# bminixhofer/zett

Measured on AMD Instinct MI355X. Metric: predicted token-embeddings/sec (full target vocab), higher is better.
Workload: dtype f16

## Files before the change

### include/zett_hip.h

```cpp
#ifndef ZETT_HIP_H
#define ZETT_HIP_H

#include <stdint.h>

#ifdef __cplusplus
extern "C" {
#endif

#define ZETT_ABI_VERSION 8

enum zett_status {
    ZETT_OK = 0,
    ZETT_E_INVALID = -1,
    ZETT_E_HIP = -2,
    ZETT_E_STATE = -3,
    ZETT_E_INDEX = -4,
    ZETT_E_NOT_IMPLEMENTED = -5,
    ZETT_E_KEY = -6,
    ZETT_E_RANGE = -7
};

enum zett_range_bits {
    ZETT_RANGE_SOURCE = 1,
    ZETT_RANGE_ACTIVATION = 2,
    ZETT_RANGE_OUTPUT = 4,
    ZETT_RANGE_WEIGHT = 8,
    ZETT_RANGE_DEST = 16
};

enum zett_dtype { ZETT_F32 = 0, ZETT_F16 = 1, ZETT_BF16 = 2 };

enum zett_precision { ZETT_PREC_BF16 = 0, ZETT_PREC_F32 = 1, ZETT_PREC_F16 = 2 };

typedef struct zett_config {
    int32_t n_embd;
    int32_t n_in_embd;
    int32_t hidden;
    int32_t intermediate;
    int32_t heads;
    int32_t layers;
    int32_t n_extra;
    int32_t original_vocab_size;
    int32_t pad_token_id;
    int32_t separate_out;
    int32_t single_head;
    int32_t rescale;
    int32_t predict_bias;
    int32_t embed_lang;
    int32_t n_langs;
    int32_t max_positions;
    float ln_eps_encoder;
    float ln_eps_projector;
} zett_config;

typedef struct zett_stats {
    int64_t rows;
    int64_t packed_tokens;
    int64_t distinct_ids;
    int64_t chunks;
    double executed_flops;
    double gemm_ms;
    int64_t gemm_launches;
    double gemm_flops_timed;
    int64_t distinct_positions;
} zett_stats;

typedef struct zett_hypernet zett_hypernet;
typedef struct zett_retok zett_retok;
typedef struct zett_lexical zett_lexical;

const char* zett_last_error(void);
int zett_abi_version(void);


int zett_create(const zett_config* cfg, int device, int precision, zett_hypernet** out);
int zett_destroy(zett_hypernet* h);

int zett_load_weight(zett_hypernet* h, const char* name, const void* data, int dtype,
                     const int64_t* shape, int ndim);

int zett_finalize(zett_hypernet* h);

int zett_forward(zett_hypernet* h, const int32_t* surface_forms, int64_t n_rows, int32_t seq,
                 const void* source_embeddings, int src_dtype, int64_t v_src, int32_t lang_index,
                 float* out_in, float* out_out, float* out_bias, void* stream);

typedef struct zett_dest {
    void* in; void* out; void* bias;
    int32_t dtype; int32_t bias_dtype;
    int64_t ld_in; int64_t ld_out;
    const int64_t* rows;
    int64_t n_dest_rows;
} zett_dest;
int zett_forward_into(zett_hypernet* h, const int32_t* surface_forms, int64_t n_rows, int32_t seq,
                      const void* source_embeddings, int src_dtype, int64_t v_src, int32_t lang_index,
                      const zett_dest* dest, void* stream);

int zett_forward_prepare(zett_hypernet* h, const int32_t* surface_forms, int64_t n_rows, int32_t seq, void* input_stream);

int zett_get_stats(const zett_hypernet* h, zett_stats* out);

typedef struct zett_gemm_record {
    int32_t m, n, k;
    int32_t variant;
    int32_t epilogue;
    float ms;
    double flops;
    double bytes;
} zett_gemm_record;
int zett_get_gemm_log(const zett_hypernet* h, zett_gemm_record* out, int64_t capacity, int64_t* count);

int zett_check_range(zett_hypernet* h, void* stream, int32_t* flags);

enum zett_output { ZETT_OUT_IN = 0, ZETT_OUT_BIAS = 1 };
int zett_stream_wait_output(zett_hypernet* h, int which, void* stream);

int zett_workspace_bytes(const zett_hypernet* h, int64_t n_rows, int32_t seq, int64_t* out_bytes);

int zett_set_option(zett_hypernet* h, const char* key, int64_t value);

int zett_partition_workspace_bytes(int64_t n_rows, int32_t n_ids, int64_t* out_bytes);
int zett_partition_rows(const int32_t* surface_forms, int64_t n_rows, int32_t seq, int32_t pad_id, int32_t n_ids, int32_t world,
                        const int32_t* caps, int32_t* perm_out, void* workspace, int64_t workspace_bytes, int32_t device, void* stream);
int zett_scatter_rows(const void* src, void* dst, const int64_t* order, int64_t n_rows, int64_t row_bytes, int32_t device, void* stream);

int zett_table_plan(zett_hypernet* h, const int32_t* surface_forms, int64_t n_rows, int32_t seq, int32_t* id_slot_out, int32_t* id_list_out,
                    int64_t* n_ids_out, void* stream);
int zett_table_rows(zett_hypernet* h, const int32_t* id_list, int64_t first, int64_t count, const void* source_embeddings, int src_dtype,
                    int64_t v_src, void* table_out, float* stats_out, void* stream);
int zett_forward_table(zett_hypernet* h, const int32_t* surface_forms, int64_t n_rows, int32_t seq, const void* table, const float* table_stats,
                       const int32_t* id_slot, int32_t lang_index, float* out_in, float* out_out, float* out_bias, void* stream);
int zett_forward_table_into(zett_hypernet* h, const int32_t* surface_forms, int64_t n_rows, int32_t seq, const void* table,
                            const float* table_stats, const int32_t* id_slot, int32_t lang_index, const zett_dest* dest, void* stream);


enum zett_retok_kind { ZETT_RETOK_BPE = 0, ZETT_RETOK_UNIGRAM = 1, ZETT_RETOK_WORDPIECE = 2 };

typedef struct zett_retok_model {
    int32_t kind;
    int32_t n_pieces;
    const uint8_t* piece_bytes;
    const int32_t* piece_offsets;
    const int32_t* piece_ids;
    const double* piece_scores;
    double unigram_min_score;
    int32_t n_merges;
    const int32_t* merges;
    int32_t unk_id;
    int32_t fuse_unk;
    int32_t byte_fallback;
    const int32_t* byte_fallback_ids;
    int32_t ignore_merges;
    int32_t n_special;
    const uint8_t* special_bytes;
    const int32_t* special_offsets;
    const int32_t* special_ids;
    const uint8_t* piece_continuing;
    int32_t max_input_chars_per_word;
} zett_retok_model;

int zett_retok_create(const zett_retok_model* model, int device, zett_retok** out);
int zett_retok_destroy(zett_retok* r);
int zett_retok_set_option(zett_retok* r, const char* key, int64_t value);

int zett_retokenize(zett_retok* r, const uint8_t* token_chars, const int32_t* offsets,
                    int64_t n_tokens, int32_t maxlen, int32_t pad_id, int32_t* out,
                    int64_t* n_truncated, int64_t* bad_token, void* stream);

int zett_retokenize_async(zett_retok* r, const uint8_t* token_chars, const int32_t* offsets, int64_t n_tokens, int64_t n_text,
                          int32_t maxlen, int32_t pad_id, int32_t* out, void* stream);
int zett_retok_result(zett_retok* r, int64_t* n_truncated, int64_t* bad_call, int64_t* bad_token);

enum zett_lexical_mode { ZETT_LEXICAL_NO = 0, ZETT_LEXICAL_FVT = 1, ZETT_LEXICAL_BFVT = 2 };

int zett_lexical_create(const zett_retok_model* model, int32_t n_vocab, const uint8_t* vocab_bytes, const int32_t* vocab_offsets,
                        const int32_t* vocab_ids, int device, zett_lexical** out);
int zett_lexical_destroy(zett_lexical* h);

int zett_lexical_plan(zett_lexical* h, const uint8_t* token_chars, int64_t n_tokens, int64_t n_text, int64_t n_source_rows, int32_t fvt_mode,
                      int32_t width, int32_t* ids, int32_t* count, int64_t* n_overlap, int64_t* n_wide, int64_t* n_ids, int64_t* bad_token,
                      void* stream);

int zett_lexical_rows_into(zett_lexical* h, const int32_t* ids, const int32_t* count, int64_t n_tokens, int32_t width, const void* src_in,
                           int64_t ld_src_in, const void* src_out, int64_t ld_src_out, int32_t src_dtype, int64_t n_source_rows, int32_t n_embd,
                           int64_t fallback_id, const zett_dest* dest, void* stream);

int zett_op_gemm_f32(const float* a, int32_t lda, const float* w, int32_t ldw, int64_t m, int32_t n, int32_t k, const float* bias, int32_t act,
                     const float* residual, int32_t ld_res, float* out, int32_t ld_out, void* stream);
int zett_op_gemm_lo(int32_t prec, const void* a, int32_t lda, const void* w, int32_t ldw, int64_t m, int32_t n, int32_t k, const float* bias, int32_t act,
                    const float* residual, int32_t ld_res, float* out, int32_t ld_out, void* stream);
int zett_op_convert_lo(int32_t prec, const float* in, int32_t ld_in, void* out, int32_t ld_out, int64_t rows, int32_t cols, int32_t cols_padded, void* stream);
int zett_op_transpose_lo(int32_t prec, const float* in, int32_t ld_in, void* out, int32_t ld_out, int64_t rows, int32_t cols, int64_t rows_padded, void* stream);
int zett_op_transpose_lo16(int32_t prec, const void* in, int32_t ld_in, void* out, int32_t ld_out, int64_t rows, int32_t cols, int64_t rows_padded, void* stream);
int zett_op_grad_operands_lo(int32_t prec, const float* dy, int32_t ld, const float* act_z, int32_t ld_z, int32_t act_kind, int64_t rows, int32_t cols,
                             int64_t rows_padded, void* dy_lo, int32_t ld_lo, void* dy_t, int32_t ld_t, float* colsum_part, void* stream);
int zett_op_transpose_f32(const float* in, int32_t ld_in, float* out, int32_t ld_out, int64_t rows, int32_t cols, int64_t rows_padded, void* stream);
int zett_op_colsum_f32(const float* in, int32_t ld, int64_t rows, int32_t cols, float* out, int32_t accumulate, void* stream);
int zett_op_elementwise_f32(int32_t op, const float* a, const float* b, const float* vec, const float* vec2, const float* s, float* out,
                            int64_t n, int32_t cols, void* stream);
int zett_op_rowdot_f32(const float* a, int32_t ld, const float* w, const float* b, float* out, int64_t rows, int32_t cols, void* stream);
int zett_op_layernorm_fwd_f32(const float* x, int32_t ld, const float* gamma, const float* beta, float eps, float* y, float* stats,
                              int64_t rows, int32_t h, void* y_lo, int32_t prec, void* stream);
int zett_op_layernorm_bwd_f32(const float* dy, const float* dy2, const float* x, int32_t ld, const float* stats, const float* gamma, float* dx,
                              float* partials, int32_t n_part, int64_t rows, int32_t h, void* stream);
int zett_op_gelu_fwd_f32(const float* z, float* h, int64_t n, int32_t kind, void* stream);
int zett_op_gelu_bwd_f32(const float* z, const float* dh, float* dz, int64_t n, int32_t kind, void* stream);
int zett_op_gelu_fwd_lo(int32_t prec, const float* z, void* h_lo, int64_t n, int32_t kind, void* stream);
int zett_op_attention_fwd_f32(const float* q, int32_t ldq, const float* k, const float* v, int32_t ld, const uint8_t* mask, const int32_t* row_offset,
                              int64_t n_rows, int32_t seq, int32_t heads, int32_t head_dim, int32_t cls_only, float* ctx, int32_t ld_ctx, float* probs,
                              void* ctx_lo, int32_t prec, void* stream);
int zett_op_attention_bwd_f32(const float* dctx, int32_t ld_ctx, const float* q, int32_t ldq, const float* k, const float* v, int32_t ld, const float* probs,
                              const int32_t* row_offset, int64_t n_rows, int32_t seq, int32_t heads, int32_t head_dim, int32_t cls_only, float* dq, int32_t ld_dq,
                              float* dk, float* dv, int32_t ld_d, void* stream);
int zett_op_gather_rows_f32(const float* a, const float* src, int32_t ld_src, const int32_t* idx, float* out, int64_t rows, int32_t cols, void* stream);
int zett_op_scatter_add_rows_f32(float* dst, int32_t ld_dst, const int32_t* idx, const float* src, int64_t rows, int32_t cols, void* stream);
int zett_op_gather_fwd_f32(const int32_t* ids, int64_t n_tokens, const void* src, int32_t src_dtype, int32_t e_in, int32_t v0, const float* fallback,
                           const float* sw, const float* sb, float* x, void* stream);
int zett_op_gather_bwd_f32(const int32_t* ids, int64_t n_tokens, const void* src, int32_t src_dtype, int32_t e_in, int32_t v0, const float* dx,
                           float* dfallback, float* prod, float* keep, void* stream);
int zett_op_gather_bwd_rows_f32(const int32_t* ids, int64_t n_tokens, const void* src, int32_t src_dtype, int32_t e_in, int32_t v0, const float* dx, float* prod,
                                float* keep, void* stream);

enum zett_ln_kernel {
    ZETT_LN_ROWS8_32 = 0,
    ZETT_LN_ROWS8_64 = 1,
    ZETT_LN_WAVE = 2,
    ZETT_LN_WORKGROUP = 3
};
int zett_op_fwd_layernorm(int32_t prec, const float* in, const void* in_lo, int32_t ld_in, int32_t rows, int32_t h, const float* gamma, const float* beta,
                          float eps, int32_t ln_rows8, float* out_f32, void* out_lo, float* stats, const float* bias_w, const float* bias_b, void* out_bias,
                          const int64_t* bias_rows, int32_t bias_dtype, int32_t* range_flag, int32_t* kernel_id, void* stream);
int zett_op_fwd_embed_layernorm(int32_t prec, const float* table, const void* table_lo, const float* table_stats, const float* table_gamma, const float* table_beta,
                                const int32_t* tok_slot, const int32_t* tok_pos, const float* type0, const float* pos_emb, const float* lang, int32_t lang_pos,
                                const int32_t* tok_row, const int32_t* row_offset, int64_t row0, int32_t rows, int32_t tok0, int32_t m, int32_t h, const float* gamma,
                                const float* beta, float eps, int32_t ln_rows8, void* out_lo, float* stats, float* sum, int32_t* kernel_id, void* stream);
int zett_op_fwd_attention(int32_t prec, const void* q, int64_t ldq, const void* k, const void* v, int64_t ldkv, int32_t h, int32_t head_dim,
                          const int32_t* row_offset, const uint8_t* row_uniform, const uint8_t* tok_key, int64_t row0, int32_t rows, int32_t tok0, float scaling,
                          int32_t flags, const int32_t* tok_pair, void* ctx, void* stream);
int zett_op_fwd_gather_src(int32_t prec, const int32_t* id_list, int32_t slot0, int32_t n_slots, const void* src, int32_t src_dtype, int32_t e_in, int32_t v0,
                           const float* fallback, const float* sc_w, const float* sc_b, void* out, int32_t* range_flag, void* stream);
int zett_op_fwd_ln_stats(int32_t prec, const float* parts, int32_t ld_part, int32_t rows, int32_t h, float eps, float* stats, void* stream);
int zett_op_fwd_fold_weight(int32_t prec, const float* w, int32_t n, int32_t k, const float* gamma, const float* beta, const float* bias, void* w_fold,
                            float* c_out, float* b_out, int32_t* range_flag, void* stream);

enum zett_distance { ZETT_DIST_MSE = 0, ZETT_DIST_RMSE = 1, ZETT_DIST_HUBER = 2 };
enum zett_loss_mode { ZETT_LOSS_MEAN = 0, ZETT_LOSS_LEXICAL = 1 };
enum zett_adamw_flags { ZETT_ADAMW_DECAY = 1, ZETT_ADAMW_FROZEN = 2 };
#define ZETT_MT_CHUNK 65536
int zett_op_single_token_mask(const void* ids, int32_t ids_bytes, int64_t n, int32_t width, int64_t ld, int64_t pad_token_id, float* mask, void* stream);
int zett_op_embed_dist_rows(const float* pred, int64_t ld_pred, const void* src, int32_t src_dtype, int64_t ld_src, int64_t src_rows, int32_t col0, const void* ids,
                            int32_t ids_bytes, int64_t ids_stride, const float* mask, int64_t n, int32_t e, int32_t kind, float* row_dist, float* row_tnorm,
                            void* stream);
int zett_op_embed_dist_finalize(const float* row_dist, const float* row_tnorm, const float* mask, int64_t n, int32_t mode, float* record, void* stream);
// ... 128 lines not shown
```

### zett_amd/_lib.py

```python
from __future__ import annotations

import ctypes as C
import os
import threading

from .build import LIB_PATH

ZETT_OK = 0
E_INVALID, E_HIP, E_STATE, E_INDEX, E_NOT_IMPLEMENTED, E_KEY, E_RANGE = -1, -2, -3, -4, -5, -6, -7
RANGE_SOURCE, RANGE_ACTIVATION, RANGE_OUTPUT, RANGE_WEIGHT, RANGE_DEST = 1, 2, 4, 8, 16
DTYPE_F32, DTYPE_F16, DTYPE_BF16 = 0, 1, 2
PREC_BF16, PREC_F32, PREC_F16 = 0, 1, 2
RETOK_BPE, RETOK_UNIGRAM, RETOK_WORDPIECE = 0, 1, 2
OUT_IN, OUT_BIAS = 0, 1
LEXICAL_NO, LEXICAL_FVT, LEXICAL_BFVT = 0, 1, 2
DIST_MSE, DIST_RMSE, DIST_HUBER = 0, 1, 2
LOSS_MEAN, LOSS_LEXICAL = 0, 1
ADAMW_DECAY, ADAMW_FROZEN = 1, 2
MT_CHUNK = 65536
CE_AUTO, CE_ONCE, CE_TWICE = 0, 1, 2
CE_ONCE_MAX_COLS = 32768
SPLICE_MAX_ROWS = 256
EMBED_BWD_CHUNK = 64
BATCH_POSITIVES_ONLY, BATCH_RANDOM = 0, 1
BATCH_BAD_ID, BATCH_OVERFLOW, BATCH_BAD_ORDER, BATCH_REPEAT = 1, 2, 4, 8
LABEL_CLM, LABEL_MLM = 0, 1
LABEL_BAD_ID = 1
LABEL_WORKSPACE_BYTES = 16384
ENCODE_MAX_TEMPLATE = 8
ENCODE_MARKS_ARE_LETTERS, ENCODE_RESPLIT = 1, 2
ENCODE_PREFIX_NONE, ENCODE_PREFIX_ALWAYS, ENCODE_PREFIX_UNLESS_SPACE = 0, 1, 2
ENCODE_NO_UNK, ENCODE_BAD_OFFSETS = 1, 2
SAMPLE_BAD_OFFSETS, SAMPLE_TABLE_FULL, SAMPLE_LIST_FULL, SAMPLE_SUM_OVERFLOW, SAMPLE_OUT_FULL = 2, 4, 8, 16, 32
VOCAB_NOT_A_SAMPLE, VOCAB_DUPLICATE, VOCAB_TABLE_FULL, VOCAB_OUT_FULL = 1, 2, 4, 8
VOCAB_SCORES_THROUGH_JSON = 1
SAMPLED_VOCAB_KEY_BYTES = 64

ABI_SYMBOLS = (
    "zett_last_error", "zett_abi_version", "zett_create", "zett_destroy", "zett_load_weight",
    "zett_finalize", "zett_forward", "zett_get_stats", "zett_workspace_bytes", "zett_set_option",
    "zett_retok_create", "zett_retok_destroy", "zett_retokenize", "zett_check_range", "zett_get_gemm_log",
    "zett_stream_wait_output", "zett_forward_prepare", "zett_retokenize_async", "zett_retok_result", "zett_retok_set_option",
    "zett_partition_rows", "zett_partition_workspace_bytes", "zett_scatter_rows",
    "zett_table_plan", "zett_table_rows", "zett_forward_table",
    "zett_forward_into", "zett_forward_table_into",
    "zett_lexical_create", "zett_lexical_destroy", "zett_lexical_plan", "zett_lexical_rows_into",
    "zett_op_gemm_f32", "zett_op_transpose_f32", "zett_op_colsum_f32", "zett_op_elementwise_f32", "zett_op_rowdot_f32",
    "zett_op_layernorm_fwd_f32", "zett_op_layernorm_bwd_f32", "zett_op_gelu_fwd_f32", "zett_op_gelu_bwd_f32",
    "zett_op_attention_fwd_f32", "zett_op_attention_bwd_f32", "zett_op_gather_fwd_f32", "zett_op_gather_bwd_f32",
    "zett_op_gather_rows_f32", "zett_op_scatter_add_rows_f32", "zett_op_gemm_lo", "zett_op_convert_lo", "zett_op_transpose_lo", "zett_op_grad_operands_lo", "zett_op_transpose_lo16", "zett_op_gelu_fwd_lo",
    "zett_op_single_token_mask", "zett_op_embed_dist_rows", "zett_op_embed_dist_finalize", "zett_op_embed_dist_grad", "zett_op_grad_norm", "zett_op_adamw",
    "zett_op_ce_addend", "zett_op_ce_rows", "zett_op_ce_finalize", "zett_op_ce_colsum", "zett_op_ce_scale", "zett_op_ce_cast",
    "zett_op_splice_rows", "zett_op_embed_lookup", "zett_op_embed_lookup_workspace_bytes", "zett_op_embed_lookup_plan", "zett_op_embed_lookup_bwd",
    "zett_op_batch_vocab_workspace_bytes", "zett_op_batch_vocab",
    "zett_op_label_batch", "zett_op_pad_vocabulary",
    "zett_encode_workspace_bytes", "zett_encode_texts",
    "zett_sampler_create", "zett_sampler_destroy", "zett_sampler_depth", "zett_sampler_workspace_bytes", "zett_sampler_sample", "zett_sampler_table",
    "zett_retok_create_unigram_device", "zett_sampled_vocab_workspace_bytes", "zett_sampled_vocab_build", "zett_sampled_vocab_commit", "zett_sampled_vocab_table",
    "zett_sampled_vocab_patch_rows",
    "zett_op_embed_lookup_plan_base", "zett_op_gather_bwd_rows_f32",
    "zett_op_fwd_layernorm", "zett_op_fwd_embed_layernorm", "zett_op_fwd_attention", "zett_op_fwd_gather_src", "zett_op_fwd_ln_stats", "zett_op_fwd_fold_weight",
)


class ZettConfig(C.Structure):
    _fields_ = [(n, C.c_int32) for n in (
        "n_embd", "n_in_embd", "hidden", "intermediate", "heads", "layers", "n_extra",
        "original_vocab_size", "pad_token_id", "separate_out", "single_head", "rescale",
        "predict_bias", "embed_lang", "n_langs", "max_positions")] + [
        ("ln_eps_encoder", C.c_float), ("ln_eps_projector", C.c_float)]


ABI_VERSION = 8


class ZettStats(C.Structure):
    _fields_ = [("rows", C.c_int64), ("packed_tokens", C.c_int64), ("distinct_ids", C.c_int64),
                ("chunks", C.c_int64), ("executed_flops", C.c_double), ("gemm_ms", C.c_double),
                ("gemm_launches", C.c_int64), ("gemm_flops_timed", C.c_double), ("distinct_positions", C.c_int64)]


class ZettGemmRecord(C.Structure):
    _fields_ = [("m", C.c_int32), ("n", C.c_int32), ("k", C.c_int32), ("variant", C.c_int32), ("epilogue", C.c_int32),
                ("ms", C.c_float), ("flops", C.c_double), ("bytes", C.c_double)]


class ZettDest(C.Structure):
    _fields_ = [("in_", C.c_void_p), ("out", C.c_void_p), ("bias", C.c_void_p), ("dtype", C.c_int32), ("bias_dtype", C.c_int32),
                ("ld_in", C.c_int64), ("ld_out", C.c_int64), ("rows", C.c_void_p), ("n_dest_rows", C.c_int64)]


class ZettSampledVocabRecord(C.Structure):
    _fields_ = [("n_vocab", C.c_int32), ("n_removed", C.c_int32), ("n_text", C.c_int32), ("status", C.c_int32), ("min_score", C.c_double), ("table_min_score", C.c_double)]


class ZettRetokModel(C.Structure):
    _fields_ = [
        ("kind", C.c_int32), ("n_pieces", C.c_int32),
        ("piece_bytes", C.c_void_p), ("piece_offsets", C.c_void_p), ("piece_ids", C.c_void_p),
        ("piece_scores", C.c_void_p), ("unigram_min_score", C.c_double),
        ("n_merges", C.c_int32), ("merges", C.c_void_p),
        ("unk_id", C.c_int32), ("fuse_unk", C.c_int32), ("byte_fallback", C.c_int32),
        ("byte_fallback_ids", C.c_void_p), ("ignore_merges", C.c_int32),
        ("n_special", C.c_int32), ("special_bytes", C.c_void_p), ("special_offsets", C.c_void_p),
        ("special_ids", C.c_void_p),
        ("piece_continuing", C.c_void_p), ("max_input_chars_per_word", C.c_int32),
    ]


_lib = None
_lock = threading.Lock()


def lib_path() -> str:
    return os.environ.get("ZETT_HIP_LIB", LIB_PATH)


def load():
    global _lib
    if _lib is not None:
        return _lib
    with _lock:
        if _lib is not None:
            return _lib
        path = lib_path()
        if not os.path.exists(path):
            raise RuntimeError(
                f"{path} is missing: the HIP extension has not been built. Run "
                "`python -m zett_amd.build` (needs hipcc); zett_amd has no CPU fallback.")
        lib = C.CDLL(path)
        lib.zett_last_error.restype = C.c_char_p
        lib.zett_abi_version.restype = C.c_int
        lib.zett_create.argtypes = [C.POINTER(ZettConfig), C.c_int, C.c_int, C.POINTER(C.c_void_p)]
        lib.zett_destroy.argtypes = [C.c_void_p]
        lib.zett_load_weight.argtypes = [C.c_void_p, C.c_char_p, C.c_void_p, C.c_int, C.POINTER(C.c_int64), C.c_int]
        lib.zett_finalize.argtypes = [C.c_void_p]
        lib.zett_forward.argtypes = [C.c_void_p, C.c_void_p, C.c_int64, C.c_int32, C.c_void_p, C.c_int, C.c_int64,
                                     C.c_int32, C.c_void_p, C.c_void_p, C.c_void_p, C.c_void_p]
        lib.zett_get_stats.argtypes = [C.c_void_p, C.POINTER(ZettStats)]
        lib.zett_workspace_bytes.argtypes = [C.c_void_p, C.c_int64, C.c_int32, C.POINTER(C.c_int64)]
        lib.zett_set_option.argtypes = [C.c_void_p, C.c_char_p, C.c_int64]
        lib.zett_check_range.argtypes = [C.c_void_p, C.c_void_p, C.POINTER(C.c_int32)]
        lib.zett_stream_wait_output.argtypes = [C.c_void_p, C.c_int, C.c_void_p]
        lib.zett_get_gemm_log.argtypes = [C.c_void_p, C.POINTER(ZettGemmRecord), C.c_int64, C.POINTER(C.c_int64)]
        lib.zett_retok_create.argtypes = [C.POINTER(ZettRetokModel), C.c_int, C.POINTER(C.c_void_p)]
        lib.zett_retok_destroy.argtypes = [C.c_void_p]
        lib.zett_retok_set_option.argtypes = [C.c_void_p, C.c_char_p, C.c_int64]
        lib.zett_retokenize.argtypes = [C.c_void_p, C.c_void_p, C.c_void_p, C.c_int64, C.c_int32, C.c_int32,
                                        C.c_void_p, C.POINTER(C.c_int64), C.POINTER(C.c_int64), C.c_void_p]
        lib.zett_retokenize_async.argtypes = [C.c_void_p, C.c_void_p, C.c_void_p, C.c_int64, C.c_int64, C.c_int32, C.c_int32,
                                              C.c_void_p, C.c_void_p]
        lib.zett_retok_result.argtypes = [C.c_void_p, C.POINTER(C.c_int64), C.POINTER(C.c_int64), C.POINTER(C.c_int64)]
        lib.zett_forward_prepare.argtypes = [C.c_void_p, C.c_void_p, C.c_int64, C.c_int32, C.c_void_p]
        lib.zett_table_plan.argtypes = [C.c_void_p, C.c_void_p, C.c_int64, C.c_int32, C.c_void_p, C.c_void_p, C.POINTER(C.c_int64), C.c_void_p]
        lib.zett_table_rows.argtypes = [C.c_void_p, C.c_void_p, C.c_int64, C.c_int64, C.c_void_p, C.c_int, C.c_int64, C.c_void_p, C.c_void_p, C.c_void_p]
        lib.zett_forward_table.argtypes = [C.c_void_p, C.c_void_p, C.c_int64, C.c_int32, C.c_void_p, C.c_void_p, C.c_void_p, C.c_int32,
                                           C.c_void_p, C.c_void_p, C.c_void_p, C.c_void_p]
        lib.zett_forward_into.argtypes = [C.c_void_p, C.c_void_p, C.c_int64, C.c_int32, C.c_void_p, C.c_int, C.c_int64, C.c_int32,
                                          C.POINTER(ZettDest), C.c_void_p]
        lib.zett_forward_table_into.argtypes = [C.c_void_p, C.c_void_p, C.c_int64, C.c_int32, C.c_void_p, C.c_void_p, C.c_void_p, C.c_int32,
                                                C.POINTER(ZettDest), C.c_void_p]
        lib.zett_lexical_create.argtypes = [C.POINTER(ZettRetokModel), C.c_int32, C.c_void_p, C.c_void_p, C.c_void_p, C.c_int, C.POINTER(C.c_void_p)]
        lib.zett_lexical_destroy.argtypes = [C.c_void_p]
        lib.zett_lexical_plan.argtypes = [C.c_void_p, C.c_void_p, C.c_int64, C.c_int64, C.c_int64, C.c_int32, C.c_int32, C.c_void_p, C.c_void_p,
                                          C.POINTER(C.c_int64), C.POINTER(C.c_int64), C.POINTER(C.c_int64), C.POINTER(C.c_int64), C.c_void_p]
        lib.zett_lexical_rows_into.argtypes = [C.c_void_p, C.c_void_p, C.c_void_p, C.c_int64, C.c_int32, C.c_void_p, C.c_int64, C.c_void_p, C.c_int64,
                                               C.c_int32, C.c_int64, C.c_int32, C.c_int64, C.POINTER(ZettDest), C.c_void_p]
        lib.zett_partition_workspace_bytes.argtypes = [C.c_int64, C.c_int32, C.POINTER(C.c_int64)]
        lib.zett_scatter_rows.argtypes = [C.c_void_p, C.c_void_p, C.c_void_p, C.c_int64, C.c_int64, C.c_int32, C.c_void_p]
        lib.zett_partition_rows.argtypes = [C.c_void_p, C.c_int64, C.c_int32, C.c_int32, C.c_int32, C.c_int32, C.POINTER(C.c_int32),
                                            C.c_void_p, C.c_void_p, C.c_int64, C.c_int32, C.c_void_p]
        P, I32, I64, F = C.c_void_p, C.c_int32, C.c_int64, C.c_float
        lib.zett_op_gemm_f32.argtypes = [P, I32, P, I32, I64, I32, I32, P, I32, P, I32, P, I32, P]
        lib.zett_op_transpose_f32.argtypes = [P, I32, P, I32, I64, I32, I64, P]
        lib.zett_op_gemm_lo.argtypes = [I32, P, I32, P, I32, I64, I32, I32, P, I32, P, I32, P, I32, P]
        lib.zett_op_convert_lo.argtypes = [I32, P, I32, P, I32, I64, I32, I32, P]
        lib.zett_op_transpose_lo.argtypes = [I32, P, I32, P, I32, I64, I32, I64, P]
        lib.zett_op_grad_operands_lo.argtypes = [I32, P, I32, P, I32, I32, I64, I32, I64, P, I32, P, I32, P, P]
        lib.zett_op_transpose_lo16.argtypes = [I32, P, I32, P, I32, I64, I32, I64, P]
        lib.zett_op_gelu_fwd_lo.argtypes = [I32, P, P, I64, I32, P]
        lib.zett_op_colsum_f32.argtypes = [P, I32, I64, I32, P, I32, P]
        lib.zett_op_elementwise_f32.argtypes = [I32, P, P, P, P, P, P, I64, I32, P]
        lib.zett_op_rowdot_f32.argtypes = [P, I32, P, P, P, I64, I32, P]
        lib.zett_op_layernorm_fwd_f32.argtypes = [P, I32, P, P, F, P, P, I64, I32, P, I32, P]
        lib.zett_op_layernorm_bwd_f32.argtypes = [P, P, P, I32, P, P, P, P, I32, I64, I32, P]
        lib.zett_op_gelu_fwd_f32.argtypes = [P, P, I64, I32, P]
        lib.zett_op_gelu_bwd_f32.argtypes = [P, P, P, I64, I32, P]
        lib.zett_op_attention_fwd_f32.argtypes = [P, I32, P, P, I32, P, P, I64, I32, I32, I32, I32, P, I32, P, P, I32, P]
        lib.zett_op_attention_bwd_f32.argtypes = [P, I32, P, I32, P, P, I32, P, P, I64, I32, I32, I32, I32, P, I32, P, P, I32, P]
        lib.zett_op_gather_rows_f32.argtypes = [P, P, I32, P, P, I64, I32, P]
        lib.zett_op_scatter_add_rows_f32.argtypes = [P, I32, P, P, I64, I32, P]
        lib.zett_op_gather_fwd_f32.argtypes = [P, I64, P, I32, I32, I32, P, P, P, P, P]
        lib.zett_op_gather_bwd_f32.argtypes = [P, I64, P, I32, I32, I32, P, P, P, P, P]
        lib.zett_op_gather_bwd_rows_f32.argtypes = [P, I64, P, I32, I32, I32, P, P, P, P]
        D = C.c_double
        lib.zett_op_single_token_mask.argtypes = [P, I32, I64, I32, I64, I64, P, P]
        lib.zett_op_embed_dist_rows.argtypes = [P, I64, P, I32, I64, I64, I32, P, I32, I64, P, I64, I32, I32, P, P, P]
        lib.zett_op_embed_dist_finalize.argtypes = [P, P, P, I64, I32, P, P]
        lib.zett_op_embed_dist_grad.argtypes = [P, I64, P, I32, I64, I64, I32, P, I32, I64, P, P, I64, I32, I32, P, P, P, I64, I32, P]
        lib.zett_op_grad_norm.argtypes = [P, P, I32, D, D, D, P, I64, P, P]
        lib.zett_op_adamw.argtypes = [P, P, P, P, P, P, I32, D, D, D, D, D, I32, P, P]
        lib.zett_op_ce_addend.argtypes = [P, P, P, I32, I32, P, P]
        lib.zett_op_ce_rows.argtypes = [P, I64, P, P, I64, I32, I32, P, I32, I64, P, P, P, I32, P]
        lib.zett_op_ce_finalize.argtypes = [P, P, P, P, I64, P, P]
        lib.zett_op_ce_colsum.argtypes = [P, I32, I64, I64, I32, P, I32, P]
        lib.zett_op_ce_scale.argtypes = [P, I64, P, P, P, I32, P]
        lib.zett_op_ce_cast.argtypes = [P, I32, I64, P, I32, I64, I64, I32, I32, P]
        lib.zett_op_splice_rows.argtypes = [P, I64, P, I64, I64, I32, P, I32, I64, I64, I32, P, P, I32, P]
        lib.zett_op_embed_lookup.argtypes = [P, I32, I64, I64, I32, P, I32, I64, P, I32, P, P]
        lib.zett_op_embed_lookup_workspace_bytes.argtypes = [I64, I64, I32, C.POINTER(I64), C.POINTER(I64), C.POINTER(I64)]
        lib.zett_op_embed_lookup_plan.argtypes = [P, I32, I64, I64, P, I64, P, I64, P]
        lib.zett_op_embed_lookup_plan_base.argtypes = [P, I32, I64, I64, I64, P, I64, P, I64, P]
        lib.zett_op_embed_lookup_bwd.argtypes = [P, I32, I64, I64, I32, P, I64, P, I64, P, I64, P]
        lib.zett_op_batch_vocab_workspace_bytes.argtypes = [I64, I64, I64, C.POINTER(I64)]
        lib.zett_op_batch_vocab.argtypes = [P, I32, P, I32, I64, I64, I64, P, I32, I64, I32, P, P, I32, I32, P, P, P, I32, P, P, P, P, P, P, P, P, P, I64, P]
        U64 = C.c_uint64
        lib.zett_op_label_batch.argtypes = [P, I32, I64, I64, I32, P, I32, P, I32, I64, I64, I64, I64, I32, U64, U64, U64, U64, P, I64, P, P, P, P, P, I64, P]
        lib.zett_op_pad_vocabulary.argtypes = [P, I32, I64, I32, I64, I64, P, I32, P, P, P, P, P]
        lib.zett_encode_workspace_bytes.argtypes = [I64, I64, C.POINTER(I64)]
        lib.zett_encode_texts.argtypes = [P, P, P, I64, I64, P, I64, I32, I32, I32, P, I32, P, I32, P, P, I32, I32, P, P, I32, I64, P, I64, P, P]
        lib.zett_sampler_create.argtypes = [C.c_int, I32, I64, I64, I64, C.POINTER(P)]
        lib.zett_sampler_destroy.argtypes = [P]
        lib.zett_sampler_depth.argtypes = [P, C.POINTER(I32)]
        lib.zett_sampler_workspace_bytes.argtypes = [I64, I64, C.POINTER(I64)]
        lib.zett_sampler_sample.argtypes = [P, P, P, I64, I64, P, I64, I64, I32, I32, C.c_double, C.c_uint64, I32, I32, P, P, P, I64, P, P, I64, P, P]
        lib.zett_sampler_table.argtypes = [P, P, P, P, P, I64, P, P]
        lib.zett_retok_create_unigram_device.argtypes = [C.c_int, I64, C.POINTER(P)]
        lib.zett_sampled_vocab_workspace_bytes.argtypes = [I64, I32, C.POINTER(I64)]
        lib.zett_sampled_vocab_build.argtypes = [P, P, P, P, P, I64, I64, P, P, P, P, P, I32, I32, I32, P, P, P, I64, P, I64, P, I32, P, I64, P]
        lib.zett_sampled_vocab_commit.argtypes = [P, P]
        lib.zett_sampled_vocab_table.argtypes = [P, P, P, P, P, P, I64, P, P]
        lib.zett_sampled_vocab_patch_rows.argtypes = [P, P, P, P, I32, P, I64, I32, I32, P]
        lib.zett_op_fwd_layernorm.argtypes = [I32, P, P, I32, I32, I32, P, P, F, I32, P, P, P, P, P, P, P, I32, P, C.POINTER(I32), P]
        lib.zett_op_fwd_embed_layernorm.argtypes = [I32, P, P, P, P, P, P, P, P, P, P, I32, P, P, I64, I32, I32, I32, I32, P, P, F, I32, P, P, P, C.POINTER(I32), P]
        lib.zett_op_fwd_attention.argtypes = [I32, P, I64, P, P, I64, I32, I32, P, P, P, I64, I32, I32, F, I32, P, P, P]
        lib.zett_op_fwd_gather_src.argtypes = [I32, P, I32, I32, P, I32, I32, I32, P, P, P, P, P, P]
        lib.zett_op_fwd_ln_stats.argtypes = [I32, P, I32, I32, I32, F, P, P]
        lib.zett_op_fwd_fold_weight.argtypes = [I32, P, I32, I32, P, P, P, P, P, P, P, P]
        for name in ABI_SYMBOLS:
            fn = getattr(lib, name)
            if name != "zett_last_error":
                fn.restype = C.c_int
        if lib.zett_abi_version() != ABI_VERSION:
            raise RuntimeError(f"{path} has ABI version {lib.zett_abi_version()}, this package expects {ABI_VERSION}: "
                               "rebuild it (`python -m zett_amd.build`)")
        _lib = lib
    return _lib


class RangeError(OverflowError):
    """ZETT_E_RANGE: a value left the range of the 16-bit operand type, or an output is not finite."""


def check(rc: int, what: str = "") -> None:
    if rc == ZETT_OK:
        return
    msg = load().zett_last_error().decode("utf-8", "replace")
    if what:
        msg = f"{what}: {msg}"
    if rc == E_INDEX:
        raise IndexError(msg)
    if rc == E_NOT_IMPLEMENTED:
        raise NotImplementedError(msg)
    if rc == E_KEY:
        raise KeyError(msg)
    if rc == E_INVALID:
        raise ValueError(msg)
    if rc == E_RANGE:
        raise RangeError(msg)
    raise RuntimeError(msg)
```

### zett_amd/csrc/rowops.hip.h

```cpp
#pragma once

#include <hip/hip_runtime.h>
#include <stdint.h>

#include <type_traits>

#include "gemm.hip.h"
#include "scan.hip.h"

namespace zett {



struct PlanArrays {
    int32_t* row_count;
    int32_t* row_offset;
    uint8_t* row_uniform;
    int32_t* id_flag;
    int32_t* id_slot;
    int32_t* id_list;
    int32_t* tok_slot;
    int32_t* tok_pos;
    int32_t* tok_row;
    int32_t* tok_pkey;
    int32_t* pair_flag;
    int32_t* pair_slot;
    int32_t* tok_pair;
    int32_t* pair_tslot;
    int32_t* pair_pos;
    uint8_t* tok_key;
    int32_t* err;
    int32_t* counters;
    int32_t n_pair_keys;
};

static __global__ void plan_rows_kernel(const int32_t* __restrict__ sfm, int64_t n_rows, int seq, int pad, int lam,
                                 int n_ids, PlanArrays p) {
    const int64_t n = (int64_t)blockIdx.x * blockDim.x + threadIdx.x;
    if (n >= n_rows) return;
    const int32_t* row = sfm + n * seq;
    int visible = 0;
    for (int j = 0; j < seq; ++j) {
        const int id = row[j];
        if (id < 0 || id >= n_ids) {
            atomicMax(p.err, (int)(n < 0x7ffffffe ? n + 1 : 0x7fffffff));
            p.row_count[n] = 0;
            p.row_uniform[n] = 2;
            return;
        }
        visible += (id != pad);
    }
    const bool uniform = (visible + lam) == 0;
    int count;
    if (uniform) {
        count = seq;
        for (int j = 0; j < seq; ++j) p.id_flag[row[j]] = 1;
    } else {
        count = visible + lam + (row[0] == pad ? 1 : 0);
        for (int j = 0; j < seq; ++j)
            if (j == 0 || row[j] != pad) p.id_flag[row[j]] = 1;
    }
    p.row_count[n] = count;
    p.row_uniform[n] = uniform ? 1 : 0;
}

static __global__ __launch_bounds__(1024) void exclusive_scan_kernel(const int32_t* __restrict__ in,
                                                              int32_t* __restrict__ out, int64_t n) {
    __shared__ int32_t s_waves[16];
    const int t = threadIdx.x;
    const int64_t per = (n + 1023) / 1024;
    const int64_t b = (int64_t)t * per, e = (b + per < n) ? b + per : n;
    int32_t s = 0;
    for (int64_t i = b; i < e; ++i) s += in[i];
    int32_t total;
    int32_t run = block_exclusive_scan<1024>(s, s_waves, &total);
    for (int64_t i = b; i < e; ++i) { const int32_t v = in[i]; out[i] = run; run += v; }
    if (t == 1023) out[n] = total;
}

constexpr int SCAN_CHUNK = 4096;

static __global__ __launch_bounds__(256) void scan_chunk_sums_kernel(const int32_t* __restrict__ in, int64_t n, int32_t* __restrict__ sums) {
    __shared__ int32_t s_waves[4];
    const int64_t base = (int64_t)blockIdx.x * SCAN_CHUNK + threadIdx.x * 16;
    int32_t s = 0;
#pragma unroll
    for (int k = 0; k < 16; ++k) { const int64_t i = base + k; if (i < n) s += in[i]; }
    int32_t total;
    block_exclusive_scan<256>(s, s_waves, &total);
    if (threadIdx.x == 0) sums[blockIdx.x] = total;
}

static __global__ __launch_bounds__(256) void scan_apply_kernel(const int32_t* __restrict__ in, int64_t n, const int32_t* __restrict__ offs,
                                                         int32_t* __restrict__ out) {
    __shared__ int32_t s_waves[4];
    const int64_t base = (int64_t)blockIdx.x * SCAN_CHUNK + threadIdx.x * 16;
    int32_t v[16];
    int32_t s = 0;
#pragma unroll
    for (int k = 0; k < 16; ++k) { const int64_t i = base + k; v[k] = i < n ? in[i] : 0; s += v[k]; }
    int32_t run = offs[blockIdx.x] + block_exclusive_scan<256>(s, s_waves);
#pragma unroll
    for (int k = 0; k < 16; ++k) { const int64_t i = base + k; if (i < n) out[i] = run; run += v[k]; }
    if (blockIdx.x == gridDim.x - 1 && threadIdx.x == 0) out[n] = offs[gridDim.x];
}

inline void launch_exclusive_scan(const int32_t* in, int32_t* out, int64_t n, int32_t* scratch, hipStream_t st) {
    if (n <= SCAN_CHUNK * 4) {
        hipLaunchKernelGGL(exclusive_scan_kernel, dim3(1), dim3(1024), 0, st, in, out, n);
        return;
    }
    const int chunks = (int)((n + SCAN_CHUNK - 1) / SCAN_CHUNK);
    int32_t* sums = scratch;
    int32_t* offs = scratch + chunks;
    hipLaunchKernelGGL(scan_chunk_sums_kernel, dim3(chunks), dim3(256), 0, st, in, n, sums);
    hipLaunchKernelGGL(exclusive_scan_kernel, dim3(1), dim3(1024), 0, st, (const int32_t*)sums, offs, (int64_t)chunks);
    hipLaunchKernelGGL(scan_apply_kernel, dim3(chunks), dim3(256), 0, st, in, n, (const int32_t*)offs, out);
}

static __global__ void plan_tokens_kernel(const int32_t* __restrict__ sfm, int64_t n_rows, int seq, int pad, int lam,
                                   int n_ids, PlanArrays p) {
    const int64_t n = (int64_t)blockIdx.x * blockDim.x + threadIdx.x;
    if (n >= n_rows) return;
    const int32_t* row = sfm + n * seq;
    int t = p.row_offset[n];
    if (p.row_uniform[n] == 2) return;
    const bool uniform = p.row_uniform[n] == 1;
    const int lp = seq + lam;
    for (int j = 0; j < seq; ++j) {
        const int id = row[j];
        const bool vis = id != pad;
        if (uniform || vis || j == 0) {
            p.tok_slot[t] = p.id_slot[id];
            p.tok_pos[t] = j;
            p.tok_row[t] = (int32_t)n;
            p.tok_key[t] = vis ? 1 : 0;
            if (p.pair_flag) { const int key = id * lp + j; p.tok_pkey[t] = key; p.pair_flag[key] = 1; }
            ++t;
        }
    }
    if (lam) {
        p.tok_slot[t] = -1;
        p.tok_pos[t] = seq;
        p.tok_row[t] = (int32_t)n;
        p.tok_key[t] = 1;
        if (p.pair_flag) { const int key = n_ids * lp + seq; p.tok_pkey[t] = key; p.pair_flag[key] = 1; }
    }
}

static __global__ void plan_pairs_kernel(int64_t n_rows, PlanArrays p) {
    const int64_t t = (int64_t)blockIdx.x * blockDim.x + threadIdx.x;
    if (t >= p.row_offset[n_rows]) return;
    const int ps = p.pair_slot[p.tok_pkey[t]];
    p.tok_pair[t] = ps;
    p.pair_tslot[ps] = p.tok_slot[t];
    p.pair_pos[ps] = p.tok_pos[t];
}

__device__ __forceinline__ int chunk_row(int t_rel, int row_rel, bool first, int rows);
static __global__ void pair_rows_kernel(int m, int tok0, int64_t row0, int rows, PlanArrays p, int32_t* __restrict__ brow_pair) {
    const int t = blockIdx.x * blockDim.x + threadIdx.x;
    if (t >= m) return;
    const int n = p.tok_row[tok0 + t];
    brow_pair[chunk_row(t, (int)(n - row0), p.row_offset[n] == tok0 + t, rows)] = p.tok_pair[tok0 + t];
}

static __global__ void plan_idlist_kernel(int n_ids, PlanArrays p) {
    const int id = blockIdx.x * blockDim.x + threadIdx.x;
    if (id < n_ids && p.id_flag[id]) p.id_list[p.id_slot[id]] = id;
    if (id == 0) {
        p.counters[0] = p.id_slot[n_ids];
        p.counters[1] = p.err[0];
        p.counters[2] = p.n_pair_keys ? p.pair_slot[p.n_pair_keys] : 0;
    }
}

__device__ __forceinline__ float wave_sum(float v) {
#pragma unroll
    for (int off = 32; off > 0; off >>= 1) v += __shfl_xor(v, off, 64);
    return v;
}

__device__ __forceinline__ float block_sum_256(float v, float* red ) {
    v = wave_sum(v);
    __syncthreads();
    if ((threadIdx.x & 63) == 0) red[threadIdx.x >> 6] = v;
    __syncthreads();
    return red[0] + red[1] + red[2] + red[3];
}

template <typename T> __device__ __forceinline__ void store_lo4(T* dst, float4 v);
template <> __device__ __forceinline__ void store_lo4<float>(float* dst, float4 v) { *(float4*)dst = v; }
template <> __device__ __forceinline__ void store_lo4<bf16_t>(bf16_t* dst, float4 v) {
    *(uint2*)dst = make_uint2(pack2_lo<bf16_t>(v.x, v.y), pack2_lo<bf16_t>(v.z, v.w));
}
template <> __device__ __forceinline__ void store_lo4<f16_t>(f16_t* dst, float4 v) {
    *(uint2*)dst = make_uint2(pack2_lo<f16_t>(v.x, v.y), pack2_lo<f16_t>(v.z, v.w));
}

template <int SRC_DTYPE> __device__ __forceinline__ float4 load_src4(const void* base, size_t elem);
template <> __device__ __forceinline__ float4 load_src4<0>(const void* base, size_t e) {
    return *(const float4*)((const float*)base + e);
}
template <> __device__ __forceinline__ float4 load_src4<1>(const void* base, size_t e) {
    const uint2 u = *(const uint2*)((const uint16_t*)base + e);
    typedef __attribute__((ext_vector_type(4))) _Float16 f16x4;
    const f16x4 hv = __builtin_bit_cast(f16x4, u);
    return make_float4((float)hv[0], (float)hv[1], (float)hv[2], (float)hv[3]);
}
template <> __device__ __forceinline__ float4 load_src4<2>(const void* base, size_t e) {
    const uint2 u = *(const uint2*)((const uint16_t*)base + e);
    return make_float4(__uint_as_float(u.x << 16), __uint_as_float(u.x & 0xffff0000u),
                       __uint_as_float(u.y << 16), __uint_as_float(u.y & 0xffff0000u));
}

template <typename T, int SRC_DTYPE>
__global__ __launch_bounds__(256) void gather_src_kernel(const int32_t* __restrict__ id_list, int slot0, int n_slots,
                                                         const void* __restrict__ src, int e_in, int v0,
                                                         const float* __restrict__ fallback,
                                                         const float* __restrict__ sc_w, const float* __restrict__ sc_b,
                                                         T* __restrict__ out, int32_t* __restrict__ range_flag) {
    const int s = blockIdx.x;
    if (s >= n_slots) return;
    const int id = id_list[slot0 + s];
    T* dst = out + (size_t)s * e_in;
    bool bad = false;
    auto chk = [&](float4 v) {
        if (LoRange<T>::checked)
            bad |= out_of_range(v.x, LoRange<T>::limit) | out_of_range(v.y, LoRange<T>::limit) | out_of_range(v.z, LoRange<T>::limit) |
                   out_of_range(v.w, LoRange<T>::limit);
    };
    if (id >= v0) {
        const float* f = fallback + (size_t)(id - v0) * e_in;
        for (int c = threadIdx.x * 4; c < e_in; c += 1024) { const float4 v = *(const float4*)(f + c); chk(v); store_lo4<T>(dst + c, v); }
    } else {
        const size_t base = (size_t)id * e_in;
        for (int c = threadIdx.x * 4; c < e_in; c += 1024) {
            float4 v = load_src4<SRC_DTYPE>(src, base + c);
            if (sc_w) {
                const float4 w = *(const float4*)(sc_w + c), b = *(const float4*)(sc_b + c);
                v.x = w.x * v.x + b.x; v.y = w.y * v.y + b.y; v.z = w.z * v.z + b.z; v.w = w.w * v.w + b.w;
            }
            chk(v);
            store_lo4<T>(dst + c, v);
        }
    }
    range_report(range_flag, bad, ZETT_RANGE_BIT_SOURCE);
}

struct LnEmbed {
    const float* table;
    const int32_t* tok_slot;
    const int32_t* tok_pos;
    const float* type0;
    const float* pos_emb;
    const float* lang;
    int lang_pos;
    const int32_t* tok_row;
    const int32_t* row_offset;
    int64_t row0;
    int rows;
    const void* table_lo;
    const float* table_stats;
    const float* table_gamma;
    const float* table_beta;
};

__device__ __forceinline__ int chunk_row(int t_rel, int row_rel, bool first, int rows) {
    return first ? row_rel : rows + t_rel - row_rel - 1;
}

struct LnReadout {
    const float* bias_w;
    const float* bias_b;
    float* out_bias;
    const void* in_lo;
    const int64_t* bias_rows;
    int32_t* range_flag;
};

template <typename BT> __device__ __forceinline__ void ln_readout_store(const LnReadout& ro, int r, float v) {
    if constexpr (std::is_void<BT>::value) {
        ro.out_bias[r] = v;
    } else {
        const int64_t d = ro.bias_rows ? ro.bias_rows[r] : (int64_t)r;
        if (d < 0) return;
        ((BT*)ro.out_bias)[d] = to_lo<BT>(v);
        range_report(ro.range_flag, dest_overflow<BT>(v), ZETT_RANGE_BIT_DEST);
    }
}

constexpr int LN_MAX_VEC = 8;

template <typename T, bool EMBED, int TPR = 256, bool READOUT = false, typename BT = void>
__global__ __launch_bounds__(256) void layernorm_rows_kernel(const float* __restrict__ in, int ld_in, int rows, int H,
                                                             const float* __restrict__ gamma,
                                                             const float* __restrict__ beta, float eps,
                                                             float* __restrict__ out_f32, T* __restrict__ out_lo,
                                                             float* __restrict__ stats_out, float* __restrict__ sum_out,
                                                             LnEmbed emb, int tok0, LnReadout readout) {
    __shared__ float red[4];
    const int r = blockIdx.x * (256 / TPR) + (int)threadIdx.x / TPR;
    if (r >= rows) return;
    const int nvec = H >> 2;
    const int tid = threadIdx.x % TPR;
    auto row_sum = [&](float x_) { return TPR == 256 ? block_sum_256(x_, red) : wave_sum(x_); };
    const float* x = nullptr;
    const float* posr = nullptr;
    bool is_lang = false;
    int ro = r;
    const T* tbl_lo = nullptr;
    float2 tbl_st = make_float2(0.f, 1.f);
    if constexpr (EMBED) {
        const int slot = emb.tok_slot[tok0 + r];
        is_lang = slot < 0;
        if (emb.table_lo && !is_lang) {
            tbl_lo = (const T*)emb.table_lo + (size_t)slot * H;
            tbl_st = *(const float2*)(emb.table_stats + 2 * (size_t)slot);
            x = emb.lang;
        } else
        x = is_lang ? emb.lang : emb.table + (size_t)slot * H;
        posr = emb.pos_emb + (size_t)emb.tok_pos[tok0 + r] * H;
        if (emb.tok_row) {
            const int n = emb.tok_row[tok0 + r];
            ro = chunk_row(r, (int)(n - emb.row0), emb.row_offset[n] == tok0 + r, emb.rows);
        }
    } else {
        x = in + (size_t)r * ld_in;
    }
    auto load = [&](int v) -> float4 {
        if constexpr (READOUT && sizeof(T) == 2) {
            if (readout.in_lo) {
                const uint2 u = *(const uint2*)((const T*)readout.in_lo + (size_t)r * ld_in + v * 4);
                float4 a;
                unpack2_lo<T>(u.x, a.x, a.y); unpack2_lo<T>(u.y, a.z, a.w);
                return a;
            }
        }
        float4 a;
        if constexpr (EMBED && sizeof(T) == 2) {
            if (tbl_lo) {
                const uint2 u = *(const uint2*)(tbl_lo + v * 4);
                unpack2_lo<T>(u.x, a.x, a.y); unpack2_lo<T>(u.y, a.z, a.w);
                const float4 g = *(const float4*)(emb.table_gamma + v * 4), b = *(const float4*)(emb.table_beta + v * 4);
                a = make_float4(ln_affine(a.x, tbl_st.x, tbl_st.y, g.x, b.x), ln_affine(a.y, tbl_st.x, tbl_st.y, g.y, b.y),
                                ln_affine(a.z, tbl_st.x, tbl_st.y, g.z, b.z), ln_affine(a.w, tbl_st.x, tbl_st.y, g.w, b.w));
            } else {
                a = *(const float4*)(x + v * 4);
            }
        } else {
            a = *(const float4*)(x + v * 4);
        }
        if constexpr (EMBED) {
            const float4 t0 = *(const float4*)(emb.type0 + v * 4);
            const float4 p = *(const float4*)(posr + v * 4);
            if (is_lang) {
                const float4 pl = *(const float4*)(emb.pos_emb + (size_t)emb.lang_pos * H + v * 4);
                a.x -= (t0.x + pl.x); a.y -= (t0.y + pl.y); a.z -= (t0.z + pl.z); a.w -= (t0.w + pl.w);
            }
            a.x = (a.x + t0.x) + p.x; a.y = (a.y + t0.y) + p.y; a.z = (a.z + t0.z) + p.z; a.w = (a.w + t0.w) + p.w;
        }
        return a;
    };
    float4 v[LN_MAX_VEC];
    float s = 0.f;
#pragma unroll
    for (int j = 0; j < LN_MAX_VEC; ++j) {
        const int idx = tid + TPR * j;
        if (idx < nvec) { v[j] = load(idx); s += (v[j].x + v[j].y) + (v[j].z + v[j].w); }
    }
    for (int idx = tid + TPR * LN_MAX_VEC; idx < nvec; idx += TPR) { const float4 a = load(idx); s += (a.x + a.y) + (a.z + a.w); }
    const float mean = row_sum(s) / (float)H;
    float q = 0.f;
#pragma unroll
    for (int j = 0; j < LN_MAX_VEC; ++j) {
        const int idx = tid + TPR * j;
        if (idx < nvec) {
            const float a = v[j].x - mean, b = v[j].y - mean, c = v[j].z - mean, d = v[j].w - mean;
            q += (a * a + b * b) + (c * c + d * d);
        }
    }
    for (int idx = tid + TPR * LN_MAX_VEC; idx < nvec; idx += TPR) {
        const float4 t = load(idx);
        const float a = t.x - mean, b = t.y - mean, c = t.z - mean, d = t.w - mean;
        q += (a * a + b * b) + (c * c + d * d);
    }
    const float var = row_sum(q) / (float)H;
    const float rstd = 1.0f / sqrtf(var + eps);
    if (stats_out && tid == 0) *(float2*)(stats_out + 2 * (size_t)ro) = make_float2(mean, rstd);
    float dot = 0.f;
    auto emit = [&](int idx, float4 a) {
        const float4 g = *(const float4*)(gamma + idx * 4), b = *(const float4*)(beta + idx * 4);
        const float4 o = make_float4(ln_affine(a.x, mean, rstd, g.x, b.x), ln_affine(a.y, mean, rstd, g.y, b.y),
                                     ln_affine(a.z, mean, rstd, g.z, b.z), ln_affine(a.w, mean, rstd, g.w, b.w));
        if (EMBED && sum_out) *(float4*)(sum_out + (size_t)ro * H + idx * 4) = a;
        if (out_f32) *(float4*)(out_f32 + (size_t)ro * H + idx * 4) = o;
        if (out_lo) store_lo4<T>(out_lo + (size_t)ro * H + idx * 4, o);
        if (READOUT && readout.bias_w) {
            const float4 w = *(const float4*)(readout.bias_w + idx * 4);
            dot += (o.x * w.x + o.y * w.y) + (o.z * w.z + o.w * w.w);
        }
    };
#pragma unroll
    for (int j = 0; j < LN_MAX_VEC; ++j) {
        const int idx = tid + TPR * j;
        if (idx < nvec) emit(idx, v[j]);
    }
    for (int idx = tid + TPR * LN_MAX_VEC; idx < nvec; idx += TPR) emit(idx, load(idx));
    if constexpr (READOUT) {
        if (readout.out_bias) {
            const float tot = row_sum(dot);
            if (tid == 0) ln_readout_store<BT>(readout, r, readout.bias_w ? tot + readout.bias_b[0] : 0.f);
        }
    }
}

template <typename T> struct Vec8 { float v[8]; };

template <typename T> __device__ __forceinline__ void load8(const T* p, float (&o)[8]);
template <> __device__ __forceinline__ void load8<float>(const float* p, float (&o)[8]) {
    const float4 a = *(const float4*)p, b = *(const float4*)(p + 4);
    o[0] = a.x; o[1] = a.y; o[2] = a.z; o[3] = a.w; o[4] = b.x; o[5] = b.y; o[6] = b.z; o[7] = b.w;
}
template <typename T> __device__ __forceinline__ void load8_16bit(const T* p, float (&o)[8]) {
    const uint4 u = *(const uint4*)p;
    unpack2_lo<T>(u.x, o[0], o[1]); unpack2_lo<T>(u.y, o[2], o[3]);
    unpack2_lo<T>(u.z, o[4], o[5]); unpack2_lo<T>(u.w, o[6], o[7]);
}
template <> __device__ __forceinline__ void load8<bf16_t>(const bf16_t* p, float (&o)[8]) { load8_16bit<bf16_t>(p, o); }
template <> __device__ __forceinline__ void load8<f16_t>(const f16_t* p, float (&o)[8]) { load8_16bit<f16_t>(p, o); }
template <typename T> __device__ __forceinline__ void store8(T* p, const float (&o)[8]);
template <> __device__ __forceinline__ void store8<float>(float* p, const float (&o)[8]) {
    *(float4*)p = make_float4(o[0], o[1], o[2], o[3]);
    *(float4*)(p + 4) = make_float4(o[4], o[5], o[6], o[7]);
}
template <typename T> __device__ __forceinline__ void store8_16bit(T* p, const float (&o)[8]) {
    *(uint4*)p = make_uint4(pack2_lo<T>(o[0], o[1]), pack2_lo<T>(o[2], o[3]), pack2_lo<T>(o[4], o[5]), pack2_lo<T>(o[6], o[7]));
}
template <> __device__ __forceinline__ void store8<bf16_t>(bf16_t* p, const float (&o)[8]) { store8_16bit<bf16_t>(p, o); }
template <> __device__ __forceinline__ void store8<f16_t>(f16_t* p, const float (&o)[8]) { store8_16bit<f16_t>(p, o); }

template <int TPR>
__device__ __forceinline__ float group_sum(float v) {
#pragma unroll
    for (int off = TPR / 2; off > 0; off >>= 1) v += __shfl_xor(v, off, 64);
    return v;
}

inline int ln_rows8_tpr(int H) {
    if (H % 256 == 0 && H <= 1024) return 32;
    if (H % 512 == 0 && H <= 2048) return 64;
    return 0;
}

template <typename T, bool EMBED, int TPR, bool READOUT, typename BT = void>
__global__ __launch_bounds__(256) void layernorm_rows8_kernel(const float* __restrict__ in, int ld_in, int rows, int H,
                                                              const float* __restrict__ gamma,
                                                              const float* __restrict__ beta, float eps,
                                                              float* __restrict__ out_f32, T* __restrict__ out_lo,
                                                              float* __restrict__ stats_out, float* __restrict__ sum_out,
                                                              LnEmbed emb, int tok0, LnReadout readout) {
    static_assert(sizeof(T) == 2 && (TPR == 32 || TPR == 64), "16-bit operand types, 32 or 64 lanes per row");
    constexpr int NVMAX = 4;
    const int r = blockIdx.x * (256 / TPR) + (int)threadIdx.x / TPR;
    if (r >= rows) return;
    const int nv = H / (8 * TPR);
    const int tid = threadIdx.x % TPR;
    const float* x = nullptr;
    const float* posr = nullptr;
    bool is_lang = false;
    int ro = r;
    const T* tbl_lo = nullptr;
    float2 tbl_st = make_float2(0.f, 1.f);
    if constexpr (EMBED) {
        const int slot = emb.tok_slot[tok0 + r];
        is_lang = slot < 0;
        if (emb.table_lo && !is_lang) {
            tbl_lo = (const T*)emb.table_lo + (size_t)slot * H;
            tbl_st = *(const float2*)(emb.table_stats + 2 * (size_t)slot);
            x = emb.lang;
        } else
        x = is_lang ? emb.lang : emb.table + (size_t)slot * H;
        posr = emb.pos_emb + (size_t)emb.tok_pos[tok0 + r] * H;
        if (emb.tok_row) {
            const int n = emb.tok_row[tok0 + r];
            ro = chunk_row(r, (int)(n - emb.row0), emb.row_offset[n] == tok0 + r, emb.rows);
        }
    } else {
        x = in + (size_t)r * ld_in;
    }
    auto load = [&](int c, float (&a)[8]) {
        bool have = false;
        if constexpr (READOUT) {
            if (readout.in_lo) { load8<T>((const T*)readout.in_lo + (size_t)r * ld_in + c, a); have = true; }
        }
        if constexpr (EMBED) {
            if (tbl_lo) {
                load8<T>(tbl_lo + c, a);
                float g[8], b[8];
                load8<float>(emb.table_gamma + c, g);
                load8<float>(emb.table_beta + c, b);
#pragma unroll
                for (int k = 0; k < 8; ++k) a[k] = ln_affine(a[k], tbl_st.x, tbl_st.y, g[k], b[k]);
                have = true;
            }
        }
        if (!have) load8<float>(x + c, a);
        if constexpr (EMBED) {
            float t0[8], p[8];
            load8<float>(emb.type0 + c, t0);
            load8<float>(posr + c, p);
            if (is_lang) {
                float pl[8];
                load8<float>(emb.pos_emb + (size_t)emb.lang_pos * H + c, pl);
#pragma unroll
                for (int k = 0; k < 8; ++k) a[k] -= (t0[k] + pl[k]);
            }
#pragma unroll
            for (int k = 0; k < 8; ++k) a[k] = (a[k] + t0[k]) + p[k];
        }
    };
    float v[NVMAX][8];
    float s = 0.f;
#pragma unroll
    for (int j = 0; j < NVMAX; ++j) {
        if (j < nv) {
            load((tid + TPR * j) * 8, v[j]);
            s += ((v[j][0] + v[j][1]) + (v[j][2] + v[j][3])) + ((v[j][4] + v[j][5]) + (v[j][6] + v[j][7]));
        }
    }
    const float mean = group_sum<TPR>(s) / (float)H;
    float q = 0.f;
#pragma unroll
    for (int j = 0; j < NVMAX; ++j) {
        if (j < nv) {
            float d[8];
#pragma unroll
            for (int k = 0; k < 8; ++k) { d[k] = v[j][k] - mean; d[k] *= d[k]; }
            q += ((d[0] + d[1]) + (d[2] + d[3])) + ((d[4] + d[5]) + (d[6] + d[7]));
        }
    }
    const float var = group_sum<TPR>(q) / (float)H;
    const float rstd = 1.0f / sqrtf(var + eps);
    if (stats_out && tid == 0) *(float2*)(stats_out + 2 * (size_t)ro) = make_float2(mean, rstd);
    float dot = 0.f;
#pragma unroll
    for (int j = 0; j < NVMAX; ++j) {
        if (j < nv) {
            const int c = (tid + TPR * j) * 8;
            float g[8], b[8], o[8];
            load8<float>(gamma + c, g);
            load8<float>(beta + c, b);
#pragma unroll
            for (int k = 0; k < 8; ++k) o[k] = ln_affine(v[j][k], mean, rstd, g[k], b[k]);
            if (EMBED && sum_out) store8<float>(sum_out + (size_t)ro * H + c, v[j]);
            if (out_f32) store8<float>(out_f32 + (size_t)ro * H + c, o);
            if (out_lo) store8<T>(out_lo + (size_t)ro * H + c, o);
            if (READOUT && readout.bias_w) {
                float w[8];
                load8<float>(readout.bias_w + c, w);
                dot += ((o[0] * w[0] + o[1] * w[1]) + (o[2] * w[2] + o[3] * w[3])) + ((o[4] * w[4] + o[5] * w[5]) + (o[6] * w[6] + o[7] * w[7]));
            }
        }
    }
    if constexpr (READOUT) {
        if (readout.out_bias) {
            const float tot = group_sum<TPR>(dot);
            if (tid == 0) ln_readout_store<BT>(readout, r, readout.bias_w ? tot + readout.bias_b[0] : 0.f);
        }
    }
}

constexpr int ATT_FAST_KEYS = 8;

template <typename T> __device__ __forceinline__ float dot8_lo(const uint4& a, const uint4& b);
template <> __device__ __forceinline__ float dot8_lo<f16_t>(const uint4& a, const uint4& b) {
    typedef __attribute__((ext_vector_type(2))) _Float16 h2;
    float s = __builtin_amdgcn_fdot2(__builtin_bit_cast(h2, a.x), __builtin_bit_cast(h2, b.x), 0.f, false);
    s = __builtin_amdgcn_fdot2(__builtin_bit_cast(h2, a.y), __builtin_bit_cast(h2, b.y), s, false);
    s = __builtin_amdgcn_fdot2(__builtin_bit_cast(h2, a.z), __builtin_bit_cast(h2, b.z), s, false);
    return __builtin_amdgcn_fdot2(__builtin_bit_cast(h2, a.w), __builtin_bit_cast(h2, b.w), s, false);
}
template <> __device__ __forceinline__ float dot8_lo<bf16_t>(const uint4& a, const uint4& b) {
    float x[8], y[8];
    unpack2_lo<bf16_t>(a.x, x[0], x[1]); unpack2_lo<bf16_t>(a.y, x[2], x[3]); unpack2_lo<bf16_t>(a.z, x[4], x[5]); unpack2_lo<bf16_t>(a.w, x[6], x[7]);
    unpack2_lo<bf16_t>(b.x, y[0], y[1]); unpack2_lo<bf16_t>(b.y, y[2], y[3]); unpack2_lo<bf16_t>(b.z, y[4], y[5]); unpack2_lo<bf16_t>(b.w, y[6], y[7]);
    float s = 0.f;
#pragma unroll
    for (int c = 0; c < 8; ++c) s = fmaf(x[c], y[c], s);
    return s;
}
template <> __device__ __forceinline__ float dot8_lo<float>(const uint4&, const uint4&) { return 0.f; }

__device__ __forceinline__ float head_sum(float s, int lph) {
    auto dpp = [](float v, auto ctrl) {
        return __builtin_bit_cast(float, __builtin_amdgcn_update_dpp(0, __builtin_bit_cast(int, v), decltype(ctrl)::value, 0xf, 0xf, true));
    };
    if (lph >= 2) s += dpp(s, std::integral_constant<int, 0xB1>{});
    if (lph >= 4) s += dpp(s, std::integral_constant<int, 0x4E>{});
    if (lph >= 8) s += dpp(s, std::integral_constant<int, 0x141>{});
    if (lph >= 16) s += dpp(s, std::integral_constant<int, 0x140>{});
    if (lph >= 32) s += __builtin_bit_cast(float, __builtin_amdgcn_ds_swizzle(__builtin_bit_cast(int, s), (16 << 10) | 0x1f));
    if (lph >= 64) s += __shfl_xor(s, 32, 64);
    return s;
}

struct AttentionWaves { int64_t total, full; int full_groups, lanes_per_row; };
__host__ __device__ inline AttentionWaves attention_waves(int rows, int H, bool pack) {
    const int rem = H & 511, gfull = H >> 9;
    AttentionWaves a;
    if (pack && (rem == 256 || rem == 128 || rem == 64)) {
        a.full_groups = gfull; a.lanes_per_row = rem >> 3;
        a.full = (int64_t)rows * gfull;
        const int per = 64 / a.lanes_per_row;
        a.total = a.full + (rows + per - 1) / per;
    } else {
        a.full_groups = (H + 511) >> 9; a.lanes_per_row = 64;
        a.full = (int64_t)rows * a.full_groups;
        a.total = a.full;
    }
    return a;
}

template <typename T>
__global__ __launch_bounds__(256) void attention_rows_kernel(const T* __restrict__ qbase, size_t ldq,
                                                             const T* __restrict__ kbase, const T* __restrict__ vbase,
                                                             size_t ldkv, int H, int head_dim,
                                                             const int32_t* __restrict__ row_offset,
                                                             const uint8_t* __restrict__ row_uniform,
                                                             const uint8_t* __restrict__ tok_key, int64_t row0,
                                                             int rows, int tok0, float scaling, int flags ,
                                                             const int32_t* __restrict__ tok_pair, T* __restrict__ ctx) {
    const int cls_only = flags & 1;
    const int lane = threadIdx.x & 63;
    const int64_t w = (int64_t)blockIdx.x * 4 + (threadIdx.x >> 6);
    const AttentionWaves aw = attention_waves(rows, H, (flags & 4) != 0);
    if (w >= aw.total) return;
    int rl, grp, li = lane, base = 0, lpr = 64;
    bool valid = true;
    if (w < aw.full) { rl = (int)(w / aw.full_groups); grp = (int)(w % aw.full_groups); }
    else {
        lpr = aw.lanes_per_row;
        const int sub = lane / lpr;
        li = lane - sub * lpr;
        base = sub * lpr;
        rl = (int)(w - aw.full) * (64 / lpr) + sub;
        grp = aw.full_groups;
        valid = rl < rows;
        if (!valid) rl = rows - 1;
    }
    const int col = grp * 512 + li * 8;
    const bool active = valid && col < H;
    const int lph = head_dim >> 3;
    const int64_t n = row0 + rl;
    const int t0 = row_offset[n] - tok0, t1 = row_offset[n + 1] - tok0;
    const bool uniform = row_uniform[n];
    const int nq = cls_only ? 1 : (t1 - t0);
    const int ccol = active ? col : 0;
    auto brow = [&](int t) -> size_t { return (size_t)chunk_row(t, rl, t == t0, rows); };
    int pslot = 0;
    if (tok_pair) { const int t = t0 + li; pslot = t < t1 ? tok_pair[tok0 + t] : 0; }
    auto qrow = [&](int t) -> size_t {
        if (!tok_pair) return brow(t);
        return t - t0 < lpr ? (size_t)__shfl(pslot, base + (t - t0), 64) : (size_t)tok_pair[tok0 + t];
    };
    const int nk = t1 - t0;
    if constexpr (sizeof(T) == 2) {
        if (nk <= ATT_FAST_KEYS && (flags & 2)) {
            const bool mine = li < nk && (uniform || tok_key[tok0 + t0 + li] != 0);
            const unsigned on = (unsigned)(__ballot(mine) >> base) & (lpr >= 32 ? 0xffffffffu : ((1u << lpr) - 1u));
            uint4 kk[ATT_FAST_KEYS], vv[ATT_FAST_KEYS], qq[ATT_FAST_KEYS];
#pragma unroll
            for (int j = 0; j < ATT_FAST_KEYS; ++j) {
                if (j < nk) {
                    const size_t kr = qrow(t0 + j);
                    kk[j] = *(const uint4*)(kbase + kr * ldkv + ccol);
                    vv[j] = *(const uint4*)(vbase + kr * ldkv + ccol);
                    if (!cls_only) qq[j] = *(const uint4*)(qbase + kr * ldq + ccol);
                }
            }
            if (cls_only) qq[0] = *(const uint4*)(qbase + (size_t)rl * ldq + ccol);
            const float sc2 = scaling * 1.4426950408889634f;
#pragma unroll
            for (int qi = 0; qi < ATT_FAST_KEYS; ++qi) {
                if (qi < nq) {
                    float sj[ATT_FAST_KEYS];
                    float mx = -INFINITY;
#pragma unroll
                    for (int j = 0; j < ATT_FAST_KEYS; ++j) {
                        sj[j] = -INFINITY;
                        if (j < nk && ((on >> j) & 1u)) {
                            const float d = head_sum(dot8_lo<T>(qq[qi], kk[j]), lph);
                            sj[j] = uniform ? 0.f : d * sc2;
                            mx = fmaxf(mx, sj[j]);
                        }
                    }
                    float l = 0.f, acc[8];
#pragma unroll
                    for (int c = 0; c < 8; ++c) acc[c] = 0.f;
#pragma unroll
                    for (int j = 0; j < ATT_FAST_KEYS; ++j) {
                        if (j < nk && ((on >> j) & 1u)) {
                            const float pj = __builtin_amdgcn_exp2f(sj[j] - mx);
                            l += pj;
                            float v[8];
                            unpack2_lo<T>(vv[j].x, v[0], v[1]); unpack2_lo<T>(vv[j].y, v[2], v[3]);
                            unpack2_lo<T>(vv[j].z, v[4], v[5]); unpack2_lo<T>(vv[j].w, v[6], v[7]);
#pragma unroll
                            for (int c = 0; c < 8; ++c) acc[c] = fmaf(pj, v[c], acc[c]);
                        }
                    }
                    const float inv = 1.0f / l;
#pragma unroll
                    for (int c = 0; c < 8; ++c) acc[c] *= inv;
                    if (active) {
                        const size_t orow = cls_only ? (size_t)rl : brow(t0 + qi);
                        store8<T>(ctx + orow * H + col, acc);
                    }
                }
            }
            return;
        }
    }
    for (int qi = 0; qi < nq; ++qi) {
        float q[8];
        load8<T>(qbase + (cls_only ? (size_t)rl : qrow(t0 + qi)) * ldq + ccol, q);
        float mx = -INFINITY, l = 0.f, acc[8];
#pragma unroll
        for (int c = 0; c < 8; ++c) acc[c] = 0.f;
        for (int kj = t0; kj < t1; ++kj) {
            if (!uniform && !tok_key[tok0 + kj]) continue;
            float k[8], v[8];
            const size_t kr = qrow(kj);
            load8<T>(kbase + kr * ldkv + ccol, k);
            load8<T>(vbase + kr * ldkv + ccol, v);
            float s = 0.f;
#pragma unroll
            for (int c = 0; c < 8; ++c) s = fmaf(q[c], k[c], s);
            for (int off = 1; off < lph; off <<= 1) s += __shfl_xor(s, off, 64);
            s = uniform ? 0.f : s * scaling;
            const float nm = fmaxf(mx, s);
            const float corr = expf(mx - nm);
            const float p = expf(s - nm);
            l = fmaf(l, corr, p);
#pragma unroll
            for (int c = 0; c < 8; ++c) acc[c] = fmaf(acc[c], corr, p * v[c]);
            mx = nm;
        }
        const float inv = 1.0f / l;
#pragma unroll
        for (int c = 0; c < 8; ++c) acc[c] *= inv;
        if (active) {
            const size_t orow = cls_only ? (size_t)rl : brow(t0 + qi);
            store8<T>(ctx + orow * H + col, acc);
        }
    }
}

static __global__ __launch_bounds__(64) void ln_stats_kernel(const float2* __restrict__ part, int parts, int ld_part, int rows, int H, float eps,
                                                      float* __restrict__ stats) {
    const int r = blockIdx.x * blockDim.x + threadIdx.x;
    if (r >= rows) return;
    float s = 0.f, q = 0.f;
    const float2* col = part + r;
    int p = 0;
    for (; p + 8 <= parts; p += 8) {
        float2 v[8];
#pragma unroll
        for (int j = 0; j < 8; ++j) v[j] = col[(size_t)(p + j) * ld_part];
#pragma unroll
        for (int j = 0; j < 8; ++j) { s += v[j].x; q += v[j].y; }
    }
    {
        float2 v[8];
#pragma unroll
        for (int j = 0; j < 8; ++j) v[j] = p + j < parts ? col[(size_t)(p + j) * ld_part] : make_float2(0.f, 0.f);
#pragma unroll
        for (int j = 0; j < 8; ++j)
            if (p + j < parts) { s += v[j].x; q += v[j].y; }
    }
    const float mean = s / (float)H;
    const float var = fmaxf(q / (float)H - mean * mean, 0.f);
    *(float2*)(stats + 2 * (size_t)r) = make_float2(mean, 1.0f / sqrtf(var + eps));
}

template <typename T>
__global__ __launch_bounds__(256) void fold_weight_kernel(const float* __restrict__ w, int K, const float* __restrict__ gamma,
                                                          const float* __restrict__ beta, const float* __restrict__ bias,
                                                          T* __restrict__ w_fold, float* __restrict__ c_out, float* __restrict__ b_out,
                                                          int32_t* __restrict__ range_flag) {
    __shared__ float red[4];
    const int n = blockIdx.x;
    const float* row = w + (size_t)n * K;
    float cs = 0.f, bs = 0.f;
    for (int k = threadIdx.x; k < K; k += 256) {
        const float x = row[k];
        if (LoRange<T>::checked) range_report(range_flag, out_of_range(x * gamma[k], LoRange<T>::limit), ZETT_RANGE_BIT_WEIGHT);
        const T lo = to_lo<T>(x * gamma[k]);
        w_fold[(size_t)n * K + k] = lo;
        cs += lo_to_f32<T>(lo);
        bs = fmaf(x, beta[k], bs);
    }
    const float ct = block_sum_256(cs, red);
    const float bt = block_sum_256(bs, red);
    if (threadIdx.x == 0) { c_out[n] = ct; b_out[n] = bias[n] + bt; }
}

template <typename T>
__global__ void convert_f32_to_lo_kernel(const float* __restrict__ in, T* __restrict__ out, size_t n, int32_t* __restrict__ range_flag) {
    size_t i = ((size_t)blockIdx.x * blockDim.x + threadIdx.x) * 4;
    const size_t stride = (size_t)gridDim.x * blockDim.x * 4;
    bool bad = false;
    for (; i + 3 < n; i += stride) {
        const float4 v = *(const float4*)(in + i);
        if (LoRange<T>::checked)
            bad |= out_of_range(v.x, LoRange<T>::limit) | out_of_range(v.y, LoRange<T>::limit) | out_of_range(v.z, LoRange<T>::limit) |
                   out_of_range(v.w, LoRange<T>::limit);
        store_lo4<T>(out + i, v);
    }
    if (blockIdx.x == 0 && threadIdx.x == 0) {
        for (size_t j = n & ~(size_t)3; j < n; ++j) { out[j] = to_lo<T>(in[j]); if (LoRange<T>::checked) bad |= out_of_range(in[j], LoRange<T>::limit); }
    }
    range_report(range_flag, bad, ZETT_RANGE_BIT_WEIGHT);
}
template <int SRC_DTYPE>
__global__ void convert_to_f32_kernel(const void* __restrict__ in, float* __restrict__ out, size_t n) {
    size_t i = (size_t)blockIdx.x * blockDim.x + threadIdx.x;
    const size_t stride = (size_t)gridDim.x * blockDim.x;
    for (; i < n; i += stride) {
        if constexpr (SRC_DTYPE == 1) out[i] = (float)((const _Float16*)in)[i];
        else out[i] = __uint_as_float(((uint32_t)((const uint16_t*)in)[i]) << 16);
    }
}

template <typename OT> __device__ __forceinline__ void store4_dst(OT* d, float4 v) {
    if constexpr (std::is_same<OT, float>::value) *(float4*)d = v;
    else *(uint2*)d = make_uint2(pack2_lo<OT>(v.x, v.y), pack2_lo<OT>(v.z, v.w));
}

template <typename OT, bool VEC>
__global__ __launch_bounds__(256) void dest_store_rows_kernel(const float* __restrict__ src, int64_t ld_src, OT* __restrict__ dst, int64_t ld_dst,
                                                              const int64_t* __restrict__ rows, int64_t n_rows, int cols, int32_t* range_flag) {
    bool bad = false;
    for (int64_t i = blockIdx.x; i < n_rows; i += gridDim.x) {
        const int64_t d = rows ? rows[i] : i;
        if (d < 0) continue;
        const float* s = src + i * ld_src;
        OT* o = dst + d * ld_dst;
        if constexpr (VEC) {
            for (int c = (int)threadIdx.x * 4; c < cols; c += 256 * 4) {
                const float4 v = *(const float4*)(s + c);
                store4_dst<OT>(o + c, v);
                bad |= dest_overflow<OT>(v.x) | dest_overflow<OT>(v.y) | dest_overflow<OT>(v.z) | dest_overflow<OT>(v.w);
            }
        } else {
            for (int c = (int)threadIdx.x; c < cols; c += 256) {
                const float v = s[c];
                o[c] = to_lo<OT>(v);
                bad |= dest_overflow<OT>(v);
            }
        }
    }
    range_report(range_flag, bad, ZETT_RANGE_BIT_DEST);
}

static __global__ void dest_rows_check_kernel(const int64_t* __restrict__ rows, int64_t n, int64_t n_dest, int32_t* err) {
    const int64_t i = (int64_t)blockIdx.x * blockDim.x + threadIdx.x;
    if (i < n && rows[i] >= n_dest) atomicMax(err, (int)(i < 0x7ffffffe ? i + 1 : 0x7fffffff));
}

}
```

### zett_amd/csrc/rowops_launch.hip.h

```cpp
#pragma once

#include "../../include/zett_hip.h"
#include "rowops.hip.h"

namespace zett {

template <typename T, bool EMBED, bool READOUT, typename BT>
inline int launch_layernorm(hipStream_t st, int H, int ln_rows8, const float* in, int ld_in, int rows, const float* gamma, const float* beta, float eps,
                            float* of, T* ol, float* stats, float* sum, const LnEmbed& embed, int t0, const LnReadout& readout) {
    auto go = [&](auto kernel, dim3 grid) {
        hipLaunchKernelGGL(kernel, grid, dim3(256), 0, st, in, ld_in, rows, H, gamma, beta, eps, of, ol, stats, sum, embed, t0, readout);
    };
    if constexpr (sizeof(T) == 2) {
        if (const int tpr8 = ln_rows8 ? ln_rows8_tpr(H) : 0) {
            const dim3 grid8((rows + 256 / tpr8 - 1) / (256 / tpr8));
            if (tpr8 == 32) { go(layernorm_rows8_kernel<T, EMBED, 32, READOUT, BT>, grid8); return ZETT_LN_ROWS8_32; }
            go(layernorm_rows8_kernel<T, EMBED, 64, READOUT, BT>, grid8);
            return ZETT_LN_ROWS8_64;
        }
    }
    if (H <= 2048) { go(layernorm_rows_kernel<T, EMBED, 64, READOUT, BT>, dim3((rows + 3) / 4)); return ZETT_LN_WAVE; }
    go(layernorm_rows_kernel<T, EMBED, 256, READOUT, BT>, dim3(rows));
    return ZETT_LN_WORKGROUP;
}

template <typename T>
inline int launch_attention(hipStream_t st, int H, int attention_fast, int attention_pack, const T* q, size_t ldq, const T* k, const T* v, size_t ldkv,
                            int head_dim, const int32_t* row_offset, const uint8_t* row_uniform, const uint8_t* tok_key, int64_t row0, int rows, int tok0,
                            float scaling, int cls_only, const int32_t* tok_pair, T* ctx) {
    const int64_t waves = attention_waves(rows, H, attention_pack != 0).total;
    const int flags = (cls_only ? 1 : 0) | (attention_fast ? 2 : 0) | (attention_pack ? 4 : 0);
    hipLaunchKernelGGL((attention_rows_kernel<T>), dim3((unsigned)((waves + 3) / 4)), dim3(256), 0, st, q, ldq, k, v, ldkv, H, head_dim, row_offset,
                       row_uniform, tok_key, row0, rows, tok0, scaling, flags, tok_pair, ctx);
    return flags;
}

inline int launch_ln_stats(hipStream_t st, int H, const float2* parts, int ld_part, int rows, float eps, float* stats) {
    hipLaunchKernelGGL(ln_stats_kernel, dim3((rows + 63) / 64), dim3(64), 0, st, parts, H / 128, ld_part, rows, H, eps, stats);
    return H / 128;
}

template <typename T, int SRC_DTYPE>
inline int launch_gather_src(hipStream_t st, const int32_t* id_list, int slot0, int n_slots, const void* src, int e_in, int v0, const float* fallback,
                             const float* sc_w, const float* sc_b, T* out, int32_t* range_flag) {
    hipLaunchKernelGGL((gather_src_kernel<T, SRC_DTYPE>), dim3(n_slots), dim3(256), 0, st, id_list, slot0, n_slots, src, e_in, v0, fallback, sc_w, sc_b, out,
                       range_flag);
    return SRC_DTYPE;
}

template <typename T>
inline int launch_fold_weight(hipStream_t st, const float* w, int N, int K, const float* gamma, const float* beta, const float* bias, T* w_fold, float* c_out,
                              float* b_out, int32_t* range_flag) {
    hipLaunchKernelGGL(fold_weight_kernel<T>, dim3((unsigned)N), dim3(256), 0, st, w, K, gamma, beta, bias, w_fold, c_out, b_out, range_flag);
    return N;
}

}
```

### zett_amd/csrc/zett_hip.hip

```cpp
#include <hip/hip_runtime.h>

#include <algorithm>
#include <cstdlib>
#include <cmath>
#include <cstdarg>
#include <cstdio>
#include <cstring>
#include <map>
#include <string>
#include <type_traits>
#include <vector>

#include "../../include/zett_hip.h"
#include "common.hip.h"
#include "gemm.hip.h"
#include "gemm_launch.hip.h"
#include "rowops.hip.h"
#include "rowops_launch.hip.h"
#include "retok.hip.h"
#include "lexical.hip.h"
#include "partition.hip.h"

using namespace zett;

namespace {

struct Tensor {
    float* f32 = nullptr;
    void* lo = nullptr;
    std::vector<int64_t> shape;
    size_t numel = 0;
};

inline size_t round_up(size_t v, size_t m) { return (v + m - 1) / m * m; }

}

struct zett_hypernet {
    zett_config cfg{};
    int device = 0;
    int precision = ZETT_PREC_BF16;
    bool finalized = false;
    std::map<std::string, Tensor> w;
    std::vector<void*> qkv_w;
    std::vector<float*> qkv_b;
    struct Folded { void* w = nullptr; float* c = nullptr; float* b = nullptr; };
    std::vector<Folded> fold_qkv, fold_up;
    Folded fold_head_in, fold_head_out;
    float* head_one = nullptr;
    float* head_zero = nullptr;
    int ln_fold = 1;
    float* head_scale = nullptr;
    float* head_shift = nullptr;
    std::vector<void*> owned;
    int64_t max_chunk_tokens = 0;
    int time_gemm = 0;
    int cls_only_last = 1;
    int pair_dedupe = 1;
    int residual_lo = 1;
    int concurrent_lanes = 0;
    hipStream_t lane_stream = nullptr;
    hipEvent_t lane_ev[4] = {nullptr, nullptr, nullptr, nullptr};
    int attention_fast = 1;
    int attention_pack = 1;
    int gemm_tail_split = 1;
    int gemm_tile_order = 0;
    int ln_rows8 = 1;
    int table_lo = 1;
    int gemm_group = 0;
    int gemm4d_min_k = 512;
    int gemm_variant = 0;
    struct PlanSlot {
        DevBuf i32, u8;
        int32_t* host = nullptr;
        size_t host_ints = 0;
        hipEvent_t done = nullptr;
        hipEvent_t released = nullptr;
        const int32_t* sfm = nullptr;
        int64_t n_rows = 0;
        int seq = 0;
        bool pair_plan = false;
        const int32_t* ext_id_slot = nullptr;
        bool pending = false;
    } plan[2];
    PlanSlot table_plan;
    struct ExtTable { const void* table = nullptr; const float* stats = nullptr; const int32_t* id_slot = nullptr; } ext;
    int plan_cur = 0;
    hipStream_t plan_stream = nullptr;
    hipEvent_t plan_fork = nullptr;
    DevBuf table, x0, yf, yt, big, pre, ctx, cf, ct, lnstats, lnparts;
    hipEvent_t out_ready[2] = {nullptr, nullptr};
    bool out_recorded = false;
    int range_accumulate = 0;
    int32_t* range_word = nullptr;
    int32_t* range_host = nullptr;
    DevBuf dest_word, dest_stage[2], dest_sink;
    int32_t* dest_host = nullptr;
    hipEvent_t dest_checked = nullptr;
    std::vector<hipEvent_t> ev;
    size_t ev_used = 0;
    std::vector<zett_gemm_record> gemm_log;
    zett_stats stats{};
};

namespace {

size_t elt_size(int precision) { return precision == ZETT_PREC_F32 ? 4 : 2; }

bool is_gemm_weight(const std::string& n) {
    static const char* suffixes[] = {"input_projection.0.weight", "dense1.weight", "dense2.weight",
                                     "query.weight", "key.weight", "value.weight", "dense.weight",
                                     "output_projection.1.weight", "output_projection_out.1.weight"};
    for (const char* s : suffixes) {
        const size_t ls = strlen(s);
        if (n.size() >= ls && n.compare(n.size() - ls, ls, s) == 0) return true;
    }
    return false;
}

void expected_shapes(const zett_config& c, std::map<std::string, std::vector<int64_t>>& s) {
    const int64_t H = c.hidden, I = c.intermediate;
    auto proj = [&](const std::string& p) {
        s[p + "dense1.weight"] = {I, H}; s[p + "dense1.bias"] = {I};
        s[p + "dense2.weight"] = {H, I}; s[p + "dense2.bias"] = {H};
        s[p + "ln.weight"] = {H}; s[p + "ln.bias"] = {H};
    };
    if (c.embed_lang) s["lang_embeddings.weight"] = {c.n_langs, H};
    s["model.embeddings.token_type_embeddings.weight"] = {1, H};
    s["model.embeddings.LayerNorm.weight"] = {H};
    s["model.embeddings.LayerNorm.bias"] = {H};
    s["model.embeddings.position_embeddings.weight"] = {c.max_positions, H};
    for (int l = 0; l < c.layers; ++l) {
        const std::string p = "model.encoder.layer." + std::to_string(l) + ".";
        for (const char* q : {"query", "key", "value"}) {
            s[p + "attention.self." + q + ".weight"] = {H, H};
            s[p + "attention.self." + q + ".bias"] = {H};
        }
        s[p + "attention.output.dense.weight"] = {H, H}; s[p + "attention.output.dense.bias"] = {H};
        s[p + "attention.output.LayerNorm.weight"] = {H}; s[p + "attention.output.LayerNorm.bias"] = {H};
        s[p + "intermediate.dense.weight"] = {I, H}; s[p + "intermediate.dense.bias"] = {I};
        s[p + "output.dense.weight"] = {H, I}; s[p + "output.dense.bias"] = {H};
        s[p + "output.LayerNorm.weight"] = {H}; s[p + "output.LayerNorm.bias"] = {H};
    }
    s["fallback_embeddings.weight"] = {c.n_extra, c.n_in_embd};
    s["input_projection.0.weight"] = {H, c.n_in_embd}; s["input_projection.0.bias"] = {H};
    proj("input_projection.1.");
    proj("output_projection.0.");
    const int64_t w0 = c.single_head ? c.n_in_embd : c.n_embd;
    s["output_projection.1.weight"] = {w0, H}; s["output_projection.1.bias"] = {w0};
    if (c.separate_out && !c.single_head) {
        proj("output_projection_out.0.");
        s["output_projection_out.1.weight"] = {c.n_embd, H}; s["output_projection_out.1.bias"] = {c.n_embd};
    }
    if (c.rescale) {
        s["in_scaler.w"] = {1, c.n_in_embd}; s["in_scaler.b"] = {1, c.n_in_embd};
        s["scaler.w"] = {1, c.n_embd}; s["scaler.b"] = {1, c.n_embd};
        if (c.separate_out) { s["out_scaler.w"] = {1, c.n_embd}; s["out_scaler.b"] = {1, c.n_embd}; }
    }
    if (c.predict_bias) { s["bias_projection.weight"] = {1, H}; s["bias_projection.bias"] = {1}; }
}

int validate_config(const zett_config& c, int precision) {
    if (c.n_embd <= 0 || c.hidden <= 0 || c.intermediate <= 0 || c.heads <= 0 || c.layers <= 0)
        return fail(ZETT_E_INVALID, "non-positive dimension in zett_config");
    if (c.n_in_embd != (c.separate_out ? 2 * c.n_embd : c.n_embd))
        return fail(ZETT_E_INVALID, "n_in_embd must be 2*n_embd iff separate_out");
    if (c.hidden % c.heads) return fail(ZETT_E_INVALID, "hidden %d not divisible by heads %d", c.hidden, c.heads);
    const int d = c.hidden / c.heads;
    if (d < 8 || d > 512 || (d & (d - 1))) return fail(ZETT_E_INVALID, "head_dim %d unsupported (need a power of two in [8,512])", d);
    const int kq = precision == ZETT_PREC_F32 ? 32 : 64;
    for (int k : {c.n_in_embd, c.hidden, c.intermediate})
        if (k % kq) return fail(ZETT_E_INVALID, "contraction width %d is not a multiple of %d", k, kq);
    if (c.n_embd % 4) return fail(ZETT_E_INVALID, "n_embd must be a multiple of 4");
    if (c.n_extra < 1) return fail(ZETT_E_INVALID, "n_extra must be >= 1 (reference allocates max(hn_n_extra_tokens,1))");
    if (c.pad_token_id < 0) return fail(ZETT_E_INVALID, "pad_token_id is required");
    if (c.embed_lang && c.n_langs <= 0) return fail(ZETT_E_INVALID, "hn_embed_lang_id needs n_langs");
    return 0;
}

struct WorkspaceSizes {
    int64_t chunk_tokens;
    size_t table, x0, f32_rows, lo_rows, big, stats, parts;
    size_t total() const { return table + x0 + 3 * f32_rows + 3 * lo_rows + big + stats + parts; }
};

static int64_t pair_keys(const zett_config& c, int seq) {
    return ((int64_t)c.original_vocab_size + c.n_extra + 1) * (int64_t)(seq + (c.embed_lang ? 1 : 0));
}

static int64_t chunk_token_cap(const zett_config& c, size_t es) {
    const size_t wide = (size_t)std::max(c.intermediate, 3 * c.hidden);
    const size_t per_token = (size_t)c.n_in_embd * es + 3 * (size_t)c.hidden * 4 + 3 * (size_t)c.hidden * es + wide * es + 24;
    return std::max<int64_t>(131072, (int64_t)(((size_t)12 << 30) / per_token));
}

static WorkspaceSizes workspace_sizes(const zett_config& c, size_t es, int seq, int64_t Ttot, int64_t D, int64_t cap) {
    const int lam = c.embed_lang ? 1 : 0;
    WorkspaceSizes w{};
    if (cap <= 0) cap = chunk_token_cap(c, es);
    w.chunk_tokens = std::max<int64_t>(std::min<int64_t>(cap, std::max<int64_t>(Ttot, D)), seq + lam);
    const size_t MC = (size_t)w.chunk_tokens, MCS = MC + 768;
    const size_t wide = (size_t)std::max(c.intermediate, 3 * c.hidden);
    w.table = (size_t)D * c.hidden * 4;
    w.x0 = MCS * c.n_in_embd * es;
    w.f32_rows = MCS * c.hidden * 4;
    w.lo_rows = MCS * c.hidden * es;
    w.big = MCS * wide * es;
    w.stats = 2 * MCS * 2 * sizeof(float);
    w.parts = c.hidden % 128 == 0 ? (size_t)(c.hidden / 128) * MCS * sizeof(float2) : 0;
    return w;
}

struct PlanLayout {
    PlanArrays p{};
    int32_t* scan_tmp = nullptr;
    bool pair_plan = false;
    int64_t PK = 0;
    size_t n_clear = 0;
    size_t words = 0;
};
static PlanLayout plan_layout(const zett_hypernet* h, const zett_hypernet::PlanSlot* s, int64_t N, int seq, bool worst_case = false) {
    const zett_config& c = h->cfg;
    const int lam = c.embed_lang ? 1 : 0;
    const int64_t V = (int64_t)c.original_vocab_size + c.n_extra;
    const int64_t max_tok = N * (int64_t)(seq + lam);
    PlanLayout L;
    PlanArrays& p = L.p;
    L.PK = pair_keys(c, seq);
    L.pair_plan = worst_case || (h->pair_dedupe && c.layers >= 2 && L.PK <= std::max<int64_t>(4 * max_tok, (int64_t)1 << 23) && L.PK < (int64_t)0x7fffffff);
    int32_t* const base = s ? s->i32.as<int32_t>() : nullptr;
    auto take = [&](int32_t*& array, int64_t n) { array = base ? base + L.words : nullptr; L.words += (size_t)n; };
    take(p.id_flag, V);
    if (L.pair_plan) take(p.pair_flag, L.PK);
    take(p.err, 1);
    L.n_clear = L.words;
    take(p.row_count, N); take(p.row_offset, N + 1); take(p.counters, 3);
    take(p.id_slot, V + 1); take(p.id_list, V);
    take(p.tok_slot, max_tok); take(p.tok_pos, max_tok); take(p.tok_row, max_tok);
    p.n_pair_keys = L.pair_plan ? (int32_t)L.PK : 0;
    if (L.pair_plan) {
        take(p.tok_pkey, max_tok); take(p.tok_pair, max_tok); take(p.pair_tslot, max_tok); take(p.pair_pos, max_tok);
        take(p.pair_slot, L.PK + 1);
    }
    take(L.scan_tmp, 2 * (std::max<int64_t>(std::max<int64_t>(N, V), L.PK) / SCAN_CHUNK + 2) + 1);
    if (s) {
        p.row_uniform = s->u8.as<uint8_t>();
        p.tok_key = p.row_uniform + N;
    }
    return L;
}
static size_t plan_i32_bytes(const zett_hypernet* h, int64_t N, int seq) { return plan_layout(h, nullptr, N, seq, true).words * 4; }

static int enqueue_plan(zett_hypernet* h, zett_hypernet::PlanSlot& s, const int32_t* sfm, int64_t N, int seq, hipStream_t st) {
    const zett_config& c = h->cfg;
    const int lam = c.embed_lang ? 1 : 0;
    const int V = c.original_vocab_size + c.n_extra;
    const int64_t max_tok = N * (int64_t)(seq + lam);
    if (int rc = s.i32.reserve(plan_i32_bytes(h, N, seq))) return rc;
    if (int rc = s.u8.reserve((size_t)N + (size_t)max_tok)) return rc;
    const size_t need_ints = (size_t)N + 1 + 3;
    if (s.host_ints < need_ints) {
        if (s.host) (void)hipHostFree(s.host);
        s.host = nullptr;
        HIP_TRY(hipHostMalloc((void**)&s.host, need_ints * 4, hipHostMallocDefault));
        s.host_ints = need_ints;
    }
    if (!s.done) HIP_TRY(hipEventCreateWithFlags(&s.done, hipEventDisableTiming));
    if (!s.released) HIP_TRY(hipEventCreateWithFlags(&s.released, hipEventDisableTiming));
    const PlanLayout L = plan_layout(h, &s, N, seq);
    const PlanArrays& p = L.p;
    HIP_TRY(hipMemsetAsync(s.i32.p, 0, L.n_clear * 4, st));
    const int rb = (int)((N + 255) / 256);
    hipLaunchKernelGGL(plan_rows_kernel, dim3(rb), dim3(256), 0, st, sfm, N, seq, c.pad_token_id, lam, V, p);
    launch_exclusive_scan(p.row_count, p.row_offset, N, L.scan_tmp, st);
    launch_exclusive_scan(p.id_flag, p.id_slot, (int64_t)V, L.scan_tmp, st);
    {
        PlanArrays pt = p;
        if (h->ext.id_slot) pt.id_slot = const_cast<int32_t*>(h->ext.id_slot);
        hipLaunchKernelGGL(plan_tokens_kernel, dim3(rb), dim3(256), 0, st, sfm, N, seq, c.pad_token_id, lam, V, pt);
    }
    if (L.pair_plan) {
        launch_exclusive_scan(p.pair_flag, p.pair_slot, L.PK, L.scan_tmp, st);
        hipLaunchKernelGGL(plan_pairs_kernel, dim3((unsigned)((max_tok + 255) / 256)), dim3(256), 0, st, N, p);
    }
    hipLaunchKernelGGL(plan_idlist_kernel, dim3((V + 255) / 256), dim3(256), 0, st, V, p);
    HIP_TRY(hipGetLastError());
    HIP_TRY(hipMemcpyAsync(s.host, p.row_offset, ((size_t)N + 1 + 3) * 4, hipMemcpyDeviceToHost, st));
    HIP_TRY(hipEventRecord(s.done, st));
    s.sfm = sfm; s.n_rows = N; s.seq = seq; s.pair_plan = L.pair_plan; s.ext_id_slot = h->ext.id_slot;
    return 0;
}

template <typename T>
int do_forward(zett_hypernet* h, const int32_t* sfm, int64_t N, int seq, const void* src, int src_dtype, const zett_dest* dest,
               int lang_index, float* out_in, float* out_out, float* out_bias, hipStream_t st);
template <typename T>
int do_table_rows(zett_hypernet* h, const int32_t* id_list, int first, int count, const void* src, int src_dtype, void* table_out, float* stats_out, hipStream_t st);

constexpr int CALL_EMPTY = 1;
struct CallCheck {
    int64_t n_rows = 0; int32_t seq = 1;
    bool shape = true;
    bool empty_ok = false;
    bool null_arg = false, null_first = false;
    const char* null_text = "null tensor argument";
    bool encoder = false, need_out_out = false; int32_t lang_index = 0;
    bool source = false; int src_dtype = ZETT_F32; int64_t v_src = 0;
    const char* table_mode = nullptr;
};
int check_call(const zett_hypernet* h, const CallCheck& k) {
    if (!h) return fail(ZETT_E_INVALID, "null handle");
    if (!h->finalized) return fail(ZETT_E_STATE, "zett_finalize has not been called");
    const zett_config& c = h->cfg;
    if (k.null_first && k.null_arg) return fail(ZETT_E_INVALID, "%s", k.null_text);
    if (k.shape && (k.n_rows < (k.empty_ok ? 0 : 1) || k.seq < 1)) return fail(ZETT_E_INVALID, "bad surface-form shape [%lld, %d]", (long long)k.n_rows, k.seq);
    if (k.encoder && k.seq + (c.embed_lang ? 1 : 0) > c.max_positions)
        return fail(ZETT_E_INDEX, "sequence %d exceeds position_embeddings (%d rows)", k.seq, c.max_positions);
    if (k.shape && k.n_rows == 0) return CALL_EMPTY;
    if (k.null_arg) return fail(ZETT_E_INVALID, "%s", k.null_text);
    if (k.need_out_out) return fail(ZETT_E_INVALID, "out_out is required when separate_out_embeddings is set");
    if (k.source) {
        if (!is_dtype(k.src_dtype)) return fail(ZETT_E_INVALID, "unknown source dtype %d", k.src_dtype);
        if (k.v_src < c.original_vocab_size)
            return fail(ZETT_E_INDEX, "source_embeddings has %lld rows, config.original_vocab_size is %d", (long long)k.v_src, c.original_vocab_size);
    }
    if (k.encoder && c.embed_lang && (k.lang_index < 0 || k.lang_index >= c.n_langs)) return fail(ZETT_E_INDEX, "lang_index %d outside [0,%d)", k.lang_index, c.n_langs);
    if (k.shape && k.n_rows * (int64_t)(k.seq + 1) >= (int64_t)0x7fffffff) return fail(ZETT_E_INVALID, "too many positions for one call");
    if (k.table_mode && h->precision == ZETT_PREC_F32) return fail(ZETT_E_INVALID, "%s: the folded 16-bit table exists in the 16-bit modes only", k.table_mode);
    return 0;
}

}

extern "C" {

const char* zett_last_error(void) { return g_err.c_str(); }
int zett_abi_version(void) { return ZETT_ABI_VERSION; }

int zett_create(const zett_config* cfg, int device, int precision, zett_hypernet** out) {
    if (!cfg || !out) return fail(ZETT_E_INVALID, "null argument");
    if (precision != ZETT_PREC_BF16 && precision != ZETT_PREC_F32 && precision != ZETT_PREC_F16) return fail(ZETT_E_INVALID, "unknown precision %d", precision);
    if (int rc = validate_config(*cfg, precision)) return rc;
    int ndev = 0;
    HIP_TRY(hipGetDeviceCount(&ndev));
    if (device < 0 || device >= ndev) return fail(ZETT_E_INVALID, "device %d out of range (%d visible)", device, ndev);
    ZETT_ON_DEVICE(device);
    auto* h = new zett_hypernet();
    h->cfg = *cfg;
    h->device = device;
    h->precision = precision;
    if (hipMalloc((void**)&h->range_word, 64) != hipSuccess || hipHostMalloc((void**)&h->range_host, 64, hipHostMallocDefault) != hipSuccess ||
        hipMemset(h->range_word, 0, 64) != hipSuccess) {
        if (h->range_word) (void)hipFree(h->range_word);
        if (h->range_host) (void)hipHostFree(h->range_host);
        delete h;
        return fail(ZETT_E_HIP, "allocation of the range word failed");
    }
    *out = h;
    return 0;
}

int zett_destroy(zett_hypernet* h) {
    if (!h) return 0;
    ::zett::DeviceScope _scope(h->device);
    for (auto& kv : h->w) {
        if (kv.second.f32) (void)hipFree(kv.second.f32);
        if (kv.second.lo && kv.second.lo != (void*)kv.second.f32) (void)hipFree(kv.second.lo);
    }
    for (void* p : h->owned) (void)hipFree(p);
    for (DevBuf* b : {&h->table, &h->x0, &h->yf, &h->yt, &h->big, &h->pre, &h->ctx, &h->cf, &h->ct, &h->lnstats, &h->lnparts, &h->dest_word, &h->dest_stage[0], &h->dest_stage[1], &h->dest_sink})
        b->release();
    for (zett_hypernet::PlanSlot* psp : {&h->plan[0], &h->plan[1], &h->table_plan}) {
        zett_hypernet::PlanSlot& ps = *psp;
        ps.i32.release(); ps.u8.release();
        if (ps.host) (void)hipHostFree(ps.host);
        if (ps.done) (void)hipEventDestroy(ps.done);
        if (ps.released) (void)hipEventDestroy(ps.released);
    }
    if (h->plan_stream) (void)hipStreamDestroy(h->plan_stream);
    if (h->plan_fork) (void)hipEventDestroy(h->plan_fork);
    if (h->range_word) (void)hipFree(h->range_word);
    if (h->range_host) (void)hipHostFree(h->range_host);
    if (h->dest_host) (void)hipHostFree(h->dest_host);
    if (h->dest_checked) (void)hipEventDestroy(h->dest_checked);
    for (hipEvent_t e : h->out_ready) if (e) (void)hipEventDestroy(e);
    for (hipEvent_t e : h->lane_ev) if (e) (void)hipEventDestroy(e);
    if (h->lane_stream) (void)hipStreamDestroy(h->lane_stream);
    for (hipEvent_t e : h->ev) (void)hipEventDestroy(e);
    delete h;
    return 0;
}

int zett_load_weight(zett_hypernet* h, const char* name, const void* data, int dtype, const int64_t* shape, int ndim) {
    if (!h || !name || !data || !shape || ndim < 1) return fail(ZETT_E_INVALID, "null argument");
    if (h->finalized) return fail(ZETT_E_STATE, "weights are frozen after zett_finalize");
    std::map<std::string, std::vector<int64_t>> exp;
    expected_shapes(h->cfg, exp);
    const std::string n(name);
    auto it = exp.find(n);
    if (it == exp.end()) return 0;
    std::vector<int64_t> got(shape, shape + ndim);
    if (got != it->second) {
        std::string a, b;
        for (auto v : got) a += std::to_string(v) + ",";
        for (auto v : it->second) b += std::to_string(v) + ",";
        return fail(ZETT_E_INVALID, "%s: shape [%s] does not match the config's [%s]", name, a.c_str(), b.c_str());
    }
    ZETT_ON_DEVICE(h->device);
    size_t numel = 1;
    for (auto v : got) numel *= (size_t)v;
    Tensor& t = h->w[n];
    if (t.f32) { (void)hipFree(t.f32); t.f32 = nullptr; }
    t.shape = got;
    t.numel = numel;
    HIP_TRY(hipMalloc((void**)&t.f32, numel * 4));
    if (dtype == ZETT_F32) {
        HIP_TRY(hipMemcpy(t.f32, data, numel * 4, hipMemcpyDefault));
    } else if (dtype == ZETT_F16 || dtype == ZETT_BF16) {
        void* stage = nullptr;
        HIP_TRY(hipMalloc(&stage, numel * 2));
        hipError_t e = hipMemcpy(stage, data, numel * 2, hipMemcpyDefault);
        if (e == hipSuccess) {
            const int blocks = (int)std::min<size_t>((numel + 255) / 256, 65535);
            if (dtype == ZETT_F16) hipLaunchKernelGGL(convert_to_f32_kernel<1>, dim3(blocks), dim3(256), 0, 0, stage, t.f32, numel);
            else hipLaunchKernelGGL(convert_to_f32_kernel<2>, dim3(blocks), dim3(256), 0, 0, stage, t.f32, numel);
            e = hipDeviceSynchronize();
        }
        (void)hipFree(stage);
        if (e != hipSuccess) return fail(ZETT_E_HIP, "upload of %s failed: %s", name, hipGetErrorString(e));
    } else {
        return fail(ZETT_E_INVALID, "unknown dtype %d", dtype);
    }
    return 0;
}

int zett_finalize(zett_hypernet* h) {
    if (!h) return fail(ZETT_E_INVALID, "null handle");
    if (h->finalized) return 0;
    ZETT_ON_DEVICE(h->device);
    std::map<std::string, std::vector<int64_t>> exp;
    expected_shapes(h->cfg, exp);
    for (auto& kv : exp)
        if (!h->w.count(kv.first)) return fail(ZETT_E_STATE, "missing weight: %s", kv.first.c_str());
    const zett_config& c = h->cfg;
    const size_t es = elt_size(h->precision);
    for (auto& kv : h->w) {
        Tensor& t = kv.second;
        if (!is_gemm_weight(kv.first)) continue;
        if (h->precision == ZETT_PREC_F32) { t.lo = t.f32; continue; }
        HIP_TRY(hipMalloc(&t.lo, t.numel * 2));
        const int blocks = (int)std::min<size_t>((t.numel / 4 + 255) / 256 + 1, 65535);
        with_precision(h->precision, [&](auto a) {
            using T = typename decltype(a)::type;
            if constexpr (sizeof(T) == 2)
                hipLaunchKernelGGL(convert_f32_to_lo_kernel<T>, dim3(blocks), dim3(256), 0, 0, t.f32, (T*)t.lo, t.numel, h->range_word);
        });
    }
    HIP_TRY(hipDeviceSynchronize());
    const size_t H = c.hidden;
    for (int l = 0; l < c.layers; ++l) {
        const std::string p = "model.encoder.layer." + std::to_string(l) + ".attention.self.";
        void* wq = nullptr; float* bq = nullptr;
        HIP_TRY(hipMalloc(&wq, 3 * H * H * es));
        HIP_TRY(hipMalloc((void**)&bq, 3 * H * 4));
        h->owned.push_back(wq); h->owned.push_back(bq);
        int k = 0;
        for (const char* q : {"query", "key", "value"}) {
            Tensor& tw = h->w[p + q + ".weight"];
            Tensor& tb = h->w[p + q + ".bias"];
            HIP_TRY(hipMemcpy((char*)wq + (size_t)k * H * H * es, tw.lo, H * H * es, hipMemcpyDeviceToDevice));
            HIP_TRY(hipMemcpy(bq + (size_t)k * H, tb.f32, H * 4, hipMemcpyDeviceToDevice));
            ++k;
        }
        h->qkv_w.push_back(wq);
        h->qkv_b.push_back(bq);
    }
    if (h->precision != ZETT_PREC_F32 && c.hidden % 128 == 0) {
        auto fold = [&](const float* w32, size_t N, size_t K, const float* gamma, const float* beta, const float* bias,
                        zett_hypernet::Folded& f) -> int {
            HIP_TRY(hipMalloc(&f.w, N * K * es));
            HIP_TRY(hipMalloc((void**)&f.c, N * 4));
            HIP_TRY(hipMalloc((void**)&f.b, N * 4));
            h->owned.push_back(f.w); h->owned.push_back(f.c); h->owned.push_back(f.b);
            with_precision(h->precision, [&](auto a) {
                using T = typename decltype(a)::type;
                if constexpr (sizeof(T) == 2)
                    launch_fold_weight<T>(0, w32, (int)N, (int)K, gamma, beta, bias, (T*)f.w, f.c, f.b, h->range_word);
            });
            return 0;
        };
        h->fold_qkv.resize(c.layers); h->fold_up.resize(c.layers);
        float* tmp = nullptr;
        HIP_TRY(hipMalloc((void**)&tmp, 3 * H * H * 4));
        for (int l = 0; l < c.layers; ++l) {
            const std::string lp = "model.encoder.layer." + std::to_string(l) + ".";
            if (int rc = fold(h->w[lp + "intermediate.dense.weight"].f32, c.intermediate, H, h->w[lp + "attention.output.LayerNorm.weight"].f32,
                              h->w[lp + "attention.output.LayerNorm.bias"].f32, h->w[lp + "intermediate.dense.bias"].f32, h->fold_up[l])) return rc;
            if (l == 0) continue;
            const std::string pp = "model.encoder.layer." + std::to_string(l - 1) + ".output.LayerNorm.";
            int k = 0;
            for (const char* q : {"query", "key", "value"}) {
                HIP_TRY(hipMemcpy(tmp + (size_t)k * H * H, h->w[lp + "attention.self." + q + ".weight"].f32, H * H * 4, hipMemcpyDeviceToDevice));
                ++k;
            }
            if (int rc = fold(tmp, 3 * H, H, h->w[pp + "weight"].f32, h->w[pp + "bias"].f32, h->qkv_b[l], h->fold_qkv[l])) return rc;
        }
        if (!(c.single_head && c.separate_out)) {
            const size_t w0 = c.single_head ? c.n_in_embd : c.n_embd;
            if (int rc = fold(h->w["output_projection.1.weight"].f32, w0, H, h->w["output_projection.0.ln.weight"].f32,
                              h->w["output_projection.0.ln.bias"].f32, h->w["output_projection.1.bias"].f32, h->fold_head_in)) return rc;
            if (c.separate_out && !c.single_head)
                if (int rc = fold(h->w["output_projection_out.1.weight"].f32, c.n_embd, H, h->w["output_projection_out.0.ln.weight"].f32,
                                  h->w["output_projection_out.0.ln.bias"].f32, h->w["output_projection_out.1.bias"].f32, h->fold_head_out)) return rc;
            std::vector<float> ones(w0, 1.0f), zeros(w0, 0.0f);
            HIP_TRY(hipMalloc((void**)&h->head_one, w0 * 4));
            HIP_TRY(hipMalloc((void**)&h->head_zero, w0 * 4));
            h->owned.push_back(h->head_one); h->owned.push_back(h->head_zero);
            HIP_TRY(hipMemcpy(h->head_one, ones.data(), w0 * 4, hipMemcpyHostToDevice));
            HIP_TRY(hipMemcpy(h->head_zero, zeros.data(), w0 * 4, hipMemcpyHostToDevice));
        }
        HIP_TRY(hipDeviceSynchronize());
        (void)hipFree(tmp);
    }
    HIP_TRY(hipMemcpy(h->range_host, h->range_word, 4, hipMemcpyDeviceToHost));
    if (h->range_host[0] & ZETT_RANGE_WEIGHT)
        return fail(ZETT_E_RANGE, "a GEMM weight (or a LayerNorm-folded weight W*gamma) exceeds the half range (|w| > 65504 or not finite): "
                                  "this checkpoint needs ZETT_PREC_BF16 or ZETT_PREC_F32");
    if (c.rescale) {
        const size_t w0 = c.single_head ? c.n_in_embd : c.n_embd;
        HIP_TRY(hipMalloc((void**)&h->head_scale, w0 * 4));
        HIP_TRY(hipMalloc((void**)&h->head_shift, w0 * 4));
        h->owned.push_back(h->head_scale); h->owned.push_back(h->head_shift);
        HIP_TRY(hipMemcpy(h->head_scale, h->w["scaler.w"].f32, c.n_embd * 4, hipMemcpyDeviceToDevice));
        HIP_TRY(hipMemcpy(h->head_shift, h->w["scaler.b"].f32, c.n_embd * 4, hipMemcpyDeviceToDevice));
        if (c.single_head && c.separate_out) {
            HIP_TRY(hipMemcpy(h->head_scale + c.n_embd, h->w["out_scaler.w"].f32, c.n_embd * 4, hipMemcpyDeviceToDevice));
            HIP_TRY(hipMemcpy(h->head_shift + c.n_embd, h->w["out_scaler.b"].f32, c.n_embd * 4, hipMemcpyDeviceToDevice));
        }
    }
    if (h->precision != ZETT_PREC_F32) {
        for (auto& kv : h->w) {
            Tensor& t = kv.second;
            if (is_gemm_weight(kv.first) && t.f32) { (void)hipFree(t.f32); t.f32 = nullptr; }
        }
    }
    h->finalized = true;
    return 0;
}

int zett_set_option(zett_hypernet* h, const char* key, int64_t value) {
    if (!h || !key) return fail(ZETT_E_INVALID, "null argument");
    const std::string k(key);
    if (k == "max_chunk_tokens") {
        if (value < 1024) return fail(ZETT_E_INVALID, "max_chunk_tokens must be >= 1024");
        h->max_chunk_tokens = value;
    } else if (k == "time_gemm") {
        h->time_gemm = value != 0;
    } else if (k == "cls_only_last_layer") {
        h->cls_only_last = value != 0;
    } else if (k == "pair_dedupe") {
        h->pair_dedupe = value != 0;
    } else if (k == "residual_lo") {
        if (value < 0 || value > 2) return fail(ZETT_E_INVALID, "residual_lo must be 0 (fp32 residual stream), 1 (16-bit stream in f16 mode) or 2 (in bf16 mode too)");
        h->residual_lo = (int)value;
    } else if (k == "concurrent_lanes") {
        if (value < 0 || value > 2) return fail(ZETT_E_INVALID, "concurrent_lanes must be 0 (never), 1 (auto) or 2 (whenever a call is one chunk of >= 512 rows)");
        h->concurrent_lanes = (int)value;
    } else if (k == "attention_fast") {
        h->attention_fast = value != 0;
    } else if (k == "ln_fold") {
        if (value < 0 || value > 2) return fail(ZETT_E_INVALID, "ln_fold must be 0 (off), 1 (encoder and output heads) or 2 (encoder only: A/B)");
        h->ln_fold = (int)value;
    } else if (k == "gemm_tail_split") {
        if (value < 0 || value > 3) return fail(ZETT_E_INVALID, "gemm_tail_split must be 0 (never), 1 (auto), 2 (cut every gemm4d launch in the middle) or 3 (128x256 tiles only)");
        h->gemm_tail_split = (int)value;
    } else if (k == "attention_pack") {
        h->attention_pack = value != 0;
    } else if (k == "ln_rows8") {
        h->ln_rows8 = value != 0;
    } else if (k == "table_lo") {
        h->table_lo = value != 0;
    } else if (k == "gemm_group") {
        if (value < 0 || value > 64) return fail(ZETT_E_INVALID, "gemm_group must be 0 (default: 4) .. 64");
        h->gemm_group = (int)value;
    } else if (k == "gemm_tile_order") {
        if (value < 0 || value > 1) return fail(ZETT_E_INVALID, "gemm_tile_order must be 0 or 1");
        h->gemm_tile_order = (int)value;
    } else if (k == "gemm4d_min_k") {
        if (value < 64) return fail(ZETT_E_INVALID, "gemm4d_min_k must be >= 64");
        h->gemm4d_min_k = (int)value;
    } else if (k == "range_accumulate") {
        h->range_accumulate = value != 0;
    } else if (k == "gemm_variant") {
        if (value != 0 && value != 1 && value != 2 && value != 3 && value != 7 && value != 8)
            return fail(ZETT_E_INVALID, "gemm_variant must be 0 (auto), 1 (128x128), 2 (256x256 register-staged), 3 (384x256), 7 (256x256 four-wave direct-to-LDS) or 8 (7 with the generic epilogue drain)");
        h->gemm_variant = (int)value;
    } else {
        return fail(ZETT_E_INVALID, "unknown option %s", key);
    }
    return 0;
}

int zett_workspace_bytes(const zett_hypernet* h, int64_t n_rows, int32_t seq, int64_t* out_bytes) {
    if (!h || !out_bytes) return fail(ZETT_E_INVALID, "null argument");
    if (n_rows < 0 || seq < 1) return fail(ZETT_E_INVALID, "bad surface-form shape [%lld, %d]", (long long)n_rows, seq);
    const zett_config& c = h->cfg;
    const int64_t V = (int64_t)c.original_vocab_size + c.n_extra;
    const int64_t max_tok = n_rows * (int64_t)(seq + (c.embed_lang ? 1 : 0));
    const WorkspaceSizes w = workspace_sizes(c, elt_size(h->precision), seq, max_tok, std::min<int64_t>(V, max_tok), h->max_chunk_tokens);
    *out_bytes = (int64_t)(w.total() + plan_i32_bytes(h, n_rows, seq) + (size_t)n_rows + (size_t)max_tok);
    return 0;
}

int zett_get_stats(const zett_hypernet* h, zett_stats* out) {
    if (!h || !out) return fail(ZETT_E_INVALID, "null argument");
    *out = h->stats;
    return 0;
}

int zett_stream_wait_output(zett_hypernet* h, int which, void* stream) {
    if (!h) return fail(ZETT_E_INVALID, "null handle");
    if (which != ZETT_OUT_IN && which != ZETT_OUT_BIAS) return fail(ZETT_E_INVALID, "which must be ZETT_OUT_IN or ZETT_OUT_BIAS");
    if (!h->out_recorded) return fail(ZETT_E_STATE, "no forward has run on this handle");
    ZETT_ON_DEVICE(h->device);
    HIP_TRY(hipStreamWaitEvent((hipStream_t)stream, h->out_ready[which], 0));
    return 0;
}

int zett_get_gemm_log(const zett_hypernet* h, zett_gemm_record* out, int64_t capacity, int64_t* count) {
    if (!h || !count || capacity < 0 || (capacity > 0 && !out)) return fail(ZETT_E_INVALID, "null argument");
    *count = (int64_t)h->gemm_log.size();
    for (int64_t i = 0; i < capacity && i < *count; ++i) out[i] = h->gemm_log[(size_t)i];
    return 0;
}

int zett_check_range(zett_hypernet* h, void* stream, int32_t* flags) {
    if (!h) return fail(ZETT_E_INVALID, "null handle");
    ZETT_ON_DEVICE(h->device);
    hipStream_t st = (hipStream_t)stream;
    HIP_TRY(hipMemcpyAsync(h->range_host, h->range_word, 4, hipMemcpyDeviceToHost, st));
    HIP_TRY(hipStreamSynchronize(st));
    const int32_t w = h->range_host[0];
    if (h->range_accumulate && w) HIP_TRY(hipMemsetAsync(h->range_word, 0, 4, st));
    if (flags) *flags = w;
    if (!w) return 0;
    return fail(ZETT_E_RANGE, "the last forward left the range of its arithmetic:%s%s%s%s (precision %s)",
                (w & ZETT_RANGE_SOURCE) ? " in_scaler(source_embeddings) beyond the half range;" : "",
                (w & ZETT_RANGE_ACTIVATION) ? " a 16-bit activation (Q/K/V, FFN intermediate or the operand copy of the residual sum) beyond the half range;" : "",
                (w & ZETT_RANGE_OUTPUT) ? " non-finite predicted embeddings;" : "",
                (w & ZETT_RANGE_DEST) ? " a finite value beyond the range of an f16 destination (stored as inf);" : "",
                h->precision == ZETT_PREC_F16 ? "f16: re-run with ZETT_PREC_BF16" : h->precision == ZETT_PREC_BF16 ? "bf16" : "f32");
}

int zett_partition_workspace_bytes(int64_t n_rows, int32_t n_ids, int64_t* out_bytes) {
    if (!out_bytes || n_rows < 0 || n_ids < 1) return fail(ZETT_E_INVALID, "bad argument");
    *out_bytes = (int64_t)partition_workspace_bytes(n_rows, n_ids);
    return 0;
}

int zett_partition_rows(const int32_t* surface_forms, int64_t n_rows, int32_t seq, int32_t pad_id, int32_t n_ids, int32_t world,
                        const int32_t* caps, int32_t* perm_out, void* workspace, int64_t workspace_bytes, int32_t device, void* stream) {
    if (n_rows < 0 || seq < 1 || n_ids < 1) return fail(ZETT_E_INVALID, "bad surface-form shape [%lld, %d] / id range %d", (long long)n_rows, seq, n_ids);
    if (world < 1 || world > PART_MAX_RANKS) return fail(ZETT_E_INVALID, "zett_partition_rows handles 1..%d ranks (one node), got %d", PART_MAX_RANKS, world);
    if (n_rows == 0) return 0;
    if (!surface_forms || !caps || !perm_out || !workspace) return fail(ZETT_E_INVALID, "null argument");
    if (n_rows >= (int64_t)0x7fffffff) return fail(ZETT_E_INVALID, "too many rows for one call");
    int64_t total = 0;
    for (int r = 0; r < world; ++r) { if (caps[r] < 0) return fail(ZETT_E_INVALID, "negative capacity"); total += caps[r]; }
    if (total != n_rows) return fail(ZETT_E_INVALID, "the ranks' capacities sum to %lld, the matrix has %lld rows", (long long)total, (long long)n_rows);
    if ((size_t)workspace_bytes < partition_workspace_bytes(n_rows, n_ids)) return fail(ZETT_E_INVALID, "workspace too small (zett_partition_workspace_bytes)");
    ZETT_ON_DEVICE(device);
    hipStream_t st = (hipStream_t)stream;
    const size_t have_bytes = ((size_t)(n_ids + 3) / 4) * 4 + 64;
    uint32_t* have = (uint32_t*)workspace;
    PartCaps caps_arg = {};
    for (int r = 0; r < world; ++r) caps_arg.v[r] = caps[r];
    HIP_TRY(hipMemsetAsync(have, 0, have_bytes, st));
    const size_t lds_have = ((size_t)(n_ids + 3) / 4) * 4;
    if (lds_have <= 150 * 1024) {
        static bool attr_set[64] = {};
        if (device >= 64 || !attr_set[device]) {
            HIP_TRY(hipFuncSetAttribute((const void*)partition_rows_kernel<true>, hipFuncAttributeMaxDynamicSharedMemorySize, 150 * 1024));
            if (device < 64) attr_set[device] = true;
        }
        hipLaunchKernelGGL(partition_rows_kernel<true>, dim3(1), dim3(PART_THREADS), lds_have, st, surface_forms, n_rows, (int)seq, (int)pad_id, (int)n_ids,
                           (int)world, caps_arg, have, perm_out);
    } else {
        hipLaunchKernelGGL(partition_rows_kernel<false>, dim3(1), dim3(PART_THREADS), 0, st, surface_forms, n_rows, (int)seq, (int)pad_id, (int)n_ids,
                           (int)world, caps_arg, have, perm_out);
    }
    HIP_TRY(hipGetLastError());
    return 0;
}

int zett_scatter_rows(const void* src, void* dst, const int64_t* order, int64_t n_rows, int64_t row_bytes, int32_t device, void* stream) {
    if (n_rows < 0 || row_bytes < 1) return fail(ZETT_E_INVALID, "bad shape");
    if (n_rows == 0) return 0;
    if (!src || !dst || !order) return fail(ZETT_E_INVALID, "null argument");
    if (row_bytes != 4 && row_bytes % 16 != 0) return fail(ZETT_E_INVALID, "row_bytes must be 4 or a multiple of 16, got %lld", (long long)row_bytes);
    if (((uintptr_t)src | (uintptr_t)dst) % (row_bytes == 4 ? 4 : 16)) return fail(ZETT_E_INVALID, "misaligned buffer");
    ZETT_ON_DEVICE(device);
    hipStream_t st = (hipStream_t)stream;
    if (row_bytes == 4)
        hipLaunchKernelGGL(scatter_words_kernel, dim3((unsigned)((n_rows + 255) / 256)), dim3(256), 0, st, (const uint32_t*)src, (uint32_t*)dst, order, n_rows);
    else
        hipLaunchKernelGGL(scatter_rows_kernel, dim3((unsigned)std::min<int64_t>(n_rows, 65535 * 16)), dim3(256), 0, st, (const unsigned char*)src, (unsigned char*)dst,
                           order, n_rows, row_bytes);
    HIP_TRY(hipGetLastError());
    return 0;
}

int zett_forward_prepare(zett_hypernet* h, const int32_t* surface_forms, int64_t n_rows, int32_t seq, void* input_stream) {
    CallCheck k;
    k.n_rows = n_rows; k.seq = seq; k.empty_ok = true; k.null_arg = !surface_forms;
    if (int rc = check_call(h, k)) return rc == CALL_EMPTY ? 0 : rc;
    ZETT_ON_DEVICE(h->device);
    if (!h->plan_stream) {
        int least = 0, greatest = 0;
        HIP_TRY(hipDeviceGetStreamPriorityRange(&least, &greatest));
        HIP_TRY(hipStreamCreateWithPriority(&h->plan_stream, hipStreamNonBlocking, greatest));
    }
    if (!h->plan_fork) HIP_TRY(hipEventCreateWithFlags(&h->plan_fork, hipEventDisableTiming));
    zett_hypernet::PlanSlot& ps = h->plan[h->plan_cur ^ 1];
    if (ps.pending) HIP_TRY(hipEventSynchronize(ps.done));
    HIP_TRY(hipEventRecord(h->plan_fork, (hipStream_t)input_stream));
    HIP_TRY(hipStreamWaitEvent(h->plan_stream, h->plan_fork, 0));
    if (ps.released) HIP_TRY(hipStreamWaitEvent(h->plan_stream, ps.released, 0));
    if (int rc = enqueue_plan(h, ps, surface_forms, n_rows, seq, h->plan_stream)) return rc;
    ps.pending = true;
    return 0;
}

}

namespace {

int check_dest(const zett_hypernet* h, const zett_dest* d, int64_t n_rows) {
    const zett_config& c = h->cfg;
    if (!d) return fail(ZETT_E_INVALID, "null destination");
    if (!d->in) return fail(ZETT_E_INVALID, "the destination's `in` matrix is null");
    if (c.separate_out != (d->out != nullptr))
        return fail(ZETT_E_INVALID, c.separate_out ? "the destination's `out` matrix is required when separate_out_embeddings is set"
                                                   : "the destination's `out` must be null: this config has no second output");
    if (d->dtype < ZETT_F32 || d->dtype > ZETT_BF16) return fail(ZETT_E_INVALID, "unknown destination dtype %d", d->dtype);
    if (d->bias && (d->bias_dtype < ZETT_F32 || d->bias_dtype > ZETT_BF16)) return fail(ZETT_E_INVALID, "unknown bias destination dtype %d", d->bias_dtype);
    if (d->ld_in < c.n_embd || (d->out && d->ld_out < c.n_embd))
        return fail(ZETT_E_INVALID, "destination leading dimension (%lld, %lld) below n_embd %d", (long long)d->ld_in, (long long)d->ld_out, c.n_embd);
    if (d->n_dest_rows < 0 || (!d->rows && d->n_dest_rows < n_rows))
        return fail(ZETT_E_INVALID, "the destination has %lld rows, the identity map needs %lld", (long long)d->n_dest_rows, (long long)n_rows);
    return 0;
}

int forward_entry(zett_hypernet* h, const int32_t* surface_forms, int64_t n_rows, int32_t seq, const void* source_embeddings, int src_dtype,
                  int64_t v_src, int32_t lang_index, const zett_dest* dest, float* out_in, float* out_out, float* out_bias, void* stream) {
    CallCheck k;
    k.n_rows = n_rows; k.seq = seq; k.empty_ok = true; k.encoder = true; k.lang_index = lang_index;
    k.null_arg = !surface_forms || !source_embeddings || (!dest && (!out_in || !out_bias));
    k.need_out_out = h && !dest && h->cfg.separate_out && !out_out;
    k.source = true; k.src_dtype = src_dtype; k.v_src = v_src;
    const int checked = check_call(h, k);
    if (checked != 0 && checked != CALL_EMPTY) return checked;
    ZETT_ON_DEVICE(h->device);
    hipStream_t st = (hipStream_t)stream;
    if (checked == CALL_EMPTY) {
        h->stats = zett_stats{};
        if (!h->range_accumulate) HIP_TRY(hipMemsetAsync(h->range_word, 0, 4, st));
        for (hipEvent_t& e : h->out_ready) {
            if (!e) HIP_TRY(hipEventCreateWithFlags(&e, hipEventDisableTiming));
            HIP_TRY(hipEventRecord(e, st));
// ... 264 lines not shown
        check("ln_stats");
    }

    void projector(const std::string& p, const T* x_lo, const float* x_f32, int rows, T* big, float* pre, float* of, T* ol,
                   float2* fold_parts = nullptr, int ld_part = 0, float* fold_stats = nullptr) {
        const zett_config& c = h->cfg;
        GemmEpilogue<T> e1 = epi();
        e1.bias = Wf(p + "dense1.bias"); e1.act = ACT_GELU_TANH; e1.out_lo = big; e1.ld_lo = c.intermediate;
        gemm(x_lo, c.hidden, Wlo(p + "dense1.weight"), c.hidden, rows, c.intermediate, c.hidden, e1);
        GemmEpilogue<T> e2 = epi();
        e2.bias = Wf(p + "dense2.bias"); e2.act = ACT_GELU_TANH; e2.residual = x_f32; e2.ld_res = c.hidden;
        e2.ld_f32 = c.hidden;
        if (fold_parts) { e2.out_lo = ol; e2.ld_lo = c.hidden; e2.stats_part = fold_parts; e2.ld_part = ld_part; }
        else e2.out_f32 = pre;
        gemm(big, c.intermediate, Wlo(p + "dense2.weight"), c.intermediate, rows, c.hidden, c.intermediate, e2);
        if (fold_parts) ln_stats(fold_parts, ld_part, rows, c.ln_eps_projector, fold_stats);
        else layernorm(pre, rows, Wf(p + "ln.weight"), Wf(p + "ln.bias"), c.ln_eps_projector, of, ol);
    }
};

struct ForwardMode { bool fold, lo_stream, table_lo, fold_heads; };
template <typename T>
ForwardMode forward_mode(const zett_hypernet* h) {
    const zett_config& c = h->cfg;
    ForwardMode m{};
    m.fold = h->ln_fold && !std::is_same<T, float>::value && h->gemm_variant == 0 && c.hidden % 128 == 0 && c.hidden >= 512 && (int)h->fold_up.size() == c.layers;
    m.lo_stream = m.fold && c.layers >= 1 && sizeof(T) == 2 && (h->residual_lo == 2 || (h->residual_lo == 1 && std::is_same<T, f16_t>::value));
    m.table_lo = m.lo_stream && h->table_lo != 0;
    m.fold_heads = m.fold && h->ln_fold == 1 && h->fold_head_in.w != nullptr;
    return m;
}
int needs_folded_table(const char* entry) {
    return fail(ZETT_E_INVALID, "%s needs the folded 16-bit table: f16 arithmetic with the LayerNorm fold, the 16-bit residual stream and table_lo on", entry);
}

int reserve_workspace(zett_hypernet* h, const WorkspaceSizes& ws, bool fold, bool encoder) {
    const struct { DevBuf* buf; size_t bytes; bool encoder_only; } list[] = {
        {&h->table, ws.table, true}, {&h->x0, ws.x0, false}, {&h->yf, ws.f32_rows, false}, {&h->yt, ws.lo_rows, false}, {&h->big, ws.big, false},
        {&h->pre, ws.f32_rows, false}, {&h->ctx, ws.lo_rows, true}, {&h->cf, ws.f32_rows, true}, {&h->ct, ws.lo_rows, true},
        {&h->lnstats, ws.stats, true}, {&h->lnparts, fold ? ws.parts : 0, false}};
    for (const auto& r : list)
        if (encoder || !r.encoder_only)
            if (int rc = r.buf->reserve(r.bytes)) return rc;
    return 0;
}

template <typename T>
struct Workspace {
    T* X0; float* Zf; T* Zt; T* BIG; float* PRE; T* CTX; float* Cf; T* Ct; float* STa; float* STb; float2* PARTS;
    int ld_parts;
    long a_rows;
};
template <typename U> U* buf_at(const DevBuf& b, size_t n) { return b.p ? (U*)b.p + n : nullptr; }
template <typename T>
Workspace<T> lane_workspace(const zett_hypernet* h, size_t off, size_t MCS) {
    const size_t H = h->cfg.hidden, wide = (size_t)std::max(h->cfg.intermediate, 3 * h->cfg.hidden);
    Workspace<T> w{};
    w.X0 = buf_at<T>(h->x0, 0);
    w.Zf = buf_at<float>(h->yf, off * H); w.Zt = buf_at<T>(h->yt, off * H);
    w.BIG = buf_at<T>(h->big, off * wide); w.PRE = buf_at<float>(h->pre, off * H);
    w.CTX = buf_at<T>(h->ctx, off * H); w.Cf = buf_at<float>(h->cf, off * H); w.Ct = buf_at<T>(h->ct, off * H);
    w.STa = buf_at<float>(h->lnstats, 2 * off); w.STb = buf_at<float>(h->lnstats, 2 * off + 2 * MCS);
    w.PARTS = buf_at<float2>(h->lnparts, off);
    w.ld_parts = (int)MCS;
    w.a_rows = (long)(MCS - off);
    return w;
}

template <typename T>
void table_phase(Runner<T>& R, const Workspace<T>& w, const int32_t* id_list, int first, int count, const void* src, int src_dtype, int64_t MC,
                 bool table_lo, T* tbl16, float* tblst, float* tbl32) {
    zett_hypernet* h = R.h;
    const zett_config& c = h->cfg;
    const int H = c.hidden, EIN = c.n_in_embd;
    const float* in_w = c.rescale ? R.Wf("in_scaler.w") : nullptr;
    const float* in_b = c.rescale ? R.Wf("in_scaler.b") : nullptr;
    for (int s0 = first; s0 < first + count && !R.rc; s0 += (int)MC) {
        const int m = (int)std::min<int64_t>(MC, first + count - s0);
        const float* fb = R.Wf("fallback_embeddings.weight");
        with_dtype(src_dtype, [&](auto sd) {
            launch_gather_src<T, decltype(sd)::value>(R.st, id_list, s0, m, src, c.n_in_embd, c.original_vocab_size, fb, in_w, in_b, w.X0, h->range_word);
        });
        R.check("gather_src");
        GemmEpilogue<T> e0 = R.epi();
        e0.bias = R.Wf("input_projection.0.bias"); e0.out_f32 = w.Zf; e0.ld_f32 = H; e0.out_lo = w.Zt; e0.ld_lo = H;
        R.gemm(w.X0, EIN, R.Wlo("input_projection.0.weight"), EIN, m, H, EIN, e0);
        if (table_lo) R.projector("input_projection.1.", w.Zt, w.Zf, m, w.BIG, w.PRE, nullptr, tbl16 + (size_t)s0 * H, w.PARTS, w.ld_parts, tblst + 2 * (size_t)s0);
        else R.projector("input_projection.1.", w.Zt, w.Zf, m, w.BIG, w.PRE, tbl32 + (size_t)s0 * H, nullptr);
    }
}

template <typename T>
int do_table_rows(zett_hypernet* h, const int32_t* id_list, int first, int count, const void* src, int src_dtype, void* table_out, float* stats_out, hipStream_t st) {
    const ForwardMode mode = forward_mode<T>(h);
    if (!mode.table_lo) return needs_folded_table("zett_table_rows");
    const WorkspaceSizes ws = workspace_sizes(h->cfg, sizeof(T), 1, count, count, h->max_chunk_tokens);
    const size_t MCS = (size_t)ws.chunk_tokens + 768;
    if (int rc = reserve_workspace(h, ws, mode.fold, false)) return rc;
    Runner<T> R{h, st};
    R.a_rows_readable = (long)MCS;
    struct NoTiming { zett_hypernet* h; int saved; ~NoTiming() { h->time_gemm = saved; } } no_timing{h, h->time_gemm};
    h->time_gemm = 0;
    table_phase<T>(R, lane_workspace<T>(h, 0, MCS), id_list, first, count, src, src_dtype, ws.chunk_tokens, true, (T*)table_out, stats_out, nullptr);
    return R.rc;
}

struct SlotGuard {
    zett_hypernet* h; zett_hypernet::PlanSlot* ps; hipStream_t st; bool lane_forked = false;
    ~SlotGuard() {
        if (lane_forked && h->lane_stream && h->lane_ev[3]) {
            (void)hipEventRecord(h->lane_ev[3], h->lane_stream);
            (void)hipStreamWaitEvent(st, h->lane_ev[3], 0);
        }
        if (ps->released) (void)hipEventRecord(ps->released, st);
    }
};

int read_gemm_timing(zett_hypernet* h, hipStream_t st) {
    HIP_TRY(hipStreamSynchronize(st));
    const bool print = getenv("ZETT_GEMM_LOG") != nullptr;
    double ms = 0.0, fl = 0.0;
    for (size_t k = 0; 2 * k + 1 < h->ev_used && k < h->gemm_log.size(); ++k) {
        zett_gemm_record& r = h->gemm_log[k];
        float t = 0.f;
        if (hipEventElapsedTime(&t, h->ev[2 * k], h->ev[2 * k + 1]) == hipSuccess) { ms += t; fl += r.flops; r.ms = t; }
        if (print)
            fprintf(stderr, "[zett gemm] M=%6d N=%6d K=%5d tile=%s %8.3f ms %7.1f TF\n", r.m, r.n, r.k,
                    r.variant == 7 ? "4d " : r.variant == 8 ? "4dg" : r.variant == 3 ? "384" : r.variant == 2 ? "8r " : "128", t, r.flops / (t * 1e9));
    }
    h->stats.gemm_ms = ms;
    h->stats.gemm_flops_timed = fl;
    return 0;
}

template <typename T>
struct Forward {
    using DestOut = typename Runner<T>::DestOut;
    zett_hypernet* h; const int32_t* sfm; int64_t N; int seq; const void* src; int src_dtype; const zett_dest* dest; int lang_index;
    float* out_in; float* out_out; float* out_bias; hipStream_t st;
    Runner<T> R{h, st};
    const zett_config& c = h->cfg;
    const int H = c.hidden, I = c.intermediate, E = c.n_embd;
    const ForwardMode mode = forward_mode<T>(h);
    zett_hypernet::PlanSlot* ps = nullptr;
    PlanArrays p{};
    bool pair_plan = false;
    const int32_t* hoff = nullptr;
    int64_t Ttot = 0;
    int D = 0;
    int64_t MC = 0; size_t MCS = 0;
    float* TBL = nullptr; T* TBL16 = nullptr; float* TBLST = nullptr;
    const float* lang_vec = nullptr;
    const float scaling = 1.0f / std::sqrt((float)(H / c.heads));

    int run() {
        h->stats = zett_stats{};
        h->stats.rows = N;
        h->ev_used = 0;
        h->gemm_log.clear();
        if (int rc = take_plan()) return rc;
        SlotGuard guard{h, ps, st};
        if (int rc = read_plan()) return rc;
        if (int rc = reserve()) return rc;
        if (!h->ext.table)
            table_phase<T>(R, lane_workspace<T>(h, 0, MCS), p.id_list, 0, D, src, src_dtype, MC, mode.table_lo, TBL16, TBLST, TBL);
        if (R.rc) return R.rc;
        if (int rc = run_chunks(guard)) return rc;
        h->out_recorded = true;
        return h->time_gemm ? read_gemm_timing(h, st) : 0;
    }

    int take_plan() {
        zett_hypernet::PlanSlot& s = h->plan[h->plan_cur ^ 1];
        if (s.pending && s.sfm == sfm && s.n_rows == N && s.seq == seq && s.pair_plan == plan_layout(h, &s, N, seq).pair_plan &&
            s.ext_id_slot == h->ext.id_slot) {
            HIP_TRY(hipStreamWaitEvent(st, s.done, 0));
        } else {
            if (s.pending) HIP_TRY(hipEventSynchronize(s.done));
            if (s.released) HIP_TRY(hipStreamWaitEvent(st, s.released, 0));
            if (int rc = enqueue_plan(h, s, sfm, N, seq, st)) return rc;
        }
        s.pending = false;
        h->plan_cur ^= 1;
        ps = &s;
        return 0;
    }

    int read_plan() {
        const PlanLayout PL = plan_layout(h, ps, N, seq);
        p = PL.p;
        pair_plan = PL.pair_plan;
        if (!h->range_accumulate) HIP_TRY(hipMemsetAsync(h->range_word, 0, 4, st));
        for (hipEvent_t& e : h->out_ready)
            if (!e) HIP_TRY(hipEventCreateWithFlags(&e, hipEventDisableTiming));
        const bool dest_check = dest && dest->rows;
        if (dest_check) {
            if (int rc = h->dest_word.reserve(4)) return rc;
            if (!h->dest_host) HIP_TRY(hipHostMalloc((void**)&h->dest_host, 4, hipHostMallocDefault));
            if (!h->dest_checked) HIP_TRY(hipEventCreateWithFlags(&h->dest_checked, hipEventDisableTiming));
            HIP_TRY(hipMemsetAsync(h->dest_word.p, 0, 4, st));
            hipLaunchKernelGGL(dest_rows_check_kernel, dim3((unsigned)((N + 255) / 256)), dim3(256), 0, st, dest->rows, N, dest->n_dest_rows, h->dest_word.as<int32_t>());
            HIP_TRY(hipGetLastError());
            HIP_TRY(hipMemcpyAsync(h->dest_host, h->dest_word.p, 4, hipMemcpyDeviceToHost, st));
            HIP_TRY(hipEventRecord(h->dest_checked, st));
        }
        HIP_TRY(hipEventSynchronize(ps->done));
        hoff = ps->host;
        if (hoff[N + 2] != 0)
            return fail(ZETT_E_INDEX, "surface-form row %d holds an id outside [0, %d) (original_vocab_size %d + %d fallback rows)",
                        hoff[N + 2] - 1, c.original_vocab_size + c.n_extra, c.original_vocab_size, c.n_extra);
        if (dest_check) {
            HIP_TRY(hipEventSynchronize(h->dest_checked));
            if (h->dest_host[0] != 0)
                return fail(ZETT_E_INDEX, "destination row map: rows[%d] is outside the destination's %lld rows", h->dest_host[0] - 1, (long long)dest->n_dest_rows);
        }
        Ttot = hoff[N];
        D = hoff[N + 1];
        h->stats.packed_tokens = Ttot;
        h->stats.distinct_ids = D;
        h->stats.distinct_positions = Ttot;
        return 0;
    }

    int reserve() {
        const WorkspaceSizes ws = workspace_sizes(c, sizeof(T), seq, Ttot, D, h->max_chunk_tokens);
        MC = ws.chunk_tokens;
        MCS = (size_t)MC + 768;
        if (int rc = reserve_workspace(h, ws, mode.fold, true)) return rc;
        R.a_rows_readable = (long)MCS;
        const bool ext_table = h->ext.table != nullptr;
        if (ext_table && !mode.table_lo) return needs_folded_table("zett_forward_table");
        TBL = h->table.as<float>();
        TBL16 = ext_table ? (T*)const_cast<void*>(h->ext.table) : (T*)h->table.as<float>();
        TBLST = ext_table ? const_cast<float*>(h->ext.stats) : (float*)((char*)h->table.as<float>() + (((size_t)D * H * sizeof(T) + 15) / 16) * 16);
        lang_vec = c.embed_lang ? R.Wf("lang_embeddings.weight") + (size_t)lang_index * H : nullptr;
        return 0;
    }

    struct Chunk {
        int64_t r0; int rows, tok0, m; hipStream_t st; int ev_mode; Workspace<T> w;
        float* hs_sum; float* hs_stats; const float* hs_gamma; const float* hs_beta;
        int zrows;
        bool raw = false;
        bool pairs = false;
        int P = 0;
        float* other(float* b) const { return b == w.Zf ? w.PRE : w.Zf; }
        float* other_stats(float* b) const { return b == w.STa ? w.STb : w.STa; }
    };

    int run_chunk(int64_t r0, int64_t r1, hipStream_t lane_st, size_t off, int ev_mode) {
        Chunk k{r0, (int)(r1 - r0), hoff[r0], hoff[r1] - hoff[r0], lane_st, ev_mode, lane_workspace<T>(h, off, MCS)};
        h->stats.chunks += 1;
        R.st = lane_st;
        R.stage_lane = ev_mode == 2 ? 1 : 0;
        R.a_rows_readable = k.w.a_rows;
        embeddings(k);
        for (int l = 0; l < c.layers && !R.rc; ++l) {
            const std::string lp = "model.encoder.layer." + std::to_string(l) + ".";
            attention(k, l);
            feed_forward(k, l, lp);
        }
        if (R.rc) return R.rc;
        if (int rc = readout(k)) return rc;
        return heads(k);
    }

    void embeddings(Chunk& k) {
        LnEmbed emb{TBL, p.tok_slot, p.tok_pos, R.Wf("model.embeddings.token_type_embeddings.weight"),
                    R.Wf("model.embeddings.position_embeddings.weight"), lang_vec, seq, p.tok_row, p.row_offset, k.r0, k.rows,
                    mode.table_lo ? (const void*)TBL16 : nullptr, TBLST, R.Wf("input_projection.1.ln.weight"), R.Wf("input_projection.1.ln.bias")};
        k.hs_sum = k.w.Zf;
        k.hs_stats = k.w.STb;
        k.hs_gamma = R.Wf("model.embeddings.LayerNorm.weight");
        k.hs_beta = R.Wf("model.embeddings.LayerNorm.bias");
        k.zrows = k.m;
        k.P = pair_plan ? hoff[N + 3] : 0;
        k.pairs = pair_plan && k.rows == N && k.P > 0 && (int64_t)k.P * 100 <= (int64_t)k.m * 85;
        float* sum = mode.lo_stream ? (float*)nullptr : k.hs_sum;
        if (k.pairs) {
            emb.tok_slot = p.pair_tslot; emb.tok_pos = p.pair_pos; emb.tok_row = nullptr;
            R.layernorm(nullptr, k.P, k.hs_gamma, k.hs_beta, c.ln_eps_encoder, nullptr, k.w.Zt, k.hs_stats, LnReadout{}, -1, &emb, 0, sum);
            hipLaunchKernelGGL(pair_rows_kernel, dim3((k.m + 255) / 256), dim3(256), 0, k.st, k.m, k.tok0, k.r0, k.rows, p, p.tok_pkey);
            R.check("pair_rows");
            h->stats.distinct_positions = k.P;
        } else {
            R.layernorm(nullptr, k.m, k.hs_gamma, k.hs_beta, c.ln_eps_encoder, nullptr, k.w.Zt, k.hs_stats, LnReadout{}, -1, &emb, k.tok0, sum);
        }
    }

    void attention(Chunk& k, int l) {
        const Workspace<T>& w = k.w;
        const bool cls_only = h->cls_only_last && l == c.layers - 1;
        const T* wqkv = k.raw ? (const T*)h->fold_qkv[l].w : (const T*)h->qkv_w[l];
        const float* bqkv = k.raw ? h->fold_qkv[l].b : h->qkv_b[l];
        const float* cqkv = k.raw ? h->fold_qkv[l].c : nullptr;
        auto qkv = [&](int col0, int cols, int M, T* out) {
            GemmEpilogue<T> e = R.epi();
            e.bias = bqkv + col0; e.out_lo = out; e.ld_lo = cols;
            if (k.raw) { e.fold_stats = k.hs_stats; e.fold_c = cqkv + col0; }
            R.gemm(w.Zt, H, wqkv + (size_t)col0 * H, H, M, cols, H, e);
        };
        const bool by_pair = !cls_only && k.pairs && l == 0;
        const T* Q = w.BIG;
        const T* KV = w.BIG + H;
        size_t ld_q = (size_t)3 * H, ld_kv = (size_t)3 * H;
        if (!cls_only) {
            qkv(0, 3 * H, by_pair ? k.P : k.m, w.BIG);
        } else {
            qkv(H, 2 * H, k.m, w.BIG);
            qkv(0, H, k.rows, w.BIG + (size_t)k.m * 2 * H);
            KV = w.BIG; Q = w.BIG + (size_t)k.m * 2 * H;
            ld_q = (size_t)H; ld_kv = (size_t)2 * H;
            k.zrows = k.rows;
        }
        launch_attention<T>(k.st, H, h->attention_fast, h->attention_pack, Q, ld_q, KV, KV + H, ld_kv, H / c.heads, p.row_offset, p.row_uniform, p.tok_key,
                            k.r0, k.rows, k.tok0, scaling, cls_only ? 1 : 0, by_pair ? (const int32_t*)p.tok_pair : (const int32_t*)nullptr, w.CTX);
        R.check(cls_only ? "attention(position 0)" : "attention");
    }

    void feed_forward(Chunk& k, int l, const std::string& lp) {
        const Workspace<T>& w = k.w;
        const bool last = l == c.layers - 1, fold = mode.fold, lo_stream = mode.lo_stream;
        const int zrows = k.zrows;
        float* s1 = k.other(k.hs_sum);
        float* st1 = k.other_stats(k.hs_stats);
        GemmEpilogue<T> eo = R.epi();
        eo.bias = R.Wf(lp + "attention.output.dense.bias");
        if (k.pairs && l == 0) eo.res_index = p.tok_pkey;
        if (lo_stream) {
            eo.residual_lo = w.Zt; eo.ld_res_lo = H;
            if (k.raw) { eo.res_stats = k.hs_stats; eo.res_gamma = k.hs_gamma; eo.res_beta = k.hs_beta; }
            eo.out_lo = w.Ct; eo.ld_lo = H; eo.stats_part = w.PARTS; eo.ld_part = w.ld_parts;
        } else {
            eo.residual = k.hs_sum; eo.ld_res = H;
            eo.res_stats = k.hs_stats; eo.res_gamma = k.hs_gamma; eo.res_beta = k.hs_beta;
            eo.out_f32 = s1; eo.ld_f32 = H;
            if (fold) { eo.out_lo = w.Zt; eo.ld_lo = H; eo.stats_part = w.PARTS; eo.ld_part = w.ld_parts; }
        }
        R.gemm(w.CTX, H, R.Wlo(lp + "attention.output.dense.weight"), H, zrows, H, H, eo);
        const float* g1 = R.Wf(lp + "attention.output.LayerNorm.weight");
        const float* b1 = R.Wf(lp + "attention.output.LayerNorm.bias");
        const T* mid = lo_stream ? w.Ct : w.Zt;
        GemmEpilogue<T> ei = R.epi();
        ei.act = ACT_GELU_ERF; ei.out_lo = w.BIG; ei.ld_lo = I;
        if (fold) {
            R.ln_stats(w.PARTS, w.ld_parts, zrows, c.ln_eps_encoder, st1);
            ei.bias = h->fold_up[l].b; ei.fold_stats = st1; ei.fold_c = h->fold_up[l].c;
            R.gemm(mid, H, (const T*)h->fold_up[l].w, H, zrows, I, H, ei);
        } else {
            R.layernorm(s1, zrows, g1, b1, c.ln_eps_encoder, nullptr, w.Zt, st1);
            ei.bias = R.Wf(lp + "intermediate.dense.bias");
            R.gemm(w.Zt, H, R.Wlo(lp + "intermediate.dense.weight"), H, zrows, I, H, ei);
        }
        float* s2 = k.other(s1);
        float* st2 = k.other_stats(st1);
        GemmEpilogue<T> ef = R.epi();
        ef.bias = R.Wf(lp + "output.dense.bias");
        if (lo_stream) {
            ef.residual_lo = w.Ct; ef.ld_res_lo = H; ef.res_stats = st1; ef.res_gamma = g1; ef.res_beta = b1;
            ef.out_lo = w.Zt; ef.ld_lo = H; ef.stats_part = w.PARTS; ef.ld_part = w.ld_parts;
        } else {
            ef.residual = s1; ef.ld_res = H;
            ef.res_stats = st1; ef.res_gamma = g1; ef.res_beta = b1;
            ef.out_f32 = s2; ef.ld_f32 = H;
            if (fold && !last) { ef.out_lo = w.Zt; ef.ld_lo = H; ef.stats_part = w.PARTS; ef.ld_part = w.ld_parts; }
        }
        R.gemm(w.BIG, I, R.Wlo(lp + "output.dense.weight"), I, zrows, H, I, ef);
        k.hs_gamma = R.Wf(lp + "output.LayerNorm.weight");
        k.hs_beta = R.Wf(lp + "output.LayerNorm.bias");
        k.hs_sum = s2; k.hs_stats = st2;
        if (!last) {
            if (fold) { R.ln_stats(w.PARTS, w.ld_parts, zrows, c.ln_eps_encoder, st2); k.raw = true; }
            else R.layernorm(s2, zrows, k.hs_gamma, k.hs_beta, c.ln_eps_encoder, nullptr, w.Zt, st2);
        }
    }

    int output_ready(const Chunk& k, int which, hipEvent_t lane_ev) {
        if (k.ev_mode == 2) HIP_TRY(hipEventRecord(lane_ev, k.st));
        if (k.ev_mode == 3) HIP_TRY(hipStreamWaitEvent(k.st, lane_ev, 0));
        if (k.ev_mode == 1 || k.ev_mode == 3) HIP_TRY(hipEventRecord(h->out_ready[which], k.st));
        return 0;
    }

    int readout(Chunk& k) {
        LnReadout ro{c.predict_bias ? R.Wf("bias_projection.weight") : (const float*)nullptr,
                     c.predict_bias ? R.Wf("bias_projection.bias") : (const float*)nullptr, out_bias ? out_bias + k.r0 : nullptr};
        int bias_dtype = -1;
        if (dest && dest->bias) {
            const size_t bes = dest->bias_dtype == ZETT_F32 ? 4 : 2;
            ro.bias_rows = dest->rows ? dest->rows + k.r0 : nullptr;
            ro.out_bias = (float*)((char*)dest->bias + (dest->rows ? 0 : (size_t)k.r0 * bes));
            bias_dtype = dest->bias_dtype;
        } else if (dest) {
            if (int rc = h->dest_sink.reserve((size_t)N * sizeof(float))) return rc;
            ro.out_bias = h->dest_sink.as<float>() + k.r0;
        }
        ro.range_flag = h->range_word;
        ro.in_lo = mode.lo_stream ? (const T*)k.w.Zt : (const T*)nullptr;
        R.layernorm(k.hs_sum, k.rows, k.hs_gamma, k.hs_beta, c.ln_eps_encoder, k.w.Cf, k.w.Ct, nullptr, ro, bias_dtype);
        return R.rc ? 0 : output_ready(k, ZETT_OUT_BIAS, h->lane_ev[1]);
    }

    DestOut dest_out(void* base, int64_t ld, int64_t r0) const {
        const size_t es = dest->dtype == ZETT_F32 ? 4 : 2;
        return DestOut{dest->rows ? base : (void*)((char*)base + (size_t)r0 * (size_t)ld * es), dest->rows ? dest->rows + r0 : nullptr, ld, dest->dtype};
    }

    void head(const Chunk& k, const std::string& name, const zett_hypernet::Folded& f, const float* scale, const float* shift, bool split,
              float* out, float* out_b, void* dst, int64_t ld_dst, void* dst_b, int64_t ld_dst_b) {
        const Workspace<T>& w = k.w;
        const bool fold = mode.fold_heads;
        if (fold) R.projector(name + ".0.", w.Ct, w.Cf, k.rows, w.BIG, w.PRE, nullptr, w.CTX, w.PARTS, w.ld_parts, w.STa);
        else R.projector(name + ".0.", w.Ct, w.Cf, k.rows, w.BIG, w.PRE, nullptr, w.CTX);
        GemmEpilogue<T> e = R.epi();
        e.bias = fold ? f.b : R.Wf(name + ".1.bias");
        e.scale = c.rescale ? scale : (fold ? h->head_one : nullptr);
        e.shift = c.rescale ? shift : (fold ? h->head_zero : nullptr);
        if (fold) { e.fold_stats = w.STa; e.fold_c = f.c; }
        e.ld_f32 = E; e.range_final = 1;
        if (split) e.split_col = E;
        const int width = split ? 2 * E : E;
        const T* wl = fold ? (const T*)f.w : R.Wlo(name + ".1.weight");
        if (dest) {
            const DestOut d = dest_out(dst, ld_dst, k.r0), d_b = split ? dest_out(dst_b, ld_dst_b, k.r0) : DestOut{};
            R.head_gemm(w.CTX, wl, k.rows, width, H, e, &d, split ? &d_b : nullptr, E);
        } else {
            e.out_f32 = out + (size_t)k.r0 * E;
            if (split) e.out_f32_b = out_b + (size_t)k.r0 * E;
            R.gemm(w.CTX, H, wl, H, k.rows, width, H, e);
        }
    }

    int heads(const Chunk& k) {
        const bool split = c.single_head && c.separate_out;
        head(k, "output_projection", h->fold_head_in, h->head_scale, h->head_shift, split, out_in, out_out,
             dest ? dest->in : nullptr, dest ? dest->ld_in : 0, dest ? dest->out : nullptr, dest ? dest->ld_out : 0);
        if (!R.rc)
            if (int rc = output_ready(k, ZETT_OUT_IN, h->lane_ev[2])) return rc;
        if (c.separate_out && !c.single_head)
            head(k, "output_projection_out", h->fold_head_out, c.rescale ? R.Wf("out_scaler.w") : nullptr, c.rescale ? R.Wf("out_scaler.b") : nullptr, false,
                 out_out, nullptr, dest ? dest->out : nullptr, dest ? dest->ld_out : 0, nullptr, 0);
        return R.rc;
    }

    bool two_lanes() const {
        if (!h->concurrent_lanes || Ttot > MC || N < 512) return false;
        const int Pn = pair_plan ? hoff[N + 3] : 0;
        const bool pairs_taken = pair_plan && Pn > 0 && (int64_t)Pn * 100 <= Ttot * 85;
        const double r = (double)((Ttot + 255) / 256) * (double)((H + 255) / 256) / 256.0;
        return h->concurrent_lanes == 2 || (!pairs_taken && !h->time_gemm && H >= 1024 && r < 4.0 && (std::ceil(r) - r) / std::ceil(r) > 0.08);
    }

    int run_chunks(SlotGuard& guard) {
        if (two_lanes()) {
            if (!h->lane_stream) HIP_TRY(hipStreamCreateWithFlags(&h->lane_stream, hipStreamNonBlocking));
            for (hipEvent_t& e : h->lane_ev)
                if (!e) HIP_TRY(hipEventCreateWithFlags(&e, hipEventDisableTiming));
            int64_t ra = ((N / 2 + 128) / 256) * 256;
            ra = std::min<int64_t>(std::max<int64_t>(ra, 256), N - 1);
            const size_t off1 = (size_t)(hoff[ra] - hoff[0]) + 384;
            HIP_TRY(hipEventRecord(h->lane_ev[0], st));
            HIP_TRY(hipStreamWaitEvent(h->lane_stream, h->lane_ev[0], 0));
            guard.lane_forked = true;
            if (int rc = run_chunk(ra, N, h->lane_stream, off1, 2)) return rc;
            if (int rc = run_chunk(0, ra, st, 0, 3)) return rc;
        } else {
            int64_t r0 = 0;
            while (r0 < N) {
                int64_t r1 = r0 + 1;
                while (r1 < N && (int64_t)hoff[r1 + 1] - hoff[r0] <= MC) ++r1;
                if (int rc = run_chunk(r0, r1, st, 0, r1 == N ? 1 : 0)) return rc;
                r0 = r1;
            }
        }
        R.st = st;
        if (R.rc) return R.rc;
        if (guard.lane_forked) {
            HIP_TRY(hipEventRecord(h->lane_ev[3], h->lane_stream));
            HIP_TRY(hipStreamWaitEvent(st, h->lane_ev[3], 0));
            guard.lane_forked = false;
        }
        return 0;
    }
};

template <typename T>
int do_forward(zett_hypernet* h, const int32_t* sfm, int64_t N, int seq, const void* src, int src_dtype, const zett_dest* dest,
               int lang_index, float* out_in, float* out_out, float* out_bias, hipStream_t st) {
    Forward<T> f{h, sfm, N, seq, src, src_dtype, dest, lang_index, out_in, out_out, out_bias, st};
    return f.run();
}

}
```

### zett_amd/hypernet.py

```python
from __future__ import annotations

import ctypes as C
import json
import os
from typing import Dict, Optional, Tuple

import torch
from torch import nn
from transformers import PreTrainedModel

from . import _glue, _lib
from ._glue import ptr, zett_dtypes
from .config import ZettHypernetConfig
from .dims import PROJECTOR_LN_EPS, ROBERTA_LN_EPS, ROBERTA_MAX_POSITIONS, HypernetDims, weight_shapes

DEFAULT_PRECISION = "f16"
_PRECISIONS = {"bf16": _lib.PREC_BF16, "bfloat16": _lib.PREC_BF16, "f32": _lib.PREC_F32,
               "fp32": _lib.PREC_F32, "float32": _lib.PREC_F32, "f16": _lib.PREC_F16, "fp16": _lib.PREC_F16,
               "float16": _lib.PREC_F16}


def _backbone_settings(name_or_path: str) -> Tuple[int, float]:
    path = os.path.join(str(name_or_path), "config.json")
    if os.path.isfile(path):
        with open(path) as f:
            d = json.load(f)
        return int(d.get("max_position_embeddings", ROBERTA_MAX_POSITIONS)), float(d.get("layer_norm_eps", ROBERTA_LN_EPS))
    return ROBERTA_MAX_POSITIONS, ROBERTA_LN_EPS


class _Node(nn.Module):
    """Plain container: gives parameters the dotted names of the reference modules."""


def _attach(root: nn.Module, dotted: str, param: nn.Parameter) -> None:
    *path, leaf = dotted.split(".")
    node = root
    for part in path:
        child = node._modules.get(part)
        if child is None:
            child = _Node()
            node.add_module(part, child)
        node = child
    node.register_parameter(leaf, param)


class HipEngine:

    def __init__(self, dims: HypernetDims, ln_eps_encoder: float, device: torch.device, precision: str):
        if device.type != "cuda":
            raise RuntimeError("zett_amd computes on MI355X only: tensors must live on a cuda (ROCm) device")
        self.lib = _lib.load()
        self.dims = dims
        self.device = device
        self.precision = precision
        cfg = _lib.ZettConfig(
            n_embd=dims.n_embd, n_in_embd=dims.n_in_embd, hidden=dims.hidden, intermediate=dims.intermediate,
            heads=dims.heads, layers=dims.layers, n_extra=dims.n_extra, original_vocab_size=dims.original_vocab_size,
            pad_token_id=dims.pad_token_id, separate_out=int(dims.separate_out), single_head=int(dims.single_head),
            rescale=int(dims.rescale), predict_bias=int(dims.predict_bias), embed_lang=int(dims.embed_lang),
            n_langs=dims.n_langs, max_positions=dims.max_positions, ln_eps_encoder=ln_eps_encoder,
            ln_eps_projector=PROJECTOR_LN_EPS)
        handle = C.c_void_p()
        index = device.index if device.index is not None else torch.cuda.current_device()
        _lib.check(self.lib.zett_create(C.byref(cfg), index, _PRECISIONS[precision], C.byref(handle)), "zett_create")
        self.handle = handle
        self.weights_stamp = None

    def load_weights(self, tensors: Dict[str, torch.Tensor]) -> None:
        for name, t in tensors.items():
            t = t.detach()
            if t.dtype not in zett_dtypes():
                t = t.float()
            t = t.contiguous()
            shape = (C.c_int64 * t.dim())(*t.shape)
            _lib.check(self.lib.zett_load_weight(self.handle, name.encode(), ptr(t), zett_dtypes()[t.dtype], shape, t.dim()), f"zett_load_weight({name})")
        _lib.check(self.lib.zett_finalize(self.handle), "zett_finalize")

    def set_option(self, key: str, value: int) -> None:
        _lib.check(self.lib.zett_set_option(self.handle, key.encode(), int(value)), f"zett_set_option({key})")

    def workspace_bytes(self, n_rows: int, seq: int) -> int:
        out = C.c_int64(0)
        _lib.check(self.lib.zett_workspace_bytes(self.handle, int(n_rows), int(seq), C.byref(out)), "zett_workspace_bytes")
        return out.value

    def range_flags(self) -> int:
        flags = C.c_int32(0)
        with torch.cuda.device(self.device):
            rc = self.lib.zett_check_range(self.handle, _glue.stream(self.device), C.byref(flags))
        if rc not in (_lib.ZETT_OK, _lib.E_RANGE):
            _lib.check(rc, "zett_check_range")
        return int(flags.value)

    def stream_wait_output(self, which: str, stream: "torch.cuda.Stream") -> None:
        code = {"in": _lib.OUT_IN, "bias": _lib.OUT_BIAS}[which]
        _lib.check(self.lib.zett_stream_wait_output(self.handle, code, _glue.stream(of=stream)), "zett_stream_wait_output")

    def gemm_log(self) -> list:
        n = C.c_int64(0)
        _lib.check(self.lib.zett_get_gemm_log(self.handle, None, 0, C.byref(n)), "zett_get_gemm_log")
        buf = (_lib.ZettGemmRecord * max(1, n.value))()
        _lib.check(self.lib.zett_get_gemm_log(self.handle, buf, n.value, C.byref(n)), "zett_get_gemm_log")
        return [{f: getattr(buf[i], f) for f, _ in _lib.ZettGemmRecord._fields_} for i in range(n.value)]

    def stats(self) -> dict:
        s = _lib.ZettStats()
        _lib.check(self.lib.zett_get_stats(self.handle, C.byref(s)))
        return {n: getattr(s, n) for n, _ in s._fields_}

    def prepare(self, surface_forms: torch.Tensor, input_stream: Optional["torch.cuda.Stream"] = None) -> None:
        if surface_forms.dtype != torch.int32 or not surface_forms.is_contiguous() or surface_forms.device != self.device or surface_forms.dim() != 2:
            raise ValueError("prepare() takes the int32, contiguous [n_tokens, surface_maxlen] tensor on the engine's device that forward() will get")
        n, seq = surface_forms.shape
        with torch.cuda.device(self.device):
            _lib.check(self.lib.zett_forward_prepare(self.handle, ptr(surface_forms), n, seq, _glue.stream(self.device, of=input_stream)),
                       "zett_forward_prepare")
        self._prepared = surface_forms

    def forward(self, surface_forms: torch.Tensor, source_embeddings: torch.Tensor, lang_index: int):
        d = self.dims
        if surface_forms.dim() != 2:
            raise ValueError("target_surface_forms must be [n_tokens, surface_maxlen]")
        if surface_forms.device != self.device or source_embeddings.device != self.device:
            raise RuntimeError(f"all tensors must be on {self.device}")
        ids = surface_forms.to(torch.int32).contiguous()
        src = source_embeddings
        if src.dtype not in zett_dtypes():
            src = src.float()
        src = src.contiguous()
        if src.dim() != 2 or src.shape[1] != d.n_in_embd:
            raise ValueError(f"source_embeddings must be [V, {d.n_in_embd}], got {tuple(src.shape)}")
        n, seq = ids.shape
        out_in = torch.empty((n, d.n_embd), dtype=torch.float32, device=self.device)
        out_out = torch.empty((n, d.n_embd), dtype=torch.float32, device=self.device) if d.separate_out else None
        out_bias = torch.empty((n,), dtype=torch.float32, device=self.device)
        with torch.cuda.device(self.device):
            rc = self.lib.zett_forward(self.handle, ptr(ids), n, seq, ptr(src), zett_dtypes()[src.dtype], src.shape[0], int(lang_index),
                                       ptr(out_in), ptr(out_out), ptr(out_bias), _glue.stream(self.device))
        self._prepared = None
        _lib.check(rc, "zett_forward")
        return out_in, out_out, out_bias

    def _dest(self, n: int, out_in: torch.Tensor, out_out: Optional[torch.Tensor], out_bias: Optional[torch.Tensor], rows):
        d = self.dims

        def matrix(t, what):
            if not torch.is_tensor(t) or t.dim() != 2:
                raise ValueError(f"{what} must be a 2-d tensor")
            if t.device != self.device:
                raise ValueError(f"{what} must live on {self.device}, got {t.device}")
            if t.dtype not in zett_dtypes():
                raise ValueError(f"{what}: dtype {t.dtype} is not one of float32 / float16 / bfloat16")
            if t.shape[1] != d.n_embd or t.stride(1) != 1:
                raise ValueError(f"{what} must be [rows, {d.n_embd}] with unit column stride, got shape {tuple(t.shape)} strides {t.stride()}")
            return t

        out_in = matrix(out_in, "out_in")
        if d.separate_out:
            if out_out is None:
                raise ValueError("out_out is required: this hypernetwork predicts separate output embeddings")
            out_out = matrix(out_out, "out_out")
            if out_out.dtype != out_in.dtype or out_out.shape[0] != out_in.shape[0]:
                raise ValueError("out_out must have out_in's dtype and number of rows")
        elif out_out is not None:
            raise ValueError("out_out must be None: this hypernetwork has no separate output embeddings")
        if out_bias is not None:
            if not torch.is_tensor(out_bias) or out_bias.dim() != 1 or out_bias.device != self.device or out_bias.dtype not in zett_dtypes():
                raise ValueError(f"out_bias must be a 1-d float32 / float16 / bfloat16 tensor on {self.device}")
            if out_bias.stride(0) != 1 or out_bias.shape[0] != out_in.shape[0]:
                raise ValueError("out_bias must be contiguous with one entry per row of out_in")
        keep = [out_in, out_out, out_bias]
        if rows is not None:
            if not torch.is_tensor(rows) or rows.dtype != torch.int64 or rows.device != self.device or rows.dim() != 1 or rows.shape[0] != n:
                raise ValueError(f"rows must be an int64 tensor of {n} entries on {self.device}")
            rows = rows.contiguous()
            keep.append(rows)
        st = _lib.ZettDest(in_=out_in.data_ptr(), out=out_out.data_ptr() if out_out is not None else None,
                           bias=out_bias.data_ptr() if out_bias is not None else None, dtype=zett_dtypes()[out_in.dtype],
                           bias_dtype=zett_dtypes()[out_bias.dtype] if out_bias is not None else 0, ld_in=out_in.stride(0),
                           ld_out=out_out.stride(0) if out_out is not None else 0, rows=rows.data_ptr() if rows is not None else None,
                           n_dest_rows=out_in.shape[0])
        return st, keep

    def forward_into(self, surface_forms: torch.Tensor, source_embeddings: torch.Tensor, lang_index: int, out_in: torch.Tensor,
                     out_out: Optional[torch.Tensor] = None, out_bias: Optional[torch.Tensor] = None, rows: Optional[torch.Tensor] = None) -> None:
        d = self.dims
        if surface_forms.dim() != 2:
            raise ValueError("target_surface_forms must be [n_tokens, surface_maxlen]")
        if surface_forms.device != self.device or source_embeddings.device != self.device:
            raise RuntimeError(f"all tensors must be on {self.device}")
        ids = surface_forms.to(torch.int32).contiguous()
        src = source_embeddings
        if src.dtype not in zett_dtypes():
            src = src.float()
        src = src.contiguous()
        if src.dim() != 2 or src.shape[1] != d.n_in_embd:
            raise ValueError(f"source_embeddings must be [V, {d.n_in_embd}], got {tuple(src.shape)}")
        n, seq = ids.shape
        dest, keep = self._dest(n, out_in, out_out, out_bias, rows)
        with torch.cuda.device(self.device):
            rc = self.lib.zett_forward_into(self.handle, ptr(ids), n, seq, ptr(src), zett_dtypes()[src.dtype],
                                            src.shape[0], int(lang_index), C.byref(dest), _glue.stream(self.device))
        self._prepared = None
        _lib.check(rc, "zett_forward_into")
        del keep

    def forward_table_into(self, surface_forms: torch.Tensor, table: torch.Tensor, stats: torch.Tensor, id_slot: torch.Tensor, lang_index: int,
                           out_in: torch.Tensor, out_out: Optional[torch.Tensor] = None, out_bias: Optional[torch.Tensor] = None,
                           rows: Optional[torch.Tensor] = None) -> None:
        if surface_forms.dim() != 2 or surface_forms.device != self.device:
            raise ValueError(f"target_surface_forms must be [n_tokens, surface_maxlen] on {self.device}")
        ids = surface_forms.to(torch.int32).contiguous()
        n, seq = ids.shape
        dest, keep = self._dest(n, out_in, out_out, out_bias, rows)
        with torch.cuda.device(self.device):
            rc = self.lib.zett_forward_table_into(self.handle, ptr(ids), n, seq, ptr(table), ptr(stats),
                                                  ptr(id_slot), int(lang_index), C.byref(dest), _glue.stream(self.device))
        self._prepared = None
        _lib.check(rc, "zett_forward_table_into")
        del keep

    def table_plan(self, surface_forms_all: torch.Tensor):
        ids = surface_forms_all.to(torch.int32).contiguous()
        if ids.dim() != 2 or ids.device != self.device:
            raise ValueError(f"table_plan takes the [n_tokens, surface_maxlen] matrix on {self.device}")
        v = self.dims.original_vocab_size + self.dims.n_extra
        id_slot = torch.empty((v + 1,), dtype=torch.int32, device=self.device)
        id_list = torch.empty((v,), dtype=torch.int32, device=self.device)
        n_ids = C.c_int64(0)
        with torch.cuda.device(self.device):
            _lib.check(self.lib.zett_table_plan(self.handle, ptr(ids), ids.shape[0], ids.shape[1], ptr(id_slot),
                                                ptr(id_list), C.byref(n_ids), _glue.stream(self.device)), "zett_table_plan")
        return id_slot, id_list[:n_ids.value], int(n_ids.value)

    def table_buffers(self, n_rows: int):
        lo = {"f16": torch.float16, "fp16": torch.float16, "float16": torch.float16, "bf16": torch.bfloat16}.get(self.precision)
        if lo is None:
            raise ValueError("the folded 16-bit table exists in the 16-bit modes only")
        return (torch.empty((n_rows, self.dims.hidden), dtype=lo, device=self.device), torch.empty((n_rows, 2), dtype=torch.float32, device=self.device))

    def table_rows(self, id_list: torch.Tensor, first: int, count: int, source_embeddings: torch.Tensor, table: torch.Tensor, stats: torch.Tensor) -> None:
        src = source_embeddings
        if src.dtype not in zett_dtypes():
            src = src.float()
        src = src.contiguous()
        if src.dim() != 2 or src.shape[1] != self.dims.n_in_embd or src.device != self.device:
            raise ValueError(f"source_embeddings must be [V, {self.dims.n_in_embd}] on {self.device}, got {tuple(src.shape)}")
        if not (table.is_contiguous() and stats.is_contiguous() and table.shape[0] >= first + count and stats.shape[0] >= first + count and id_list.numel() >= first + count):
            raise ValueError("table / stats / id_list are smaller than the requested rows")
        with torch.cuda.device(self.device):
            _lib.check(self.lib.zett_table_rows(self.handle, ptr(id_list), first, count, ptr(src), zett_dtypes()[src.dtype],
                                                src.shape[0], ptr(table), ptr(stats), _glue.stream(self.device)), "zett_table_rows")

    def forward_table(self, surface_forms: torch.Tensor, table: torch.Tensor, stats: torch.Tensor, id_slot: torch.Tensor, lang_index: int):
        d = self.dims
        if surface_forms.dim() != 2 or surface_forms.device != self.device:
            raise ValueError(f"target_surface_forms must be [n_tokens, surface_maxlen] on {self.device}")
        ids = surface_forms.to(torch.int32).contiguous()
        n, seq = ids.shape
        out_in = torch.empty((n, d.n_embd), dtype=torch.float32, device=self.device)
        out_out = torch.empty((n, d.n_embd), dtype=torch.float32, device=self.device) if d.separate_out else None
# ... 245 lines not shown
```

Measured before the change: 624,500.

## Reorder single-token rows first and skip their Q/K projections and attention

Rows whose surface form is a single token are permuted to the front of the CLS slots via a host-built map. The Q and K projections then skip those rows, since softmax over one key is identity and the context equals V. Attention copies V directly for them, and outputs are scattered through a composed row map. This adds a host pass over the row offsets, a pinned-memory copy, an event sync per call and scatter-style output writes.

```diff
diff --git a/include/zett_hip.h b/include/zett_hip.h
--- a/include/zett_hip.h
+++ b/include/zett_hip.h
@@ -99,6 +99,8 @@
 int zett_forward_prepare(zett_hypernet* h, const int32_t* surface_forms, int64_t n_rows, int32_t seq, void* input_stream);
 
 int zett_get_stats(const zett_hypernet* h, zett_stats* out);
+
+int zett_single_rows(const zett_hypernet* h, int64_t* out);
 
 typedef struct zett_gemm_record {
     int32_t m, n, k;
diff --git a/zett_amd/_lib.py b/zett_amd/_lib.py
--- a/zett_amd/_lib.py
+++ b/zett_amd/_lib.py
@@ -60,6 +60,7 @@
     "zett_sampled_vocab_patch_rows",
     "zett_op_embed_lookup_plan_base", "zett_op_gather_bwd_rows_f32",
     "zett_op_fwd_layernorm", "zett_op_fwd_embed_layernorm", "zett_op_fwd_attention", "zett_op_fwd_gather_src", "zett_op_fwd_ln_stats", "zett_op_fwd_fold_weight",
+    "zett_single_rows",
 )
 
 
@@ -138,6 +139,7 @@
         lib.zett_forward.argtypes = [C.c_void_p, C.c_void_p, C.c_int64, C.c_int32, C.c_void_p, C.c_int, C.c_int64,
                                      C.c_int32, C.c_void_p, C.c_void_p, C.c_void_p, C.c_void_p]
         lib.zett_get_stats.argtypes = [C.c_void_p, C.POINTER(ZettStats)]
+        lib.zett_single_rows.argtypes = [C.c_void_p, C.POINTER(C.c_int64)]
         lib.zett_workspace_bytes.argtypes = [C.c_void_p, C.c_int64, C.c_int32, C.POINTER(C.c_int64)]
         lib.zett_set_option.argtypes = [C.c_void_p, C.c_char_p, C.c_int64]
         lib.zett_check_range.argtypes = [C.c_void_p, C.c_void_p, C.POINTER(C.c_int32)]
diff --git a/zett_amd/csrc/rowops.hip.h b/zett_amd/csrc/rowops.hip.h
--- a/zett_amd/csrc/rowops.hip.h
+++ b/zett_amd/csrc/rowops.hip.h
@@ -157,12 +157,13 @@
     p.pair_pos[ps] = p.tok_pos[t];
 }
 
-__device__ __forceinline__ int chunk_row(int t_rel, int row_rel, bool first, int rows);
-static __global__ void pair_rows_kernel(int m, int tok0, int64_t row0, int rows, PlanArrays p, int32_t* __restrict__ brow_pair) {
+__device__ __forceinline__ int chunk_row(int t_rel, int row_rel, bool first, int rows, const int32_t* cls_slot);
+static __global__ void pair_rows_kernel(int m, int tok0, int64_t row0, int rows, PlanArrays p, int32_t* __restrict__ brow_pair,
+                                        const int32_t* __restrict__ cls_slot) {
     const int t = blockIdx.x * blockDim.x + threadIdx.x;
     if (t >= m) return;
     const int n = p.tok_row[tok0 + t];
-    brow_pair[chunk_row(t, (int)(n - row0), p.row_offset[n] == tok0 + t, rows)] = p.tok_pair[tok0 + t];
+    brow_pair[chunk_row(t, (int)(n - row0), p.row_offset[n] == tok0 + t, rows, cls_slot)] = p.tok_pair[tok0 + t];
 }
 
 static __global__ void plan_idlist_kernel(int n_ids, PlanArrays p) {
@@ -264,10 +265,11 @@
     const float* table_stats;
     const float* table_gamma;
     const float* table_beta;
+    const int32_t* cls_slot;
 };
 
-__device__ __forceinline__ int chunk_row(int t_rel, int row_rel, bool first, int rows) {
-    return first ? row_rel : rows + t_rel - row_rel - 1;
+__device__ __forceinline__ int chunk_row(int t_rel, int row_rel, bool first, int rows, const int32_t* cls_slot) {
+    return first ? (cls_slot ? cls_slot[row_rel] : row_rel) : rows + t_rel - row_rel - 1;
 }
 
 struct LnReadout {
@@ -323,7 +325,7 @@
         posr = emb.pos_emb + (size_t)emb.tok_pos[tok0 + r] * H;
         if (emb.tok_row) {
             const int n = emb.tok_row[tok0 + r];
-            ro = chunk_row(r, (int)(n - emb.row0), emb.row_offset[n] == tok0 + r, emb.rows);
+            ro = chunk_row(r, (int)(n - emb.row0), emb.row_offset[n] == tok0 + r, emb.rows, emb.cls_slot);
         }
     } else {
         x = in + (size_t)r * ld_in;
@@ -484,7 +486,7 @@
         posr = emb.pos_emb + (size_t)emb.tok_pos[tok0 + r] * H;
         if (emb.tok_row) {
             const int n = emb.tok_row[tok0 + r];
-            ro = chunk_row(r, (int)(n - emb.row0), emb.row_offset[n] == tok0 + r, emb.rows);
+            ro = chunk_row(r, (int)(n - emb.row0), emb.row_offset[n] == tok0 + r, emb.rows, emb.cls_slot);
         }
     } else {
         x = in + (size_t)r * ld_in;
@@ -629,8 +631,9 @@
                                                              const int32_t* __restrict__ row_offset,
                                                              const uint8_t* __restrict__ row_uniform,
                                                              const uint8_t* __restrict__ tok_key, int64_t row0,
-                                                             int rows, int tok0, float scaling, int flags ,
-                                                             const int32_t* __restrict__ tok_pair, T* __restrict__ ctx) {
+                                                             int rows, int tok0, float scaling,
+                                                             int flags ,
+                                                             const int32_t* __restrict__ tok_pair, T* __restrict__ ctx, const int32_t* __restrict__ cls_slot) {
     const int cls_only = flags & 1;
     const int lane = threadIdx.x & 63;
     const int64_t w = (int64_t)blockIdx.x * 4 + (threadIdx.x >> 6);
@@ -657,7 +660,8 @@
     const bool uniform = row_uniform[n];
     const int nq = cls_only ? 1 : (t1 - t0);
     const int ccol = active ? col : 0;
-    auto brow = [&](int t) -> size_t { return (size_t)chunk_row(t, rl, t == t0, rows); };
+    const int slot0 = chunk_row(t0, rl, true, rows, cls_slot), rest = chunk_row(0, rl, false, rows, nullptr);
+    auto brow = [&](int t) -> size_t { return (size_t)(t == t0 ? slot0 : rest + t); };
     int pslot = 0;
     if (tok_pair) { const int t = t0 + li; pslot = t < t1 ? tok_pair[tok0 + t] : 0; }
     auto qrow = [&](int t) -> size_t {
@@ -665,6 +669,17 @@
         return t - t0 < lpr ? (size_t)__shfl(pslot, base + (t - t0), 64) : (size_t)tok_pair[tok0 + t];
     };
     const int nk = t1 - t0;
+    if ((flags & 8) && nk == 1) {
+        const size_t vr = qrow(t0);
+        if (active) {
+            float v[8];
+            load8<T>(vbase + vr * ldkv + ccol, v);
+#pragma unroll
+            for (int c = 0; c < 8; ++c) v[c] += 0.f;
+            store8<T>(ctx + brow(t0) * H + col, v);
+        }
+        return;
+    }
     if constexpr (sizeof(T) == 2) {
         if (nk <= ATT_FAST_KEYS && (flags & 2)) {
             const bool mine = li < nk && (uniform || tok_key[tok0 + t0 + li] != 0);
@@ -679,7 +694,7 @@
                     if (!cls_only) qq[j] = *(const uint4*)(qbase + kr * ldq + ccol);
                 }
             }
-            if (cls_only) qq[0] = *(const uint4*)(qbase + (size_t)rl * ldq + ccol);
+            if (cls_only) qq[0] = *(const uint4*)(qbase + brow(t0) * ldq + ccol);
             const float sc2 = scaling * 1.4426950408889634f;
 #pragma unroll
             for (int qi = 0; qi < ATT_FAST_KEYS; ++qi) {
@@ -714,7 +729,7 @@
 #pragma unroll
                     for (int c = 0; c < 8; ++c) acc[c] *= inv;
                     if (active) {
-                        const size_t orow = cls_only ? (size_t)rl : brow(t0 + qi);
+                        const size_t orow = brow(t0 + qi);
                         store8<T>(ctx + orow * H + col, acc);
                     }
                 }
@@ -724,7 +739,7 @@
     }
     for (int qi = 0; qi < nq; ++qi) {
         float q[8];
-        load8<T>(qbase + (cls_only ? (size_t)rl : qrow(t0 + qi)) * ldq + ccol, q);
+        load8<T>(qbase + (cls_only ? brow(t0) : qrow(t0 + qi)) * ldq + ccol, q);
         float mx = -INFINITY, l = 0.f, acc[8];
 #pragma unroll
         for (int c = 0; c < 8; ++c) acc[c] = 0.f;
@@ -751,7 +766,7 @@
 #pragma unroll
         for (int c = 0; c < 8; ++c) acc[c] *= inv;
         if (active) {
-            const size_t orow = cls_only ? (size_t)rl : brow(t0 + qi);
+            const size_t orow = brow(t0 + qi);
             store8<T>(ctx + orow * H + col, acc);
         }
     }
@@ -864,6 +879,11 @@
     range_report(range_flag, bad, ZETT_RANGE_BIT_DEST);
 }
 
+static __global__ void compose_rows_kernel(const int64_t* __restrict__ outer, const int64_t* __restrict__ inner, int64_t n, int64_t* __restrict__ out) {
+    const int64_t i = (int64_t)blockIdx.x * blockDim.x + threadIdx.x;
+    if (i < n) out[i] = outer[inner[i]];
+}
+
 static __global__ void dest_rows_check_kernel(const int64_t* __restrict__ rows, int64_t n, int64_t n_dest, int32_t* err) {
     const int64_t i = (int64_t)blockIdx.x * blockDim.x + threadIdx.x;
     if (i < n && rows[i] >= n_dest) atomicMax(err, (int)(i < 0x7ffffffe ? i + 1 : 0x7fffffff));
diff --git a/zett_amd/csrc/rowops_launch.hip.h b/zett_amd/csrc/rowops_launch.hip.h
--- a/zett_amd/csrc/rowops_launch.hip.h
+++ b/zett_amd/csrc/rowops_launch.hip.h
@@ -27,11 +27,11 @@
 template <typename T>
 inline int launch_attention(hipStream_t st, int H, int attention_fast, int attention_pack, const T* q, size_t ldq, const T* k, const T* v, size_t ldkv,
                             int head_dim, const int32_t* row_offset, const uint8_t* row_uniform, const uint8_t* tok_key, int64_t row0, int rows, int tok0,
-                            float scaling, int cls_only, const int32_t* tok_pair, T* ctx) {
+                            float scaling, int cls_only, const int32_t* tok_pair, T* ctx, const int32_t* cls_slot = nullptr, int skip_single = 0) {
     const int64_t waves = attention_waves(rows, H, attention_pack != 0).total;
-    const int flags = (cls_only ? 1 : 0) | (attention_fast ? 2 : 0) | (attention_pack ? 4 : 0);
+    const int flags = (cls_only ? 1 : 0) | (attention_fast ? 2 : 0) | (attention_pack ? 4 : 0) | (skip_single ? 8 : 0);
     hipLaunchKernelGGL((attention_rows_kernel<T>), dim3((unsigned)((waves + 3) / 4)), dim3(256), 0, st, q, ldq, k, v, ldkv, H, head_dim, row_offset,
-                       row_uniform, tok_key, row0, rows, tok0, scaling, flags, tok_pair, ctx);
+                       row_uniform, tok_key, row0, rows, tok0, scaling, flags, tok_pair, ctx, cls_slot);
     return flags;
 }
 
diff --git a/zett_amd/csrc/zett_hip.hip b/zett_amd/csrc/zett_hip.hip
--- a/zett_amd/csrc/zett_hip.hip
+++ b/zett_amd/csrc/zett_hip.hip
@@ -97,6 +97,12 @@
     DevBuf dest_word, dest_stage[2], dest_sink;
     int32_t* dest_host = nullptr;
     hipEvent_t dest_checked = nullptr;
+    int single_rows = 1;
+    int64_t single_rows_last = 0;
+    DevBuf single_map;
+    void* single_host = nullptr;
+    size_t single_host_bytes = 0;
+    hipEvent_t single_copied = nullptr;
     std::vector<hipEvent_t> ev;
     size_t ev_used = 0;
     std::vector<zett_gemm_record> gemm_log;
@@ -368,8 +374,10 @@
         if (kv.second.lo && kv.second.lo != (void*)kv.second.f32) (void)hipFree(kv.second.lo);
     }
     for (void* p : h->owned) (void)hipFree(p);
-    for (DevBuf* b : {&h->table, &h->x0, &h->yf, &h->yt, &h->big, &h->pre, &h->ctx, &h->cf, &h->ct, &h->lnstats, &h->lnparts, &h->dest_word, &h->dest_stage[0], &h->dest_stage[1], &h->dest_sink})
+    for (DevBuf* b : {&h->table, &h->x0, &h->yf, &h->yt, &h->big, &h->pre, &h->ctx, &h->cf, &h->ct, &h->lnstats, &h->lnparts, &h->dest_word, &h->dest_stage[0], &h->dest_stage[1], &h->dest_sink, &h->single_map})
         b->release();
+    if (h->single_host) (void)hipHostFree(h->single_host);
+    if (h->single_copied) (void)hipEventDestroy(h->single_copied);
     for (zett_hypernet::PlanSlot* psp : {&h->plan[0], &h->plan[1], &h->table_plan}) {
         zett_hypernet::PlanSlot& ps = *psp;
         ps.i32.release(); ps.u8.release();
@@ -591,6 +599,9 @@
         h->gemm4d_min_k = (int)value;
     } else if (k == "range_accumulate") {
         h->range_accumulate = value != 0;
+    } else if (k == "single_rows") {
+        if (value < 0 || value > 2) return fail(ZETT_E_INVALID, "single_rows must be 0 (off), 1 (auto) or 2 (whenever a call is one chunk on one lane)");
+        h->single_rows = (int)value;
     } else if (k == "gemm_variant") {
         if (value != 0 && value != 1 && value != 2 && value != 3 && value != 7 && value != 8)
             return fail(ZETT_E_INVALID, "gemm_variant must be 0 (auto), 1 (128x128), 2 (256x256 register-staged), 3 (384x256), 7 (256x256 four-wave direct-to-LDS) or 8 (7 with the generic epilogue drain)");
@@ -615,6 +626,12 @@
 int zett_get_stats(const zett_hypernet* h, zett_stats* out) {
     if (!h || !out) return fail(ZETT_E_INVALID, "null argument");
     *out = h->stats;
+    return 0;
+}
+
+int zett_single_rows(const zett_hypernet* h, int64_t* out) {
+    if (!h || !out) return fail(ZETT_E_INVALID, "null argument");
+    *out = h->single_rows_last;
     return 0;
 }
 
@@ -1185,6 +1202,10 @@
     float* TBL = nullptr; T* TBL16 = nullptr; float* TBLST = nullptr;
     const float* lang_vec = nullptr;
     const float scaling = 1.0f / std::sqrt((float)(H / c.heads));
+    int n_s = 0;
+    const int32_t* cls_slot = nullptr;
+    const int64_t* cls_row = nullptr;
+    const int64_t* out_rows = nullptr;
 
     int run() {
         h->stats = zett_stats{};
@@ -1198,6 +1219,7 @@
         if (!h->ext.table)
             table_phase<T>(R, lane_workspace<T>(h, 0, MCS), p.id_list, 0, D, src, src_dtype, MC, mode.table_lo, TBL16, TBLST, TBL);
         if (R.rc) return R.rc;
+        if (int rc = plan_single_rows()) return rc;
         if (int rc = run_chunks(guard)) return rc;
         h->out_recorded = true;
         return h->time_gemm ? read_gemm_timing(h, st) : 0;
@@ -1270,6 +1292,46 @@
         return 0;
     }
 
+    int plan_single_rows() {
+        h->single_rows_last = 0;
+        if (!h->single_rows || seq + (c.embed_lang ? 1 : 0) <= 1 || Ttot > MC || two_lanes()) return 0;
+        int64_t ns = 0;
+        for (int64_t n = 0; n < N; ++n) ns += hoff[n + 1] - hoff[n] == 1;
+        if (ns == 0 || (h->single_rows == 1 && (ns / 256) * (int64_t)(2 * H / 256) < 256)) return 0;
+        const size_t map_bytes = (size_t)N * 12, comp_at = round_up(map_bytes, 16);
+        if (h->single_copied) HIP_TRY(hipEventSynchronize(h->single_copied));
+        else HIP_TRY(hipEventCreateWithFlags(&h->single_copied, hipEventDisableTiming));
+        if (h->single_host_bytes < map_bytes) {
+            if (h->single_host) (void)hipHostFree(h->single_host);
+            h->single_host = nullptr; h->single_host_bytes = 0;
+            HIP_TRY(hipHostMalloc(&h->single_host, map_bytes, hipHostMallocDefault));
+            h->single_host_bytes = map_bytes;
+        }
+        if (int rc = h->single_map.reserve(comp_at + (size_t)N * 8)) return rc;
+        int64_t* hrow = (int64_t*)h->single_host;
+        int32_t* hslot = (int32_t*)(hrow + N);
+        int64_t at_single = 0, at_other = ns;
+        for (int64_t n = 0; n < N; ++n) {
+            const int64_t slot = hoff[n + 1] - hoff[n] == 1 ? at_single++ : at_other++;
+            hslot[n] = (int32_t)slot;
+            hrow[slot] = n;
+        }
+        HIP_TRY(hipMemcpyAsync(h->single_map.p, h->single_host, map_bytes, hipMemcpyHostToDevice, st));
+        HIP_TRY(hipEventRecord(h->single_copied, st));
+        n_s = (int)ns;
+        cls_row = h->single_map.as<int64_t>();
+        cls_slot = (const int32_t*)(cls_row + N);
+        out_rows = cls_row;
+        if (dest && dest->rows) {
+            int64_t* comp = (int64_t*)((char*)h->single_map.p + comp_at);
+            hipLaunchKernelGGL(compose_rows_kernel, dim3((unsigned)((N + 255) / 256)), dim3(256), 0, st, dest->rows, cls_row, N, comp);
+            HIP_TRY(hipGetLastError());
+            out_rows = comp;
+        }
+        h->single_rows_last = ns;
+        return 0;
+    }
+
     struct Chunk {
         int64_t r0; int rows, tok0, m; hipStream_t st; int ev_mode; Workspace<T> w;
         float* hs_sum; float* hs_stats; const float* hs_gamma; const float* hs_beta;
@@ -1301,7 +1363,7 @@
     void embeddings(Chunk& k) {
         LnEmbed emb{TBL, p.tok_slot, p.tok_pos, R.Wf("model.embeddings.token_type_embeddings.weight"),
                     R.Wf("model.embeddings.position_embeddings.weight"), lang_vec, seq, p.tok_row, p.row_offset, k.r0, k.rows,
-                    mode.table_lo ? (const void*)TBL16 : nullptr, TBLST, R.Wf("input_projection.1.ln.weight"), R.Wf("input_projection.1.ln.bias")};
+                    mode.table_lo ? (const void*)TBL16 : nullptr, TBLST, R.Wf("input_projection.1.ln.weight"), R.Wf("input_projection.1.ln.bias"), cls_slot};
         k.hs_sum = k.w.Zf;
         k.hs_stats = k.w.STb;
         k.hs_gamma = R.Wf("model.embeddings.LayerNorm.weight");
@@ -1313,7 +1375,7 @@
         if (k.pairs) {
             emb.tok_slot = p.pair_tslot; emb.tok_pos = p.pair_pos; emb.tok_row = nullptr;
             R.layernorm(nullptr, k.P, k.hs_gamma, k.hs_beta, c.ln_eps_encoder, nullptr, k.w.Zt, k.hs_stats, LnReadout{}, -1, &emb, 0, sum);
-            hipLaunchKernelGGL(pair_rows_kernel, dim3((k.m + 255) / 256), dim3(256), 0, k.st, k.m, k.tok0, k.r0, k.rows, p, p.tok_pkey);
+            hipLaunchKernelGGL(pair_rows_kernel, dim3((k.m + 255) / 256), dim3(256), 0, k.st, k.m, k.tok0, k.r0, k.rows, p, p.tok_pkey, cls_slot);
             R.check("pair_rows");
             h->stats.distinct_positions = k.P;
         } else {
@@ -1327,27 +1389,39 @@
         const T* wqkv = k.raw ? (const T*)h->fold_qkv[l].w : (const T*)h->qkv_w[l];
         const float* bqkv = k.raw ? h->fold_qkv[l].b : h->qkv_b[l];
         const float* cqkv = k.raw ? h->fold_qkv[l].c : nullptr;
-        auto qkv = [&](int col0, int cols, int M, T* out) {
+        auto qkv = [&](int col0, int cols, int row0, int M, T* out, size_t ld) {
             GemmEpilogue<T> e = R.epi();
-            e.bias = bqkv + col0; e.out_lo = out; e.ld_lo = cols;
-            if (k.raw) { e.fold_stats = k.hs_stats; e.fold_c = cqkv + col0; }
-            R.gemm(w.Zt, H, wqkv + (size_t)col0 * H, H, M, cols, H, e);
+            e.bias = bqkv + col0; e.out_lo = out + (size_t)row0 * ld; e.ld_lo = (int)ld;
+            if (k.raw) { e.fold_stats = k.hs_stats + 2 * (size_t)row0; e.fold_c = cqkv + col0; }
+            R.a_rows_readable = k.w.a_rows - row0;
+            R.gemm(w.Zt + (size_t)row0 * H, H, wqkv + (size_t)col0 * H, H, M - row0, cols, H, e);
+            R.a_rows_readable = k.w.a_rows;
         };
         const bool by_pair = !cls_only && k.pairs && l == 0;
         const T* Q = w.BIG;
         const T* KV = w.BIG + H;
         size_t ld_q = (size_t)3 * H, ld_kv = (size_t)3 * H;
         if (!cls_only) {
-            qkv(0, 3 * H, by_pair ? k.P : k.m, w.BIG);
+            if (n_s && !by_pair) {
+                qkv(0, 2 * H, n_s, k.m, w.BIG, ld_q);
+                qkv(2 * H, H, 0, k.m, w.BIG + 2 * H, ld_q);
+            } else {
+                qkv(0, 3 * H, 0, by_pair ? k.P : k.m, w.BIG, ld_q);
+            }
         } else {
-            qkv(H, 2 * H, k.m, w.BIG);
-            qkv(0, H, k.rows, w.BIG + (size_t)k.m * 2 * H);
             KV = w.BIG; Q = w.BIG + (size_t)k.m * 2 * H;
             ld_q = (size_t)H; ld_kv = (size_t)2 * H;
+            if (n_s) {
+                qkv(H, H, n_s, k.m, w.BIG, ld_kv);
+                qkv(2 * H, H, 0, k.m, w.BIG + H, ld_kv);
+            } else {
+                qkv(H, 2 * H, 0, k.m, w.BIG, ld_kv);
+            }
+            qkv(0, H, n_s, k.rows, w.BIG + (size_t)k.m * 2 * H, ld_q);
             k.zrows = k.rows;
         }
         launch_attention<T>(k.st, H, h->attention_fast, h->attention_pack, Q, ld_q, KV, KV + H, ld_kv, H / c.heads, p.row_offset, p.row_uniform, p.tok_key,
-                            k.r0, k.rows, k.tok0, scaling, cls_only ? 1 : 0, by_pair ? (const int32_t*)p.tok_pair : (const int32_t*)nullptr, w.CTX);
+                            k.r0, k.rows, k.tok0, scaling, cls_only ? 1 : 0, by_pair ? (const int32_t*)p.tok_pair : (const int32_t*)nullptr, w.CTX, cls_slot, n_s ? 1 : 0);
         R.check(cls_only ? "attention(position 0)" : "attention");
     }
 
@@ -1428,6 +1502,11 @@
             if (int rc = h->dest_sink.reserve((size_t)N * sizeof(float))) return rc;
             ro.out_bias = h->dest_sink.as<float>() + k.r0;
         }
+        if (n_s && (!dest || dest->bias)) {
+            ro.bias_rows = out_rows;
+            if (!dest) bias_dtype = ZETT_F32;
+            else ro.out_bias = (float*)dest->bias;
+        }
         ro.range_flag = h->range_word;
         ro.in_lo = mode.lo_stream ? (const T*)k.w.Zt : (const T*)nullptr;
         R.layernorm(k.hs_sum, k.rows, k.hs_gamma, k.hs_beta, c.ln_eps_encoder, k.w.Cf, k.w.Ct, nullptr, ro, bias_dtype);
@@ -1436,6 +1515,7 @@
 
     DestOut dest_out(void* base, int64_t ld, int64_t r0) const {
         const size_t es = dest->dtype == ZETT_F32 ? 4 : 2;
+        if (n_s) return DestOut{base, out_rows, ld, dest->dtype};
         return DestOut{dest->rows ? base : (void*)((char*)base + (size_t)r0 * (size_t)ld * es), dest->rows ? dest->rows + r0 : nullptr, ld, dest->dtype};
     }
 
@@ -1456,6 +1536,9 @@
         const T* wl = fold ? (const T*)f.w : R.Wlo(name + ".1.weight");
         if (dest) {
             const DestOut d = dest_out(dst, ld_dst, k.r0), d_b = split ? dest_out(dst_b, ld_dst_b, k.r0) : DestOut{};
+            R.head_gemm(w.CTX, wl, k.rows, width, H, e, &d, split ? &d_b : nullptr, E);
+        } else if (n_s) {
+            const DestOut d{out, out_rows, E, ZETT_F32}, d_b{out_b, out_rows, E, ZETT_F32};
             R.head_gemm(w.CTX, wl, k.rows, width, H, e, &d, split ? &d_b : nullptr, E);
         } else {
             e.out_f32 = out + (size_t)k.r0 * E;
diff --git a/zett_amd/hypernet.py b/zett_amd/hypernet.py
--- a/zett_amd/hypernet.py
+++ b/zett_amd/hypernet.py
@@ -108,6 +108,11 @@
         s = _lib.ZettStats()
         _lib.check(self.lib.zett_get_stats(self.handle, C.byref(s)))
         return {n: getattr(s, n) for n, _ in s._fields_}
+
+    def single_rows(self) -> int:
+        out = C.c_int64(0)
+        _lib.check(self.lib.zett_single_rows(self.handle, C.byref(out)), "zett_single_rows")
+        return out.value
 
     def prepare(self, surface_forms: torch.Tensor, input_stream: Optional["torch.cuda.Stream"] = None) -> None:
         if surface_forms.dtype != torch.int32 or not surface_forms.is_contiguous() or surface_forms.device != self.device or surface_forms.dim() != 2:
```

Measured after the change: 631,400 (median of 6 runs). +1.1%, better.
